# inferenceengine/shadernn

Measured on NVIDIA B200. Metric: frames/sec, higher is better.
Workload: dtype f32 (split-fp16 hi+lo storage for activations and weights, 3 fp16 MMAs per product, fp32 accumulate)

## Files before the change

### include/snnb.h

```cpp
#ifndef SNNB_H_
#define SNNB_H_

#include <stddef.h>
#include <stdint.h>

#ifdef __cplusplus
extern "C" {
#endif

#define SNNB_VERSION 100

typedef struct snnb_context snnb_context;
typedef struct snnb_tensor snnb_tensor;
typedef struct snnb_weights snnb_weights;
typedef struct snnb_model snnb_model;
typedef struct snnb_timer snnb_timer;

enum { SNNB_ACT_NONE = 0, SNNB_ACT_RELU = 1, SNNB_ACT_RELU6 = 2, SNNB_ACT_TANH = 3, SNNB_ACT_SIGMOID = 4, SNNB_ACT_LEAKY_RELU = 5, SNNB_ACT_SILU = 6, SNNB_ACT_SOFTMAX = 7 };
enum { SNNB_PAD_NONE = 0, SNNB_PAD_CONSTANT = 1, SNNB_PAD_REPLICATE = 2, SNNB_PAD_REFLECT = 3 };
enum { SNNB_ALGO_AUTO = 0, SNNB_ALGO_SIMT = 1, SNNB_ALGO_TCGEN05 = 2, SNNB_ALGO_TCGEN05_STREAMK = 3 };
enum { SNNB_PRECISION_FP32X3 = 0, SNNB_PRECISION_FP16W = 1, SNNB_PRECISION_FP16 = 2 };

int snnb_context_create(int device, snnb_context** out);
int snnb_context_destroy(snnb_context* ctx);
// ... 48 lines not shown
int snnb_instancenorm_launch(snnb_context* ctx, const snnb_weights* w, int activation, float leaky_alpha, const snnb_tensor* in, snnb_tensor* out);
int snnb_subpixel_launch(snnb_context* ctx, int r, const snnb_tensor* in, snnb_tensor* out);

int snnb_timer_create(snnb_context* ctx, snnb_timer** out);
int snnb_timer_start(snnb_timer* t);
int snnb_timer_stop(snnb_timer* t);
int snnb_timer_elapsed_ms(snnb_timer* t, float* ms);
int snnb_timer_destroy(snnb_timer* t);

typedef struct snnb_graph snnb_graph;
int snnb_graph_capture_begin(snnb_context* ctx);
int snnb_graph_capture_end(snnb_context* ctx, snnb_graph** out);
int snnb_graph_launch(snnb_graph* g);
int snnb_graph_destroy(snnb_graph* g);

typedef struct {
    int batch;
    int input_width;
    int input_height;
    int conv_algo;
    int use_cuda_graph;
    int fuse;
    int precision;
} snnb_model_options;

int snnb_model_load_json(snnb_context* ctx, const char* json_path, const snnb_model_options* opt, snnb_model** out);
int snnb_model_destroy(snnb_model* m);
int snnb_model_num_layers(const snnb_model* m);
int snnb_model_layer_info(const snnb_model* m, int i, char* name, int name_cap, char* type, int type_cap, int* n, int* h, int* w, int* c);
int snnb_model_num_inputs(const snnb_model* m);
int snnb_model_num_outputs(const snnb_model* m);
int snnb_model_input_dims(const snnb_model* m, int idx, int* n, int* h, int* w, int* c);
int snnb_model_output_dims(const snnb_model* m, int idx, int* n, int* h, int* w, int* c);
int snnb_model_run(snnb_model* m, const float* host_input_nhwc, float* host_output, size_t out_capacity, int* classes_1based);
int snnb_model_submit(snnb_model* m, const float* host_input_nhwc, float* host_output, size_t out_capacity, int* classes_1based, int* ticket);
int snnb_model_submit_u8(snnb_model* m, const uint8_t* host_input_nhwc_u8, const float* mean4, const float* norm4, float* host_output, size_t out_capacity,
                         int* classes_1based, int* ticket);
typedef struct {
    const uint8_t* input_u8;
    int src_height, src_width;
    int linear_filter;
    float mean4[4], norm4[4];
    float* output_f32;
    size_t output_capacity;
    uint8_t* output_u8;
    float out_scale, out_offset;
    int* classes_1based;
} snnb_image_io;
int snnb_model_submit_image(snnb_model* m, const snnb_image_io* io, int* ticket);
int snnb_model_wait(snnb_model* m, int ticket);
int snnb_model_set_input(snnb_model* m, int idx, const float* host_input_nhwc);
int snnb_model_forward(snnb_model* m);
int snnb_model_get_output(snnb_model* m, int idx, float* host_output, size_t out_capacity);
int snnb_model_layer_output(snnb_model* m, int layer, float* host_nhwc, size_t capacity);
int snnb_model_dump_outputs(snnb_model* m, const char* dir);
int snnb_model_time_layers(snnb_model* m, float* times_ms, int capacity);
int snnb_model_layer_kernel(const snnb_model* m, int layer, char* name, int name_cap);
int snnb_model_launches_per_forward(const snnb_model* m);
int snnb_model_get_boxes(snnb_model* m, int n, float* rows6, int max_rows, int* count);
int snnb_model_weight_arena(snnb_model* m, void** device_ptr, size_t* bytes);

typedef struct snnb_comm snnb_comm;
int snnb_nccl_unique_id(unsigned char id128[128]);
int snnb_nccl_comm_create(snnb_context* ctx, int rank, int world_size, const unsigned char id128[128], snnb_comm** out);
int snnb_nccl_comm_destroy(snnb_comm* comm);
int snnb_bcast_weights(snnb_model* m, snnb_comm* comm, int root);

typedef struct snnb_layer_json snnb_layer_json;
int snnb_layer_json_number(const snnb_layer_json* layer, const char* key, double* out);
int snnb_layer_json_string(const snnb_layer_json* layer, const char* key, char* buf, int cap);
int snnb_layer_json_numbers(const snnb_layer_json* layer, const char* path, const double** data, size_t* count);
typedef struct {
    void* user;
    int (*output_dims)(void* user, int num_inputs, const int* in_hwc, int* out_hwc);
    int (*run)(void* user, snnb_context* ctx, int num_inputs, const snnb_tensor* const* inputs, snnb_tensor* output);
    void (*destroy)(void* user);
} snnb_layer_impl;
typedef int (*snnb_layer_creator)(void* registry_user, const snnb_layer_json* layer, snnb_layer_impl* out);
int snnb_register_layer(const char* type_name, snnb_layer_creator creator, void* registry_user);
int snnb_unregister_layer(const char* type_name);
int snnb_tensor_planes(const snnb_tensor* t, void** hi, void** lo, int* cp);
int snnb_debug_streamk_schedule(int tiles, int num_kb, int sms, int* rows, int capacity);
int snnb_debug_feed_plan(int k, int stride, int pad_x, int ic, int out[5]);

#ifdef __cplusplus
}
#endif
#endif
```

### shadernn_b200/_lib.py

```python
import ctypes as C
import os

HERE = os.path.dirname(os.path.abspath(__file__))
LIB_PATH = os.path.join(HERE, "libsnn_b200.so")

c_float_p = C.POINTER(C.c_float)
c_int_p = C.POINTER(C.c_int)
vp = C.c_void_p


class ConvDesc(C.Structure):
    _fields_ = [
        ("in_channels", C.c_int),
        ("out_channels", C.c_int),
        ("kernel", C.c_int),
        ("stride", C.c_int),
        ("pad_x", C.c_int),
        ("pad_y", C.c_int),
        ("pad_mode", C.c_int),
        ("activation", C.c_int),
        ("leaky_alpha", C.c_float),
        ("algo", C.c_int),
    ]

# ... 29 lines not shown

SIGNATURES = {
    "snnb_version": (C.c_int, []),
    "snnb_last_error": (C.c_char_p, []),
    "snnb_context_create": (C.c_int, [C.c_int, C.POINTER(vp)]),
    "snnb_context_destroy": (C.c_int, [vp]),
    "snnb_sync": (C.c_int, [vp]),
    "snnb_context_stream": (vp, [vp]),
    "snnb_launch_count": (C.c_uint64, [vp]),
    "snnb_context_set_precision": (C.c_int, [vp, C.c_int]),
    "snnb_tensor_alloc": (C.c_int, [vp, C.c_int, C.c_int, C.c_int, C.c_int, C.POINTER(vp)]),
    "snnb_tensor_free": (C.c_int, [vp]),
    "snnb_tensor_dims": (C.c_int, [vp, c_int_p, c_int_p, c_int_p, c_int_p]),
    "snnb_tensor_upload_nhwc": (C.c_int, [vp, vp, vp]),
    "snnb_tensor_download_nhwc": (C.c_int, [vp, vp, vp]),
    "snnb_tensor_upload_c4hw4": (C.c_int, [vp, vp, vp]),
    "snnb_tensor_download_c4hw4": (C.c_int, [vp, vp, vp]),
    "snnb_tensor_dump": (C.c_int, [vp, vp, C.c_char_p]),
    "snnb_weights_pack_conv2d": (C.c_int, [vp, C.POINTER(ConvDesc), vp, vp, vp, vp, vp, vp, C.POINTER(vp)]),
    "snnb_weights_pack_depthwise": (C.c_int, [vp, C.POINTER(ConvDesc), vp, vp, vp, vp, vp, vp, C.POINTER(vp)]),
    "snnb_weights_pack_dense": (C.c_int, [vp, C.c_int, C.c_int, vp, vp, C.POINTER(vp)]),
    "snnb_weights_pack_channels": (C.c_int, [vp, C.c_int, vp, vp, vp, vp, C.POINTER(vp)]),
    "snnb_weights_free": (C.c_int, [vp]),
    "snnb_conv2d_launch": (C.c_int, [vp, C.POINTER(ConvDesc), vp, vp, vp, vp]),
    "snnb_depthwise_launch": (C.c_int, [vp, C.POINTER(ConvDesc), vp, vp, vp]),
    "snnb_maxpool_launch": (C.c_int, [vp, C.c_int, C.c_int, vp, vp]),
    "snnb_avgpool_launch": (C.c_int, [vp, C.c_int, C.c_int, vp, vp]),
    "snnb_add_launch": (C.c_int, [vp, C.c_int, C.c_float, vp, vp, vp]),
    "snnb_batchnorm_launch": (C.c_int, [vp, vp, C.c_int, C.c_float, vp, vp]),
    "snnb_activation_launch": (C.c_int, [vp, C.c_int, C.c_float, vp, vp]),
    "snnb_dense_launch": (C.c_int, [vp, vp, C.c_int, C.c_float, vp, vp]),
    "snnb_softmax_launch": (C.c_int, [vp, vp, vp]),
    "snnb_argmax1": (C.c_int, [vp, vp, c_int_p]),
    "snnb_flatten_launch": (C.c_int, [vp, vp, vp]),
    "snnb_concat_launch": (C.c_int, [vp, vp, vp, vp]),
    "snnb_upsample_launch": (C.c_int, [vp, C.c_float, C.c_int, vp, vp]),
    "snnb_pad_launch": (C.c_int, [vp, C.c_int, C.c_int, C.c_int, vp, vp]),
    "snnb_instancenorm_launch": (C.c_int, [vp, vp, C.c_int, C.c_float, vp, vp]),
    "snnb_subpixel_launch": (C.c_int, [vp, C.c_int, vp, vp]),
    "snnb_timer_create": (C.c_int, [vp, C.POINTER(vp)]),
    "snnb_timer_start": (C.c_int, [vp]),
    "snnb_timer_stop": (C.c_int, [vp]),
    "snnb_timer_elapsed_ms": (C.c_int, [vp, c_float_p]),
    "snnb_timer_destroy": (C.c_int, [vp]),
    "snnb_model_load_json": (C.c_int, [vp, C.c_char_p, C.POINTER(ModelOptions), C.POINTER(vp)]),
    "snnb_model_destroy": (C.c_int, [vp]),
    "snnb_model_num_layers": (C.c_int, [vp]),
    "snnb_model_layer_info": (C.c_int, [vp, C.c_int, C.c_char_p, C.c_int, C.c_char_p, C.c_int, c_int_p, c_int_p, c_int_p, c_int_p]),
    "snnb_model_num_inputs": (C.c_int, [vp]),
    "snnb_model_num_outputs": (C.c_int, [vp]),
    "snnb_model_input_dims": (C.c_int, [vp, C.c_int, c_int_p, c_int_p, c_int_p, c_int_p]),
    "snnb_model_output_dims": (C.c_int, [vp, C.c_int, c_int_p, c_int_p, c_int_p, c_int_p]),
    "snnb_model_run": (C.c_int, [vp, vp, vp, C.c_size_t, vp]),
    "snnb_graph_capture_begin": (C.c_int, [vp]),
    "snnb_graph_capture_end": (C.c_int, [vp, C.POINTER(C.c_void_p)]),
    "snnb_graph_launch": (C.c_int, [vp]),
    "snnb_graph_destroy": (C.c_int, [vp]),
    "snnb_model_submit": (C.c_int, [vp, vp, vp, C.c_size_t, vp, c_int_p]),
    "snnb_model_submit_u8": (C.c_int, [vp, vp, vp, vp, vp, C.c_size_t, vp, c_int_p]),
    "snnb_model_submit_image": (C.c_int, [vp, C.POINTER(ImageIO), c_int_p]),
    "snnb_model_wait": (C.c_int, [vp, C.c_int]),
    "snnb_model_set_input": (C.c_int, [vp, C.c_int, vp]),
    "snnb_model_forward": (C.c_int, [vp]),
    "snnb_model_get_output": (C.c_int, [vp, C.c_int, vp, C.c_size_t]),
    "snnb_model_layer_output": (C.c_int, [vp, C.c_int, vp, C.c_size_t]),
    "snnb_model_dump_outputs": (C.c_int, [vp, C.c_char_p]),
    "snnb_model_time_layers": (C.c_int, [vp, c_float_p, C.c_int]),
    "snnb_model_launches_per_forward": (C.c_int, [vp]),
    "snnb_model_layer_kernel": (C.c_int, [vp, C.c_int, C.c_char_p, C.c_int]),
    "snnb_model_get_boxes": (C.c_int, [vp, C.c_int, c_float_p, C.c_int, c_int_p]),
    "snnb_model_weight_arena": (C.c_int, [vp, C.POINTER(vp), C.POINTER(C.c_size_t)]),
    "snnb_nccl_unique_id": (C.c_int, [C.c_char_p]),
    "snnb_nccl_comm_create": (C.c_int, [vp, C.c_int, C.c_int, C.c_char_p, C.POINTER(vp)]),
    "snnb_nccl_comm_destroy": (C.c_int, [vp]),
    "snnb_bcast_weights": (C.c_int, [vp, vp, C.c_int]),
    "snnb_register_layer": (C.c_int, [C.c_char_p, vp, vp]),
    "snnb_unregister_layer": (C.c_int, [C.c_char_p]),
    "snnb_layer_json_number": (C.c_int, [vp, C.c_char_p, C.POINTER(C.c_double)]),
    "snnb_layer_json_string": (C.c_int, [vp, C.c_char_p, C.c_char_p, C.c_int]),
    "snnb_layer_json_numbers": (C.c_int, [vp, C.c_char_p, C.POINTER(C.POINTER(C.c_double)), C.POINTER(C.c_size_t)]),
    "snnb_tensor_planes": (C.c_int, [vp, C.POINTER(vp), C.POINTER(vp), c_int_p]),
    "snnb_debug_streamk_schedule": (C.c_int, [C.c_int, C.c_int, C.c_int, c_int_p, C.c_int]),
    "snnb_debug_feed_plan": (C.c_int, [C.c_int, C.c_int, C.c_int, C.c_int, c_int_p]),
}

_lib = None


class SnnbError(RuntimeError):
    pass


def lib():
    global _lib
    if _lib is None:
        if not os.path.exists(LIB_PATH):
            raise SnnbError(
                "%s is missing — build it with `python -m shadernn_b200._build` (or __graft_entry__.build()). "
                "shadernn_b200 has no CPU or PyTorch fallback." % LIB_PATH)
        l = C.CDLL(LIB_PATH)
        for name, (res, args) in SIGNATURES.items():
            fn = getattr(l, name)
            fn.restype = res
            fn.argtypes = args
        _lib = l
    return _lib


def check(rc, what=""):
    if rc != 0:
        msg = lib().snnb_last_error()
        raise SnnbError("%s failed (status %d): %s" % (what or "snnb call", rc, msg.decode("utf-8", "replace") if msg else "?"))
```

### shadernn_b200/csrc/capi.cpp

```cpp
#include <cstdarg>
#include <cstdlib>
#include <cstring>
#include <memory>

#include "snnb_internal.h"

namespace snnb {

static thread_local char g_err[1024] = "";
void set_error(const char* fmt, ...) {
    va_list ap;
    va_start(ap, fmt);
    vsnprintf(g_err, sizeof(g_err), fmt, ap);
    va_end(ap);
}
const char* get_error() { return g_err; }

bool pdl_enabled() {
    static const bool on = getenv("SNNB_NO_PDL") == nullptr;
    return on;
}

int ensure_stage(snnb_context* ctx, size_t bytes) {
    if (ctx->stage_dev_bytes < bytes) {
// ... 37 lines not shown
    const size_t plane  = ((size_t) t->n * feed_h * feed_w * 4 + 63) / 64 * 64;
    const size_t planes = t->lo ? 2 : 1;
    SNNB_CUDA_OK(cudaMalloc(&t->feed_hi, plane * planes * sizeof(__half)));
    SNNB_CUDA_OK(cudaMemsetAsync(t->feed_hi, 0, plane * planes * sizeof(__half), t->ctx->stream));
    t->feed_lo = t->lo ? t->feed_hi + plane : nullptr;
    t->feed_h = feed_h, t->feed_w = feed_w, t->feed_py = py, t->feed_px = px;
    return 0;
}

}

using namespace snnb;

#define CHECK_DIMS_EQ(a, b, what) SNNB_REQUIRE((a)->n == (b)->n && (a)->h == (b)->h && (a)->w == (b)->w && (a)->c == (b)->c, what ": tensor dims differ")

extern "C" {

int snnb_version(void) { return SNNB_VERSION; }
int snnb_context_set_precision(snnb_context* ctx, int precision) {
    SNNB_REQUIRE(ctx && (precision == SNNB_PRECISION_FP32X3 || precision == SNNB_PRECISION_FP16W), "snnb_context_set_precision: FP32X3 or FP16W (FP16 storage is a model option)");
    ctx->precision = precision;
    return 0;
}
const char* snnb_last_error(void) { return get_error(); }

int snnb_context_create(int device, snnb_context** out) {
    SNNB_REQUIRE(out, "snnb_context_create: null out");
    int count = 0;
    cudaError_t e = cudaGetDeviceCount(&count);
    if (e != cudaSuccess || count == 0) {
        set_error("snnb_context_create: no CUDA device available (%s). This library has no CPU fallback.", cudaGetErrorString(e));
        return 1;
    }
    SNNB_REQUIRE(device >= 0 && device < count, "snnb_context_create: device %d out of range (%d devices)", device, count);
    SNNB_CUDA_OK(cudaSetDevice(device));
    cudaDeviceProp prop;
    SNNB_CUDA_OK(cudaGetDeviceProperties(&prop, device));
    SNNB_REQUIRE(prop.major == 10, "snnb_context_create: device %d is sm_%d%d; this library is built for sm_100a (B200) only", device, prop.major, prop.minor);
    auto ctx      = std::make_unique<snnb_context>();
    ctx->device   = device;
    ctx->sm_count = prop.multiProcessorCount;
    SNNB_CUDA_OK(cudaStreamCreateWithFlags(&ctx->stream, cudaStreamNonBlocking));
    *out = ctx.release();
    return 0;
}

int snnb_context_destroy(snnb_context* ctx) {
    if (!ctx) return 0;
    cudaSetDevice(ctx->device);
    cudaStreamSynchronize(ctx->stream);
    if (ctx->stage_dev) cudaFree(ctx->stage_dev);
    if (ctx->stage_host) cudaFreeHost(ctx->stage_host);
    for (void* b : ctx->scratch_blocks) cudaFree(b);
    cudaStreamDestroy(ctx->stream);
    delete ctx;
    return 0;
}

int snnb_sync(snnb_context* ctx) {
    SNNB_REQUIRE(ctx, "snnb_sync: null context");
    SNNB_CUDA_OK(cudaStreamSynchronize(ctx->stream));
    return 0;
}
void* snnb_context_stream(snnb_context* ctx) { return ctx ? (void*) ctx->stream : nullptr; }
uint64_t snnb_launch_count(snnb_context* ctx) { return ctx ? ctx->launches : 0; }

int snnb_tensor_alloc(snnb_context* ctx, int n, int h, int w, int c, snnb_tensor** out) { return tensor_alloc(ctx, n, h, w, c, out); }
int snnb_tensor_free(snnb_tensor* t) {
    if (!t) return 0;
    if (t->owns && t->hi) cudaFree(t->hi);
    if (t->feed_hi) cudaFree(t->feed_hi);
    delete t;
    return 0;
}
int snnb_debug_feed_plan(int k, int stride, int pad_x, int ic, int out[5]) {
    FeedPlan fp;
    if (!out || !make_feed_plan(k, stride, pad_x, ic, fp)) return 0;
    out[0] = fp.px, out[1] = fp.d, out[2] = fp.nch, out[3] = fp.ksteps, out[4] = fp.rows_per_panel;
    return 1;
}
int snnb_debug_streamk_schedule(int tiles, int num_kb, int sms, int* rows, int capacity) {
    SNNB_REQUIRE(rows || capacity == 0, "snnb_debug_streamk_schedule: null buffer");
    return streamk_schedule(tiles, num_kb, sms, rows, capacity);
}
int snnb_tensor_planes(const snnb_tensor* t, void** hi, void** lo, int* cp) {
    SNNB_REQUIRE(t && hi && lo && cp, "snnb_tensor_planes: null argument");
    *hi = t->hi, *lo = t->lo, *cp = t->cp;
    return 0;
}
int snnb_tensor_dims(const snnb_tensor* t, int* n, int* h, int* w, int* c) {
    SNNB_REQUIRE(t, "snnb_tensor_dims: null tensor");
    if (n) *n = t->n;
    if (h) *h = t->h;
    if (w) *w = t->w;
    if (c) *c = t->c;
    return 0;
}
int snnb_tensor_upload_nhwc(snnb_context* ctx, snnb_tensor* t, const float* host) {
    SNNB_REQUIRE(ctx && t && host, "snnb_tensor_upload_nhwc: null argument");
    const size_t bytes = t->pixels() * t->c * sizeof(float);
    if (ensure_stage(ctx, bytes)) return 1;
    SNNB_CUDA_OK(cudaMemcpyAsync(ctx->stage_dev, host, bytes, cudaMemcpyHostToDevice, ctx->stream));
    if (launch_split_f32(ctx, ctx->stage_dev, t)) return 1;
    SNNB_CUDA_OK(cudaStreamSynchronize(ctx->stream));
    return 0;
}
int snnb_tensor_download_nhwc(snnb_context* ctx, const snnb_tensor* t, float* host) {
    SNNB_REQUIRE(ctx && t && host, "snnb_tensor_download_nhwc: null argument");
    const size_t bytes = t->pixels() * t->c * sizeof(float);
    if (ensure_stage(ctx, bytes)) return 1;
    if (launch_merge_f32(ctx, t, ctx->stage_dev)) return 1;
    SNNB_CUDA_OK(cudaMemcpyAsync(host, ctx->stage_dev, bytes, cudaMemcpyDeviceToHost, ctx->stream));
    SNNB_CUDA_OK(cudaStreamSynchronize(ctx->stream));
    return 0;
}

static void c4_to_nhwc(const float* c4, int N, int H, int W, int C, float* nhwc) {
    const int D = (C + 3) / 4;
    for (int n = 0; n < N; ++n)
        for (int y = 0; y < H; ++y)
            for (int x = 0; x < W; ++x)
                for (int c = 0; c < C; ++c)
                    nhwc[(((size_t) n * H + y) * W + x) * C + c] = c4[((((size_t) n * D + c / 4) * H + y) * W + x) * 4 + (c % 4)];
}
static void nhwc_to_c4(const float* nhwc, int N, int H, int W, int C, float* c4) {
    const int D = (C + 3) / 4;
    memset(c4, 0, sizeof(float) * (size_t) N * D * H * W * 4);
    for (int n = 0; n < N; ++n)
        for (int y = 0; y < H; ++y)
            for (int x = 0; x < W; ++x)
                for (int c = 0; c < C; ++c)
                    c4[((((size_t) n * D + c / 4) * H + y) * W + x) * 4 + (c % 4)] = nhwc[(((size_t) n * H + y) * W + x) * C + c];
}
int snnb_tensor_upload_c4hw4(snnb_context* ctx, snnb_tensor* t, const float* host_c4) {
    SNNB_REQUIRE(ctx && t && host_c4, "snnb_tensor_upload_c4hw4: null argument");
    std::vector<float> tmp(t->pixels() * t->c);
    c4_to_nhwc(host_c4, t->n, t->h, t->w, t->c, tmp.data());
    return snnb_tensor_upload_nhwc(ctx, t, tmp.data());
}
int snnb_tensor_download_c4hw4(snnb_context* ctx, const snnb_tensor* t, float* host_c4) {
    SNNB_REQUIRE(ctx && t && host_c4, "snnb_tensor_download_c4hw4: null argument");
    std::vector<float> tmp(t->pixels() * t->c);
    if (snnb_tensor_download_nhwc(ctx, t, tmp.data())) return 1;
    nhwc_to_c4(tmp.data(), t->n, t->h, t->w, t->c, host_c4);
    return 0;
}
int snnb_tensor_dump(snnb_context* ctx, const snnb_tensor* t, const char* path) {
    SNNB_REQUIRE(ctx && t && path, "snnb_tensor_dump: null argument");
    const int D = (t->c + 3) / 4;
    std::vector<float> c4((size_t) t->n * D * t->h * t->w * 4);
    if (snnb_tensor_download_c4hw4(ctx, t, c4.data())) return 1;
    for (int n = 0; n < t->n; ++n) {
        std::string p = path;
        if (t->n > 1) p += ".n" + std::to_string(n);
        FILE* f = fopen(p.c_str(), "wb");
        SNNB_REQUIRE(f, "snnb_tensor_dump: cannot open %s", p.c_str());
        char header[32];
        memset(header, 0, sizeof(header));
        snprintf(header, sizeof(header), "%d %d %d %d", t->w, t->h, D, t->c);
        fwrite(header, 1, sizeof(header), f);
        fwrite(c4.data() + (size_t) n * D * t->h * t->w * 4, sizeof(float), (size_t) D * t->h * t->w * 4, f);
        fclose(f);
    }
    return 0;
}

// ... 244 lines not shown
```

### shadernn_b200/csrc/engine/core.cpp

```cpp
#include <algorithm>
#include <cstring>
#include <unordered_map>
#include <unordered_set>

#include "engine.h"

using namespace snnb;

namespace snn {

using namespace dp;

MixedInferenceCore::~MixedInferenceCore() {
    if (ctx) {
        cudaSetDevice(ctx->device);
        cudaStreamSynchronize(ctx->stream);
    }
    if (cuGraphExec) cudaGraphExecDestroy(cuGraphExec);
    if (cuGraph) cudaGraphDestroy(cuGraph);
    for (auto* t : ownedTensors) snnb_tensor_free(t);
    if (arena) cudaFree(arena);
    if (scratchArena) cudaFree(scratchArena);
    if (ioStage) cudaFree(ioStage);
    if (argmaxDev) cudaFree(argmaxDev);
    if (yoloDev) cudaFree(yoloDev);
    if (yoloHost) cudaFreeHost(yoloHost);
    for (auto& sl : slots) {
        if (sl.yoloDev) cudaFree(sl.yoloDev);
        if (sl.yoloHost) cudaFreeHost(sl.yoloHost);
        if (sl.stageIn) cudaFree(sl.stageIn);
        if (sl.stageResize) cudaFree(sl.stageResize);
        if (sl.stageOut) cudaFree(sl.stageOut);
        if (sl.smallHost) cudaFreeHost(sl.smallHost);
        if (sl.argmax) cudaFree(sl.argmax);
        if (sl.h2dDone) cudaEventDestroy(sl.h2dDone);
        if (sl.stageFree) cudaEventDestroy(sl.stageFree);
        if (sl.resultReady) cudaEventDestroy(sl.resultReady);
    }
    if (copyStream) cudaStreamDestroy(copyStream);
}

std::unique_ptr<MixedInferenceCore> MixedInferenceCore::create(snnb_context* ctx, const std::string& modelFileName, const ShaderGenOptions& options,
                                                               std::string& err) {
    std::unique_ptr<MixedInferenceCore> core(new MixedInferenceCore());
    core->ctx     = ctx;
    core->options = options;
    try {
        core->layers = loadFromJsonModel(modelFileName);
        core->graph  = generateInferenceGraph(core->layers, options);
    } catch (std::exception& e) {
        err = e.what();
        return nullptr;
    }
    if (!core->init(err)) return nullptr;
    return core;
}

static bool allZeroPadding(const PaddingSpec& p) {
    uint32_t o[4];
    p.offsets(3, true, o);
    const bool keyword_same = !(p.t == "valid" || p.t == "none" || (!p.t.empty() && std::all_of(p.t.begin(), p.t.end(), ::isdigit)));
    return !keyword_same && o[0] == 0 && o[1] == 0 && o[2] == 0 && o[3] == 0;
}

bool MixedInferenceCore::init(std::string& err) {
    const int N = (int) options.batch;
    const bool twoPlanes = options.precision != SNNB_PRECISION_FP16;
    std::unordered_map<GenericModelLayer*, int> order;
    for (size_t i = 0; i < graph.sorted.size(); ++i) order[graph.sorted[i]] = (int) i;

    for (auto* L : graph.sorted) {
        if (L->isInputLayer) inputLayers.push_back(L);
        if (L->nextLayers.empty()) outputLayers.push_back(L);
        if (L->typeName == "YOLO") yolo = static_cast<YOLOLayer*>(L);
    }
    std::stable_sort(inputLayers.begin(), inputLayers.end(), [](GenericModelLayer* a, GenericModelLayer* b) {
        return static_cast<InputLayerLayer*>(a)->_desc.inputIndex < static_cast<InputLayerLayer*>(b)->_desc.inputIndex;
    });
    if (inputLayers.empty()) {
        err = "model has no InputLayer";
        return false;
    }

    std::unordered_map<GenericModelLayer*, GenericModelLayer*> alias;
    if (options.fuse) {
        for (auto* L : graph.sorted) {
            if (L->typeName == "Pad" && L->nextLayers.size() == 1 && L->prevLayers.size() == 1) {
                auto* pad  = static_cast<PadLayer*>(L);
                auto* next = L->nextLayers[0];
                PaddingSpec* np = nullptr;
                if (next->typeName == "Conv2D" && static_cast<Conv2DLayer*>(next)->_desc.kernelSize > 1) np = &static_cast<Conv2DLayer*>(next)->_desc.padding;
                if (next->typeName == "SeparableConv2D" && pad->mode == "constant") np = &static_cast<SeparableConv2DLayer*>(next)->_desc.padding;
                if (np && allZeroPadding(*np)) {
                    uint32_t o[4];
                    pad->padding.offsets(0, false, o);
                    np->t = std::to_string(o[0]), np->b = std::to_string(o[1]), np->l = std::to_string(o[2]), np->r = std::to_string(o[3]);
                    np->mode       = pad->mode;
                    L->fusedAway   = true;
                    alias[L]       = L->prevLayers[0];
                }
            }
            if (L->typeName == "Add" && L->prevLayers.size() == 2) {
                auto* add = static_cast<AddLayer*>(L);
                GenericModelLayer* a = L->prevLayers[0];
                GenericModelLayer* b = L->prevLayers[1];
                auto fusable = [&](GenericModelLayer* c, GenericModelLayer* other) {
                    if (c->typeName != "Conv2D" || c->nextLayers.size() != 1 || c->fusedAway) return false;
                    auto* conv = static_cast<Conv2DLayer*>(c);
                    if (conv->_desc.activation.id != SNNB_ACT_NONE || conv->residual || conv->fusedAct >= 0) return false;
                    return order[other] < order[c] && c != other;
                };
                GenericModelLayer* conv = nullptr;
                GenericModelLayer* other = nullptr;
                if (fusable(b, a))
                    conv = b, other = a;
                else if (fusable(a, b))
                    conv = a, other = b;
                if (conv) {
                    conv->fusedAct   = add->activation.id;
                    conv->fusedAlpha = add->activation.alpha;
                    conv->prevLayers.push_back(other);
                    L->fusedAway     = true;
                    alias[conv]      = L;
                }
            }
            if (L->typeName == "Dense" && L->prevLayers.size() == 1) {
                GenericModelLayer* f = L->prevLayers[0];
                GenericModelLayer* pool = (f->typeName == "Flatten" && f->prevLayers.size() == 1 && f->nextLayers.size() == 1 &&
                                           static_cast<FlattenLayer*>(f)->activation.id == SNNB_ACT_NONE)
                                              ? f->prevLayers[0]
                                              : f;
                auto dimsOf = [&](GenericModelLayer* x) { return graph.outputDims[order[x]]; };
                if (pool->typeName == "AveragePooling2D" && static_cast<PoolingLayer*>(pool)->isAvg && pool->nextLayers.size() == 1 && pool->prevLayers.size() == 1 &&
                    !pool->fusedAway && dimsOf(pool).width * dimsOf(pool).height == 1 && static_cast<DenseLayer*>(L)->units <= 256 &&
                    dimsOf(pool->prevLayers[0]).width * dimsOf(pool->prevLayers[0]).height >= 4 && dimsOf(pool->prevLayers[0]).depth <= 4096 &&
                    static_cast<PoolingLayer*>(pool)->_desc.kernelSize >= dimsOf(pool->prevLayers[0]).width &&
                    static_cast<PoolingLayer*>(pool)->_desc.kernelSize >= dimsOf(pool->prevLayers[0]).height) {
                    static_cast<DenseLayer*>(L)->gapSource = pool->prevLayers[0];
                    pool->fusedAway = true;
                }
            }
            if (L->typeName == "Flatten" && L->inputDims.size() == 1 && L->inputDims[0].width * L->inputDims[0].height == 1 &&
                static_cast<FlattenLayer*>(L)->activation.id == SNNB_ACT_NONE) {
                L->fusedAway = true;
                alias[L]     = L->prevLayers[0];
            }
        }
    }

    std::unordered_map<GenericModelLayer*, snnb_tensor*> outOf;
    auto resolve = [&](GenericModelLayer* L) -> GenericModelLayer* {
        std::unordered_set<GenericModelLayer*> seen;
        while (alias.count(L) && !seen.count(L)) {
            seen.insert(L);
            L = alias[L];
        }
        return L;
    };
    for (size_t i = 0; i < graph.sorted.size(); ++i) {
        GenericModelLayer* L = graph.sorted[i];
        if (L->typeName == "YOLO") continue;
        GenericModelLayer* owner = resolve(L);
        if (owner != L && !(L->typeName == "Conv2D")) continue;
        if (outOf.count(owner)) continue;
        const Dims& d = graph.outputDims[order[owner]];
        snnb_tensor* t = nullptr;
        if (tensor_alloc(ctx, N, (int) d.height, (int) d.width, (int) d.depth, &t, twoPlanes)) {
            err = get_error();
            return false;
        }
        ownedTensors.push_back(t);
        outOf[owner] = t;
    }
    for (auto* L : graph.sorted) {
        if (L->typeName == "YOLO") {
            for (auto* p : L->prevLayers) L->inputs.push_back(outOf.at(resolve(p)));
            continue;
        }
        GenericModelLayer* owner = resolve(L);
        L->output                = outOf.count(owner) ? outOf[owner] : nullptr;
        if (L->fusedAway) continue;
        size_t nin = L->prevLayers.size();
        if (L->typeName == "Conv2D" && static_cast<Conv2DLayer*>(L)->fusedAct >= 0) {
            nin -= 1;
            L->residual = outOf.at(resolve(L->prevLayers.back()));
        }
        for (size_t k = 0; k < nin; ++k) L->inputs.push_back(outOf.at(resolve(L->prevLayers[k])));
        if (L->typeName == "Conv2D") {
            auto* cl  = static_cast<Conv2DLayer*>(L);
            cl->algo = options.convAlgo;
            int ph = 0, pw = 0;
            snnb_weights probe_w;
            probe_w.w_hi = probe_w.w_lo = reinterpret_cast<__half*>(1);
            probe_w.w_row_hi = probe_w.w_row_lo = reinterpret_cast<__half*>(1);
            probe_w.row_stride = (int) cl->_desc.stride, probe_w.row_pad = 0;
            std::swap(cl->weights, probe_w);
            const bool prepad = cl->wantsPrepad(L->inputs[0], L->output, options.convAlgo, ph, pw);
            std::swap(cl->weights, probe_w);
            if (prepad) {
                if (tensor_alloc(ctx, N, ph, pw, L->inputs[0]->c, &cl->prepadded, twoPlanes)) {
                    err = get_error();
                    return false;
                }
                ownedTensors.push_back(cl->prepadded);
            }
            {
                static const bool noFeed = getenv("SNNB_NO_FEED") != nullptr;
                GenericModelLayer* src   = resolve(L->prevLayers[0]);
                snnb_tensor* in          = L->inputs[0];
                const int mode           = padModeId(cl->_desc.padding.mode);
                uint32_t offs[4];
                cl->_desc.padding.offsets((int) cl->_desc.kernelSize, true, offs);
                const int k = (int) cl->_desc.kernelSize, padX = (int) offs[0], padY = (int) offs[2];
                FeedPlan fp;
                if (!noFeed && !prepad && src->isInputLayer && !in->feed_hi && options.convAlgo != SNNB_ALGO_SIMT && !L->residual && L->output->c <= 64 &&
                    (mode == SNNB_PAD_NONE || mode == SNNB_PAD_CONSTANT) && make_feed_plan(k, (int) cl->_desc.stride, padX, in->c, fp)) {
                    const int tilesX = (L->output->w + 127) / 128;
                    const int needW  = 2 * (tilesX * 128 - 1) + 2 * fp.nch;
                    const int needH  = 2 * (L->output->h - 1) + k - padY + padY;
                    const int feedW  = (std::max(in->w + fp.px, needW) + 1) & ~1;
                    const int feedH  = std::max(in->h + padY, needH);
                    if (tensor_alloc_feed(in, feedH, feedW, padY, fp.px)) {
                        err = get_error();
                        return false;
                    }
                    cl->feedInput = true;
                }
            }
        }
        if (L->typeName == "Dense") {
            auto* dl = static_cast<DenseLayer*>(L);
            if (L->inputs[0]->h * L->inputs[0]->w != 1) {
                if (tensor_alloc(ctx, N, 1, 1, (int) dl->numInputPlanes, &dl->flat, twoPlanes)) {
                    err = get_error();
                    return false;
                }
                ownedTensors.push_back(dl->flat);
            }
            if ((uint32_t) (L->inputs[0]->h * L->inputs[0]->w * L->inputs[0]->c) != dl->numInputPlanes) {
                err = L->name + ": Dense expects " + std::to_string(dl->numInputPlanes) + " inputs, graph provides " +
                      std::to_string(L->inputs[0]->h * L->inputs[0]->w * L->inputs[0]->c);
                return false;
            }
        }
        if ((L->typeName == "Add" || L->typeName == "Concatenate") && L->inputs.size() != 2) {
            err = L->name + ": expects exactly two inputs";
            return false;
        }
        auto dimsStr = [](const snnb_tensor* t) { return std::to_string(t->h) + "x" + std::to_string(t->w) + "x" + std::to_string(t->c); };
        if (L->typeName == "Conv2D" || L->typeName == "SeparableConv2D" || L->typeName == "BatchNormalization" || L->typeName == "InstanceNorm") {
            if (L->inputs.empty() || !L->output) {
                err = L->name + ": layer has no input";
                return false;
            }
            if ((uint32_t) L->inputs[0]->c != L->numInputPlanes) {
                err = L->name + ": inputPlanes " + std::to_string(L->numInputPlanes) + " but the producing layer has " + std::to_string(L->inputs[0]->c) + " channels";
                return false;
            }
            const uint32_t wantOut = (L->typeName == "Conv2D") ? L->numOutputPlanes : L->numInputPlanes;
            if ((uint32_t) L->output->c != wantOut) {
                err = L->name + ": output tensor has " + std::to_string(L->output->c) + " channels, weights are packed for " + std::to_string(wantOut);
                return false;
            }
        }
        if (L->typeName == "Add") {
            for (auto* in : L->inputs)
                if (in->h != L->output->h || in->w != L->output->w || in->c != L->output->c) {
                    err = L->name + ": Add operand " + dimsStr(in) + " does not match the output " + dimsStr(L->output);
                    return false;
                }
        }
        if (L->typeName == "Conv2D" && L->residual &&
            (L->residual->h != L->output->h || L->residual->w != L->output->w || L->residual->c != L->output->c)) {
            err = L->name + ": fused Add operand " + dimsStr(L->residual) + " does not match the output " + dimsStr(L->output);
            return false;
        }
        if (L->typeName == "Concatenate") {
            if (L->inputs[0]->h != L->inputs[1]->h || L->inputs[0]->w != L->inputs[1]->w || L->inputs[0]->c + L->inputs[1]->c != L->output->c ||
                L->inputs[0]->h != L->output->h || L->inputs[0]->w != L->output->w) {
                err = L->name + ": Concatenate operands " + dimsStr(L->inputs[0]) + " and " + dimsStr(L->inputs[1]) + " do not stack into " + dimsStr(L->output);
                return false;
            }
        }
    }

    for (auto* in : inputLayers) {
        snnb_tensor* t = in->output;
        if (!t || !t->feed_hi || getenv("SNNB_NO_FEED_ONLY")) continue;
        bool only = true;
        int readers = 0;
        for (auto* L : graph.sorted) {
            if (L->fusedAway || L->isInputLayer) continue;
            const bool reads = std::find(L->inputs.begin(), L->inputs.end(), t) != L->inputs.end() || L->residual == t;
            if (!reads) continue;
            ++readers;
            only = only && L->typeName == "Conv2D" && static_cast<Conv2DLayer*>(L)->feedInput && L->inputs.size() >= 1 && L->inputs[0] == t && L->residual != t &&
                   std::count(L->inputs.begin(), L->inputs.end(), t) == 1;
        }
        for (auto* o : outputLayers) only = only && o->output != t;
        t->feed_only = only && readers > 0;
    }

    std::vector<std::pair<GenericModelLayer*, PackedHost>> packed;
    size_t total = 0, scratchTotal = 0;
    for (auto* L : graph.sorted) {
        PackedHost p;
        try {
            L->packWeights(p);
        } catch (std::exception& e) {
            err = L->name + ": " + e.what();
            return false;
        }
        if (p.kind) {
            total += p.device_bytes();
            packed.emplace_back(L, std::move(p));
        }
        if (L->typeName == "InstanceNorm") {
            static_cast<InstanceNormLayer*>(L)->computeScratch(N);
            scratchTotal += (L->scratchBytes() + 255) & ~(size_t) 255;
        }
    }
    arenaBytes = total ? total : 256;
    if (cudaMalloc(&arena, arenaBytes) != cudaSuccess) {
        err = "cudaMalloc(weight arena) failed";
        return false;
    }
    {
        char* cur = (char*) arena;
        for (auto& pr : packed) {
            if (place_weights(ctx, pr.second, cur, &pr.first->weights)) {
                err = get_error();
                return false;
            }
            cur += pr.first->weights.bytes;
        }
    }
    if (scratchTotal) {
        if (cudaMalloc(&scratchArena, scratchTotal) != cudaSuccess) {
            err = "cudaMalloc(scratch) failed";
            return false;
        }
        char* cur = (char*) scratchArena;
        for (auto* L : graph.sorted)
            if (L->scratchBytes()) {
                L->scratch = (float*) cur;
                cur += (L->scratchBytes() + 255) & ~(size_t) 255;
            }
    }

    size_t maxFloats = 1;
    for (auto* L : inputLayers) maxFloats = std::max(maxFloats, L->output->pixels() * (size_t) L->output->c);
    for (auto* L : outputLayers)
        if (L->output) maxFloats = std::max(maxFloats, L->output->pixels() * (size_t) L->output->c);
    ioStageBytes = maxFloats * sizeof(float);
    if (cudaMalloc(&ioStage, ioStageBytes) != cudaSuccess || cudaMalloc(&argmaxDev, sizeof(int) * N) != cudaSuccess) {
        err = "cudaMalloc(io staging) failed";
        return false;
    }
    if (yolo) {
        const size_t yb = yolo->candidateBytes();
        if (cudaMalloc(&yoloDev, yb) != cudaSuccess || cudaMallocHost(&yoloHost, yb) != cudaSuccess) {
            err = "cudaMalloc(YOLO candidate lists) failed";
            return false;
        }
    }
    {
        GenericModelLayer* last = nullptr;
        for (auto* L : outputLayers)
            if (L->output) {
                last = L;
                break;
            }
        isClassifier = last && last->output->h == 1 && last->output->w == 1 && last->output->c > 1;
    }

    const uint64_t before = ctx->launches;
// ... 160 lines not shown
    const bool resize = io && (io->src_height != in->h || io->src_width != in->w);
    const size_t inBytes = resize ? (size_t) in->n * io->src_height * io->src_width * in->c : in->pixels() * in->c * (u8 ? sizeof(uint8_t) : sizeof(float));
    const size_t outFloats = out ? out->pixels() * out->c : 0;
    SNNB_REQUIRE(!hostOutput || capacityFloats >= outFloats, "submit: output buffer too small (%zu < %zu floats)", capacityFloats, outFloats);
    SNNB_REQUIRE(!(io && io->output_u8) || (out && io->output_capacity >= outFloats), "submit_image: u8 output buffer too small or the model has no tensor output");
    void* stage = sl.stageIn;
    if (resize) {
        if (inBytes > sl.stageResizeBytes) {
            SNNB_CUDA_OK(cudaStreamSynchronize(ctx->stream));
            if (sl.stageResize) SNNB_CUDA_OK(cudaFree(sl.stageResize));
            SNNB_CUDA_OK(cudaMalloc(&sl.stageResize, inBytes));
            sl.stageResizeBytes = inBytes;
        }
        stage = sl.stageResize;
    }
    if (sl.everUsed) SNNB_CUDA_OK(cudaStreamWaitEvent(copyStream, sl.stageFree, 0));
    SNNB_CUDA_OK(cudaMemcpyAsync(stage, hostInput, inBytes, cudaMemcpyHostToDevice, copyStream));
    SNNB_CUDA_OK(cudaEventRecord(sl.h2dDone, copyStream));
    SNNB_CUDA_OK(cudaStreamWaitEvent(ctx->stream, sl.h2dDone, 0));
    if (resize) {
        if (launch_resize_u8(ctx, reinterpret_cast<const uint8_t*>(stage), io->src_height, io->src_width, in, mean, norm, io->linear_filter != 0)) return 1;
    } else if (u8 ? launch_split_u8(ctx, reinterpret_cast<const uint8_t*>(sl.stageIn), in, mean, norm) : launch_split_f32(ctx, sl.stageIn, in)) {
        return 1;
    }
    SNNB_CUDA_OK(cudaEventRecord(sl.stageFree, ctx->stream));
    if (forward()) return 1;
    sl.userOut = nullptr, sl.userClasses = nullptr, sl.userFloats = 0;
    static const bool noSmall = getenv("SNNB_NO_SMALL_RESULT") != nullptr;
    const bool small = !noSmall && isClassifier && !(io && io->output_u8) && (hostOutput || classes1) &&
                       outFloats * sizeof(float) + options.batch * sizeof(int) <= SMALL_RESULT_BYTES;
    if (small) {
        float* vals = static_cast<float*>(sl.smallDev);
        int* cls    = reinterpret_cast<int*>(static_cast<char*>(sl.smallDev) + outFloats * sizeof(float));
        if (launch_result_small(ctx, out, hostOutput ? vals : nullptr, classes1 ? cls : nullptr)) return 1;
        sl.userOut = hostOutput, sl.userClasses = classes1, sl.userFloats = outFloats;
        hostOutput = nullptr, classes1 = nullptr;
    }
    if (hostOutput) {
        if (launch_merge_f32(ctx, out, sl.stageOut)) return 1;
        SNNB_CUDA_OK(cudaMemcpyAsync(hostOutput, sl.stageOut, outFloats * sizeof(float), cudaMemcpyDeviceToHost, ctx->stream));
    }
    if (io && io->output_u8) {
        if (launch_merge_u8(ctx, out, reinterpret_cast<uint8_t*>(sl.stageOut), io->out_scale, io->out_offset)) return 1;
        SNNB_CUDA_OK(cudaMemcpyAsync(io->output_u8, sl.stageOut, outFloats, cudaMemcpyDeviceToHost, ctx->stream));
    }
    sl.classesHost = nullptr;
    if (classes1 && isClassifier) {
        if (launch_argmax(ctx, out, sl.argmax)) return 1;
        SNNB_CUDA_OK(cudaMemcpyAsync(classes1, sl.argmax, sizeof(int) * options.batch, cudaMemcpyDeviceToHost, ctx->stream));
        sl.classesHost = classes1;
    }
    if (yolo && decodeYolo(sl.yoloDev, sl.yoloHost, false)) return 1;
    SNNB_CUDA_OK(cudaEventRecord(sl.resultReady, ctx->stream));
    sl.busy = sl.everUsed = true;
    *ticket = nextTicket++;
    return 0;
}

int MixedInferenceCore::wait(int ticket) {
    SNNB_REQUIRE(ticket >= 0 && ticket < nextTicket && ticket >= nextTicket - 2, "wait: ticket %d is not in flight", ticket);
    Slot& sl = slots[ticket & 1];
    SNNB_REQUIRE(sl.busy, "wait: ticket %d was already waited for", ticket);
    SNNB_CUDA_OK(cudaEventSynchronize(sl.resultReady));
    if (sl.userOut) std::memcpy(sl.userOut, sl.smallHost, sl.userFloats * sizeof(float));
    if (sl.userClasses) {
        const int* cls = reinterpret_cast<const int*>(static_cast<const char*>(sl.smallHost) + sl.userFloats * sizeof(float));
        for (uint32_t i = 0; i < options.batch; ++i) sl.userClasses[i] = cls[i] + 1;
    }
    sl.userOut = nullptr, sl.userClasses = nullptr;
    if (sl.classesHost)
        for (uint32_t i = 0; i < options.batch; ++i) sl.classesHost[i] += 1;
    sl.busy = false;
    if (yolo) {
        const int rc = yolo->finishDecode(sl.yoloHost, sl.yoloDev, boxes);
        SNNB_REQUIRE(rc >= 0, "wait: corrupt detection candidate list");
        return rc;
    }
    return 0;
}

int MixedInferenceCore::layerOutput(int layerId, float* host, size_t capacityFloats) {
    SNNB_REQUIRE(layerId >= 0 && layerId < (int) layers.size() && host, "layerOutput: bad argument");
    GenericModelLayer* L = layers[layerId].get();
    SNNB_REQUIRE(L->output, "layerOutput: layer %d (%s) has no device tensor", layerId, L->name.c_str());
    SNNB_REQUIRE(!(L->typeName == "Conv2D" && static_cast<Conv2DLayer*>(L)->fusedAct >= 0),
                 "layerOutput: layer %d (%s) was fused into its Add; load the model with fuse=0 to observe it", layerId, L->name.c_str());
    SNNB_REQUIRE(!(L->fusedAway && L->typeName == "AveragePooling2D"),
                 "layerOutput: layer %d (%s) was fused into the classifier head (pool + Dense in one launch); load the model with fuse=0 to observe it", layerId,
                 L->name.c_str());
    const size_t floats = L->output->pixels() * L->output->c;
    SNNB_REQUIRE(capacityFloats >= floats, "layerOutput: buffer too small (%zu < %zu floats)", capacityFloats, floats);
    return snnb_tensor_download_nhwc(ctx, L->output, host);
}

int MixedInferenceCore::timeLayers(std::vector<float>& ms) {
    ms.assign(layers.size(), 0.0f);
    std::vector<cudaEvent_t> ev(graph.sorted.size() + 1);
    for (auto& e : ev) SNNB_CUDA_OK(cudaEventCreate(&e));
    ExecOptions eo;
    eo.convAlgo = options.convAlgo, eo.precision = options.precision;
    SNNB_CUDA_OK(cudaEventRecord(ev[0], ctx->stream));
    layerKernels.assign(layers.size(), std::string());
    for (size_t i = 0; i < graph.sorted.size(); ++i) {
        GenericModelLayer* L = graph.sorted[i];
        if (!(L->fusedAway || L->isInputLayer || L->typeName == "YOLO")) {
            ctx->last_kernel = nullptr;
            if (int rc = L->run(ctx, eo)) return rc;
            layerKernels[L->layerId] = ctx->last_kernel ? ctx->last_kernel : (L->typeName + " kernels");
        }
        SNNB_CUDA_OK(cudaEventRecord(ev[i + 1], ctx->stream));
    }
    SNNB_CUDA_OK(cudaStreamSynchronize(ctx->stream));
    for (size_t i = 0; i < graph.sorted.size(); ++i) {
        float t = 0;
        SNNB_CUDA_OK(cudaEventElapsedTime(&t, ev[i], ev[i + 1]));
        ms[graph.sorted[i]->layerId] = t;
    }
    for (auto& e : ev) cudaEventDestroy(e);
    return 0;
}

int MixedInferenceCore::dumpOutputs(const std::string& dir) {
    for (auto& l : layers) {
        if (!l->output || l->fusedAway) continue;
        SNNB_REQUIRE(!(l->typeName == "Conv2D" && l->fusedAct >= 0), "dumpOutputs: %s was fused into its Add; load the model with fuse=0 to dump every layer", l->name.c_str());
        std::string path = dir + "/" + l->name + " pass[0].dump";
        if (snnb_tensor_dump(ctx, l->output, path.c_str())) return 1;
    }
    return 0;
}

}
```

### shadernn_b200/csrc/engine/engine.h

```cpp
#pragma once

#include <algorithm>
#include <map>
#include <memory>
#include <string>
#include <vector>

#include "../snnb_internal.h"
#include "json.h"

namespace snn {

struct SNNModelOutputBoxes {
    std::vector<std::vector<float>> rows;
};

namespace dp {

class ModelParser {
public:
    explicit ModelParser(const std::string& fileName);
    ~ModelParser();
    int getLayerCount() const;
    std::string getLayerName(int layerId) const;
// ... 30 lines not shown
    int id      = SNNB_ACT_NONE;
    float alpha = 0.0f;
    static int fromString(const std::string& s);
};

struct ExecOptions;

class GenericModelLayer {
public:
    virtual ~GenericModelLayer() {}
    std::string name;
    std::string typeName;
    int layerId = -1;
    std::vector<GenericModelLayer*> prevLayers, nextLayers;
    std::vector<Dims> inputDims;
    uint32_t numInputPlanes = 0, numOutputPlanes = 0;
    bool isInputLayer = false;

    virtual void getOutputDims(uint32_t& width, uint32_t& height, uint32_t& depth) const;
    struct Transform { float scaleW = 1, scaleH = 1, transW = 0, transH = 0; };
    virtual Transform getOutputScaleDimAdjustment() const { return Transform(); }

    virtual void packWeights(snnb::PackedHost&) {}
    snnb_weights weights;
    std::vector<snnb_tensor*> inputs;
    snnb_tensor* output = nullptr;
    virtual int run(snnb_context* ctx, const ExecOptions& opt) = 0;
    bool fusedAway          = false;
    snnb_tensor* residual   = nullptr;
    int fusedAct            = -1;
    float fusedAlpha        = 0.0f;
    float* scratch          = nullptr;
    size_t scratchBytes() const { return _scratchBytes; }

protected:
    size_t _scratchBytes = 0;
};

class PluginLayer : public GenericModelLayer {
public:
    snnb_layer_impl impl {};
    ~PluginLayer() override {
        if (impl.destroy) impl.destroy(impl.user);
    }
    void getOutputDims(uint32_t& w, uint32_t& h, uint32_t& d) const override;
    int run(snnb_context* ctx, const ExecOptions& opt) override;
};

typedef GenericModelLayer* (*LayerCreator)(ModelParser&, int);
void initLayerRegisty();
void registerLayer(const std::string& layerName, LayerCreator creator);
GenericModelLayer* createLayerInstance(std::string layerName, ModelParser& parser, int i);

struct InputLayerDesc {
    uint32_t inputWidth = 0, inputHeight = 0, inputChannels = 0, inputIndex = 0;
    void parse(ModelParser& parser, int layerId);
};
class InputLayerLayer : public GenericModelLayer {
public:
    InputLayerDesc _desc;
    void getOutputDims(uint32_t& w, uint32_t& h, uint32_t& d) const override;
    int run(snnb_context*, const ExecOptions&) override { return 0; }
};

struct GenericConvDesc {
    uint32_t kernelSize = 1, stride = 1;
    PaddingSpec padding;
    ActivationSpec activation;
    std::string activationName;
    std::vector<float> weights;
    std::vector<float> biases;
    bool useBatchNormalization = false;
    std::map<std::string, std::vector<float>> batchNormalization;
};
struct Conv2DDesc : GenericConvDesc {
    void parse(ModelParser& parser, int layerId);
};
class Conv2DLayer : public GenericModelLayer {
public:
    Conv2DDesc _desc;
    int algo = SNNB_ALGO_AUTO;
    snnb_tensor* prepadded = nullptr;
    bool feedInput = false;
    bool wantsPrepad(const snnb_tensor* in, const snnb_tensor* out, int convAlgo, int& ph, int& pw) const;
    Transform getOutputScaleDimAdjustment() const override;
    void getOutputDims(uint32_t& w, uint32_t& h, uint32_t& d) const override;
    void packWeights(snnb::PackedHost& p) override;
    int run(snnb_context* ctx, const ExecOptions& opt) override;
};
struct SeparableConv2DDesc : GenericConvDesc {
    void parse(ModelParser& parser, int layerId);
};
class SeparableConv2DLayer : public GenericModelLayer {
public:
    SeparableConv2DDesc _desc;
    void getOutputDims(uint32_t& w, uint32_t& h, uint32_t& d) const override;
    void packWeights(snnb::PackedHost& p) override;
    int run(snnb_context* ctx, const ExecOptions& opt) override;
};
struct PoolDesc {
    uint32_t kernelSize = 1, stride = 1;
    PaddingSpec padding;
    void parseMax(ModelParser& parser, int layerId);
    void parseAvg(ModelParser& parser, int layerId);
};
class PoolingLayer : public GenericModelLayer {
public:
    PoolDesc _desc;
    bool isAvg = false;
    Transform getOutputScaleDimAdjustment() const override;
    int run(snnb_context* ctx, const ExecOptions& opt) override;
};
class AdaptiveAvgPool2dLayer : public GenericModelLayer {
public:
    uint32_t poolSize = 1;
    void getOutputDims(uint32_t& w, uint32_t& h, uint32_t& d) const override;
    int run(snnb_context* ctx, const ExecOptions& opt) override;
};
class AddLayer : public GenericModelLayer {
public:
    ActivationSpec activation;
    int run(snnb_context* ctx, const ExecOptions& opt) override;
};
class BatchNormalizationLayer : public GenericModelLayer {
public:
    std::map<std::string, std::vector<float>> batchNormalization;
    ActivationSpec activation;
    void packWeights(snnb::PackedHost& p) override;
    int run(snnb_context* ctx, const ExecOptions& opt) override;
};
class InstanceNormLayer : public GenericModelLayer {
public:
    std::vector<float> gamma, beta;
    ActivationSpec activation;
    void packWeights(snnb::PackedHost& p) override;
    int run(snnb_context* ctx, const ExecOptions& opt) override;
    void setScratch() { _scratchBytes = 0; }
    void computeScratch(int n) { _scratchBytes = snnb::instnorm_scratch_floats(n, snnb::round_up((int) numOutputPlanes, 8)) * sizeof(float); }
};
class ActivationLayer : public GenericModelLayer {
public:
    ActivationSpec activation;
    int run(snnb_context* ctx, const ExecOptions& opt) override;
};
class DenseLayer : public GenericModelLayer {
public:
    std::vector<float> kernel;
    std::vector<float> biases;
    ActivationSpec activation;
    uint32_t units = 0;
    void getOutputDims(uint32_t& w, uint32_t& h, uint32_t& d) const override;
    void packWeights(snnb::PackedHost& p) override;
    int run(snnb_context* ctx, const ExecOptions& opt) override;
    snnb_tensor* flat = nullptr;
    GenericModelLayer* gapSource = nullptr;
};
class FlattenLayer : public GenericModelLayer {
public:
    ActivationSpec activation;
    void getOutputDims(uint32_t& w, uint32_t& h, uint32_t& d) const override;
    int run(snnb_context* ctx, const ExecOptions& opt) override;
};
class ConcatenateLayer : public GenericModelLayer {
public:
    void getOutputDims(uint32_t& w, uint32_t& h, uint32_t& d) const override;
    int run(snnb_context* ctx, const ExecOptions& opt) override;
// ... 126 lines not shown
```

### shadernn_b200/csrc/engine/layers.cpp

```cpp
#include <algorithm>
#include <cmath>

#include <cstring>
#include <thread>

#include "engine.h"

using namespace snnb;

namespace snn {
namespace dp {

void GenericModelLayer::getOutputDims(uint32_t& width, uint32_t& height, uint32_t& depth) const {
    width = height = depth = 0U;
    float accSW = 0, accSH = 0, accTW = 0, accTH = 0;
    const Transform t = getOutputScaleDimAdjustment();
    for (auto& dim : inputDims) {
        accSW  = std::max(accSW, t.scaleW * dim.width);
        accTW  = std::max(accTW, t.transW);
        accSH  = std::max(accSH, t.scaleH * dim.height);
        accTH  = std::max(accTH, t.transH);
        width  = (uint32_t) (accSW + accTW);
        height = (uint32_t) (accSH + accTH);
        depth  = std::max(depth, dim.depth);
    }
}

void InputLayerLayer::getOutputDims(uint32_t& w, uint32_t& h, uint32_t& d) const {
    w = inputDims.empty() ? _desc.inputWidth : inputDims[0].width;
    h = inputDims.empty() ? _desc.inputHeight : inputDims[0].height;
    d = _desc.inputChannels;
}

GenericModelLayer::Transform Conv2DLayer::getOutputScaleDimAdjustment() const {
    uint32_t offset[4];
    _desc.padding.offsets((int) _desc.kernelSize, true, offset);
    float scale       = 1 / static_cast<float>(_desc.stride);
    float translation = 0.0f;
    if (_desc.kernelSize % 2 != 0) {
        translation = 1 + (static_cast<float>(offset[0] + offset[1]) - static_cast<float>(_desc.kernelSize)) / static_cast<float>(_desc.stride);
    } else {
        translation = 1 + (static_cast<float>(offset[0] + offset[1] - 1) - static_cast<float>(_desc.kernelSize)) / static_cast<float>(_desc.stride);
    }
    return Transform {scale, scale, translation, translation};
}
void Conv2DLayer::getOutputDims(uint32_t& w, uint32_t& h, uint32_t& d) const {
    GenericModelLayer::getOutputDims(w, h, d);
    d = numOutputPlanes;
}
int padModeId(const std::string& m) {
    if (m == "constant") return SNNB_PAD_CONSTANT;
    if (m == "replicate") return SNNB_PAD_REPLICATE;
    if (m == "reflect") return SNNB_PAD_REFLECT;
    return SNNB_PAD_NONE;
}
static const float* bnv(const std::map<std::string, std::vector<float>>& bn, const char* key) {
    auto it = bn.find(key);
    return (it == bn.end() || it->second.empty()) ? nullptr : it->second.data();
}
void Conv2DLayer::packWeights(PackedHost& p) {
    const auto& bn = _desc.batchNormalization;
    const bool use = _desc.useBatchNormalization;
    pack_conv2d_host((int) numInputPlanes, (int) numOutputPlanes, (int) _desc.kernelSize, _desc.weights.data(), _desc.biases.empty() ? nullptr : _desc.biases.data(),
                     use ? bnv(bn, "gamma") : nullptr, use ? bnv(bn, "beta") : nullptr, use ? bnv(bn, "movingMean") : nullptr,
                     use ? bnv(bn, "movingVariance") : nullptr, p);
    {
        uint32_t offs[4];
        _desc.padding.offsets((int) _desc.kernelSize, true, offs);
        const int mode = padModeId(_desc.padding.mode);
        if (mode == SNNB_PAD_NONE || mode == SNNB_PAD_CONSTANT) {
            pack_rowwin_host(p, (int) _desc.stride, _desc.kernelSize == 1 ? 0 : (int) offs[0]);
            if (feedInput) pack_feed_host(p, (int) _desc.stride, _desc.kernelSize == 1 ? 0 : (int) offs[0]);
        } else {
            pack_rowwin_host(p, (int) _desc.stride, 0);
        }
    }
    std::vector<float>().swap(_desc.weights);
}
bool Conv2DLayer::wantsPrepad(const snnb_tensor* in, const snnb_tensor* out, int convAlgo, int& ph, int& pw) const {
    const int mode = padModeId(_desc.padding.mode);
    if (!(mode == SNNB_PAD_REPLICATE || mode == SNNB_PAD_REFLECT) || _desc.kernelSize <= 1 || convAlgo == SNNB_ALGO_SIMT) return false;
    ConvArgs probe {in, nullptr, const_cast<snnb_tensor*>(out), &weights, (int) _desc.kernelSize, (int) _desc.stride, 0, 0, SNNB_PAD_CONSTANT, 0, 0.0f};
    if (!conv2d_umma_supported(probe)) return false;
    ph = (out->h - 1) * (int) _desc.stride + (int) _desc.kernelSize;
    pw = (out->w - 1) * (int) _desc.stride + (int) _desc.kernelSize;
    return true;
}

int Conv2DLayer::run(snnb_context* ctx, const ExecOptions& opt) {
    uint32_t offs[4];
    _desc.padding.offsets((int) _desc.kernelSize, true, offs);
    if (prepadded) {
        if (launch_pad(ctx, inputs[0], prepadded, (int) offs[0], (int) offs[2], padModeId(_desc.padding.mode))) return 1;
        ConvArgs a {prepadded, residual, output, &weights, (int) _desc.kernelSize, (int) _desc.stride, 0, 0, SNNB_PAD_CONSTANT,
                    fusedAct >= 0 ? fusedAct : _desc.activation.id, fusedAct >= 0 ? fusedAlpha : _desc.activation.alpha};
        a.precision = opt.precision;
        return launch_conv2d_umma(ctx, a);
    }
    ConvArgs a;
    a.in = inputs[0], a.residual = residual, a.out = output, a.w = &weights;
    a.k = (int) _desc.kernelSize, a.stride = (int) _desc.stride;
    a.pad_x = _desc.kernelSize == 1 ? 0 : (int) offs[0];
    a.pad_y = _desc.kernelSize == 1 ? 0 : (int) offs[2];
    a.pad_mode = padModeId(_desc.padding.mode);
    a.act      = fusedAct >= 0 ? fusedAct : _desc.activation.id;
    a.alpha    = fusedAct >= 0 ? fusedAlpha : _desc.activation.alpha;
    a.precision = opt.precision;
    const int want = algo != SNNB_ALGO_AUTO ? algo : opt.convAlgo;
    if (want != SNNB_ALGO_SIMT && conv2d_umma_supported(a)) return launch_conv2d_umma(ctx, a);
    if (want == SNNB_ALGO_TCGEN05) {
        set_error("%s: tcgen05 path requested but unsupported for this shape", name.c_str());
        return 2;
    }
    return launch_conv2d_simt(ctx, a);
}

void SeparableConv2DLayer::getOutputDims(uint32_t& width, uint32_t& height, uint32_t& depth) const {
    uint32_t po[4];
    _desc.padding.offsets((int) _desc.kernelSize, true, po);
    width = height = depth = 0;
    for (auto& dim : inputDims) {
        width  = (dim.width - _desc.kernelSize + po[0] + po[2]) / _desc.stride + 1;
        height = (dim.height - _desc.kernelSize + po[1] + po[3]) / _desc.stride + 1;
        depth  = dim.depth;
        break;
    }
}
void SeparableConv2DLayer::packWeights(PackedHost& p) {
    const auto& bn = _desc.batchNormalization;
    const bool use = _desc.useBatchNormalization;
    pack_depthwise_host((int) numInputPlanes, (int) _desc.kernelSize, _desc.weights.data(), _desc.biases.empty() ? nullptr : _desc.biases.data(),
                        use ? bnv(bn, "gamma") : nullptr, use ? bnv(bn, "beta") : nullptr, use ? bnv(bn, "movingMean") : nullptr,
                        use ? bnv(bn, "movingVariance") : nullptr, p);
}
int SeparableConv2DLayer::run(snnb_context* ctx, const ExecOptions&) {
    uint32_t offs[4];
    _desc.padding.offsets((int) _desc.kernelSize, true, offs);
    ConvArgs a;
    a.in = inputs[0], a.residual = nullptr, a.out = output, a.w = &weights;
    a.k = (int) _desc.kernelSize, a.stride = (int) _desc.stride;
    a.pad_x = (int) offs[0], a.pad_y = (int) offs[2];
    a.pad_mode = SNNB_PAD_CONSTANT, a.act = _desc.activation.id, a.alpha = _desc.activation.alpha;
    return launch_depthwise(ctx, a);
}

GenericModelLayer::Transform PoolingLayer::getOutputScaleDimAdjustment() const {
    float scale = 1.0f / _desc.stride, translation;
    if (_desc.padding.validLike())
        translation = 1.0f - (static_cast<float>(_desc.kernelSize) / static_cast<float>(_desc.stride));
    else
        translation = 1.0f - 1.0f / static_cast<float>(_desc.stride);
    return Transform {scale, scale, translation, translation};
}
int PoolingLayer::run(snnb_context* ctx, const ExecOptions&) { return launch_pool(ctx, inputs[0], output, (int) _desc.kernelSize, (int) _desc.stride, isAvg); }

void AdaptiveAvgPool2dLayer::getOutputDims(uint32_t& w, uint32_t& h, uint32_t& d) const {
    w = h = poolSize;
    d     = inputDims.empty() ? numOutputPlanes : inputDims[0].depth;
}
int AdaptiveAvgPool2dLayer::run(snnb_context* ctx, const ExecOptions&) {
    const snnb_tensor* in = inputs[0];
    if (in->h % (int) poolSize || in->w % (int) poolSize || in->h / (int) poolSize != in->w / (int) poolSize) {
        set_error("%s: AdaptiveAvgPool2d needs H and W divisible by pool (%d x %d -> %u)", name.c_str(), in->h, in->w, poolSize);
        return 2;
    }
    const int k = in->h / (int) poolSize;
    return launch_pool(ctx, in, output, k, k, true);
}

int AddLayer::run(snnb_context* ctx, const ExecOptions&) { return launch_add(ctx, inputs[0], inputs[1], output, activation.id, activation.alpha); }
void BatchNormalizationLayer::packWeights(PackedHost& p) {
    pack_channels_host((int) numOutputPlanes, bnv(batchNormalization, "gamma"), bnv(batchNormalization, "beta"), bnv(batchNormalization, "movingMean"),
                       bnv(batchNormalization, "movingVariance"), p);
}
int BatchNormalizationLayer::run(snnb_context* ctx, const ExecOptions&) { return launch_batchnorm(ctx, inputs[0], output, &weights, activation.id, activation.alpha); }
void InstanceNormLayer::packWeights(PackedHost& p) { pack_channels_host((int) numOutputPlanes, gamma.data(), beta.data(), nullptr, nullptr, p); }
int InstanceNormLayer::run(snnb_context* ctx, const ExecOptions&) {
    return launch_instancenorm(ctx, inputs[0], output, &weights, activation.id, activation.alpha, scratch);
}
int ActivationLayer::run(snnb_context* ctx, const ExecOptions&) { return launch_activation(ctx, inputs[0], output, activation.id, activation.alpha); }

void DenseLayer::getOutputDims(uint32_t& w, uint32_t& h, uint32_t& d) const {
    w = h = 1;
    d     = units;
}
void DenseLayer::packWeights(PackedHost& p) {
    pack_conv2d_host((int) numInputPlanes, (int) units, 1, kernel.data(), biases.empty() ? nullptr : biases.data(), nullptr, nullptr, nullptr, nullptr, p);
    p.kind = 3;
    std::vector<float>().swap(kernel);
}
int DenseLayer::run(snnb_context* ctx, const ExecOptions& opt) {
    if (gapSource && gapSource->output && gap_dense_supported(gapSource->output, output, &weights))
// ... 227 lines not shown
```

### shadernn_b200/csrc/kernels_umma.cu

```cuda
#include <cuda.h>

#include <algorithm>
#include <vector>
#include <cstdlib>

#include "snnb_internal.h"

namespace snnb {

constexpr int UM_BLOCK_M     = 128;
constexpr int UM_BLOCK_K     = 64;
constexpr int UM_MAX_N       = 128;
constexpr int UM_MAX_N2      = 256;
constexpr int UM_STAGES      = 3;
constexpr int UM_A_BYTES     = UM_BLOCK_M * 128;
constexpr int UM_B_BYTES     = UM_MAX_N * 128;
constexpr int UM_STAGE_BYTES = 2 * UM_A_BYTES + 2 * UM_B_BYTES;
constexpr int UM_EPI_WARPS   = 8;
constexpr int UM_THREADS     = 64 + 32 * UM_EPI_WARPS;
constexpr int UM_ACC_COLS    = 2 * UM_MAX_N;
constexpr int UM_TMEM_COLS   = 2 * UM_ACC_COLS;
constexpr int UM_STG_BYTES   = 2 * UM_BLOCK_M * 128;
constexpr int UM_SCHED_SLOTS = 8;
constexpr int UM_SMEM_BYTES  = UM_STAGES * UM_STAGE_BYTES + UM_STG_BYTES + 1024  + 320 ;
constexpr int UM_SMEM_BYTES_SPLIT = (UM_STAGES - 1) * UM_STAGE_BYTES + 2 * UM_STG_BYTES + 1024 + 320;

constexpr int HL_TW = 8, HL_TH = 16, HL_W = HL_TW + 2, HL_H = HL_TH + 2;
constexpr int HL_PLANE         = (HL_W * HL_H * 128 + 1023) / 1024 * 1024;
constexpr int HL_A_STAGES      = 2;
constexpr int HL_A_STAGE_BYTES = 2 * HL_PLANE;
constexpr int HL_B_STAGES      = 6;
constexpr int HL_B_RING_BYTES  = 6 * UM_B_BYTES;
constexpr int HL_SMEM_BYTES    = HL_A_STAGES * HL_A_STAGE_BYTES + HL_B_RING_BYTES + UM_STG_BYTES + 1024 + 384;

struct UmmaParams {
    __half* out_hi;
    __half* out_lo;
    const __half* res_hi;
    const __half* res_lo;
    const float* bias;
    int N, OH, OW, OC, OCp;
    int tw, th, tn, rows_used;
    int tiles_x, tiles_y, tiles_n, tiles_oc, n_blk;
    int ksize, stride, pad_x, pad_y;
    int cblocks, ICp;
    int act;
    float alpha;
    int has_res;
    int ksplit, kb_per_split;
    int* sched_counter;
    float* partials;
    int* counters;
    long long* trace;
    int ablate;
    int has_lo;
    int sk, sk_dp, sk_ctas;
    long long sk_units;
    int b_stages, b_stage_bytes;
};

__device__ __forceinline__ uint32_t smem_u32(const void* p) { return (uint32_t) __cvta_generic_to_shared(p); }

__device__ __forceinline__ void mbar_init(uint32_t bar, uint32_t count) { asm volatile("mbarrier.init.shared::cta.b64 [%0], %1;" ::"r"(bar), "r"(count)); }
__device__ __forceinline__ void mbar_expect_tx(uint32_t bar, uint32_t bytes) {
    asm volatile("mbarrier.arrive.expect_tx.shared::cta.b64 _, [%0], %1;" ::"r"(bar), "r"(bytes) : "memory");
}
__device__ __forceinline__ void mbar_arrive(uint32_t bar) { asm volatile("mbarrier.arrive.shared::cta.b64 _, [%0];" ::"r"(bar) : "memory"); }
__device__ __forceinline__ bool mbar_try_wait(uint32_t bar, uint32_t parity) {
    uint32_t ok;
    asm volatile(
        "{\n\t.reg .pred p;\n\t"
        "mbarrier.try_wait.parity.shared::cta.b64 p, [%1], %2;\n\t"
        "selp.u32 %0, 1, 0, p;\n\t}"
        : "=r"(ok)
        : "r"(bar), "r"(parity)
        : "memory");
    return ok != 0;
}
__device__ __forceinline__ bool mbar_test_wait(uint32_t bar, uint32_t parity) {
    uint32_t ok;
    asm volatile(
        "{\n\t.reg .pred p;\n\t"
        "mbarrier.test_wait.parity.shared::cta.b64 p, [%1], %2;\n\t"
        "selp.u32 %0, 1, 0, p;\n\t}"
        : "=r"(ok)
        : "r"(bar), "r"(parity)
        : "memory");
    return ok != 0;
}
__device__ unsigned int g_producer_progress[1024];
__device__ __forceinline__ void producer_progress(int lane, unsigned int code) {
    if (lane == 0) *reinterpret_cast<volatile unsigned int*>(&g_producer_progress[blockIdx.x & 1023]) = code;
}
__device__ __forceinline__ void mbar_wait(uint32_t bar, uint32_t parity) {
    if (mbar_try_wait(bar, parity)) return;
    const long long t0 = clock64();
    bool reported      = false;
    while (!mbar_try_wait(bar, parity)) {
        const long long dt = clock64() - t0;
        if (dt > 4000000000LL && !reported) {
            uint32_t dyn;
            asm volatile("mov.u32 %0, %%dynamic_smem_size;" : "=r"(dyn));
            printf("tcgen05 kernel (dynamic smem %u B): mbarrier wait timed out (block %d thread %d bar 0x%x parity %u, producer progress 0x%x)\n", dyn, blockIdx.x,
                   threadIdx.x, bar, parity, *reinterpret_cast<volatile unsigned int*>(&g_producer_progress[blockIdx.x & 1023]));
            reported = true;
        }
        if (dt > 4040000000LL) __trap();
    }
}
__device__ __forceinline__ bool elect_one() {
    uint32_t pred;
    asm volatile("{\n\t.reg .pred p;\n\telect.sync _|p, 0xffffffff;\n\tselp.u32 %0, 1, 0, p;\n\t}" : "=r"(pred));
    return pred != 0;
}
__device__ __forceinline__ void fence_barrier_init() { asm volatile("fence.mbarrier_init.release.cluster;" ::: "memory"); }
__device__ __forceinline__ void tc_fence_before() { asm volatile("tcgen05.fence::before_thread_sync;" ::: "memory"); }
__device__ __forceinline__ void tc_fence_after() { asm volatile("tcgen05.fence::after_thread_sync;" ::: "memory"); }

__device__ __forceinline__ void tma_prefetch_desc(const CUtensorMap* m) { asm volatile("prefetch.tensormap [%0];" ::"l"(m) : "memory"); }
__device__ __forceinline__ void tma_load_4d(uint32_t dst, const CUtensorMap* m, uint32_t bar, int c0, int c1, int c2, int c3) {
    asm volatile("cp.async.bulk.tensor.4d.shared::cluster.global.mbarrier::complete_tx::bytes [%0], [%1, {%3, %4, %5, %6}], [%2];" ::"r"(dst), "l"(m),
                 "r"(bar), "r"(c0), "r"(c1), "r"(c2), "r"(c3)
                 : "memory");
}
__device__ __forceinline__ void tma_load_2d(uint32_t dst, const CUtensorMap* m, uint32_t bar, int c0, int c1) {
    asm volatile("cp.async.bulk.tensor.2d.shared::cluster.global.mbarrier::complete_tx::bytes [%0], [%1, {%3, %4}], [%2];" ::"r"(dst), "l"(m), "r"(bar),
                 "r"(c0), "r"(c1)
                 : "memory");
}

__device__ __forceinline__ void tmem_alloc(uint32_t slot_smem, uint32_t cols) {
    asm volatile("tcgen05.alloc.cta_group::1.sync.aligned.shared::cta.b32 [%0], %1;" ::"r"(slot_smem), "r"(cols) : "memory");
    asm volatile("tcgen05.relinquish_alloc_permit.cta_group::1.sync.aligned;" ::: "memory");
}
__device__ __forceinline__ void tmem_dealloc(uint32_t taddr, uint32_t cols) {
    asm volatile("tcgen05.dealloc.cta_group::1.sync.aligned.b32 %0, %1;" ::"r"(taddr), "r"(cols) : "memory");
}
__device__ __forceinline__ void umma_f16(uint32_t d_tmem, uint64_t a_desc, uint64_t b_desc, uint32_t idesc, uint32_t accumulate) {
    asm volatile(
        "{\n\t.reg .pred p;\n\t"
        "setp.ne.b32 p, %4, 0;\n\t"
// ... 253 lines not shown
        }
        EPI_STAMP(4);
        fence_async_smem();
        EPI_STAMP(5);
        named_bar_sync(e.bar_id, NWARPS * 32);
        EPI_STAMP(6);
        if (leader) {
            if (!e.no_store && elect_one()) {
                tma_store_4d(sw ? e.o_hi64 : e.o_hiT, e.stg, slab_oc, c1, c2, c3);
                if (e.has_lo) tma_store_4d(sw ? e.o_lo64 : e.o_loT, e.stg + UM_BLOCK_M * 128, slab_oc, c1, c2, c3);
                bulk_commit();
            }
            __syncwarp();
        }
        EPI_STAMP(7);
    }
#undef EPI_STAMP
}
template <int NWARPS, int TERMS>
__device__ __forceinline__ void epilogue_dump_partial(const EpiArgs& e, uint32_t taddr, float* dst, int row, int half, int lane) {
    for (int c = (NWARPS == 8 ? half : 0) * 16; c < e.n_blk; c += (NWARPS == 8 ? 32 : 16)) {
        uint32_t r[16], r2[16];
        tmem_ld16(taddr + (uint32_t) c, r);
        if (TERMS == 3) {
            tmem_ld16(taddr + (uint32_t) (e.n_blk + c), r2);
        } else {
#pragma unroll
            for (int j = 0; j < 16; ++j) r2[j] = 0u;
        }
        tmem_ld_wait();
        float4* d = reinterpret_cast<float4*>(dst) + (size_t) (c >> 4) * 4 * UM_BLOCK_M + row;
#pragma unroll
        for (int j4 = 0; j4 < 4; ++j4)
            d[j4 * UM_BLOCK_M] = make_float4(__uint_as_float(r[4 * j4]) + __uint_as_float(r2[4 * j4]), __uint_as_float(r[4 * j4 + 1]) + __uint_as_float(r2[4 * j4 + 1]),
                                __uint_as_float(r[4 * j4 + 2]) + __uint_as_float(r2[4 * j4 + 2]), __uint_as_float(r[4 * j4 + 3]) + __uint_as_float(r2[4 * j4 + 3]));
    }
    tc_fence_before();
    __syncwarp();
    if (lane == 0) mbar_arrive(e.tmem_empty);
}

__device__ __forceinline__ void epilogue_drain(bool leader) {
    if (leader) {
        if (elect_one()) asm volatile("cp.async.bulk.wait_group 0;" ::: "memory");
        __syncwarp();
    }
}

struct WorkItem {
    int tile, kb0, kb1, piece, pieces, slot;
};
template <bool SK>
__host__ __device__ __forceinline__ WorkItem decode_work(const UmmaParams& p, int work, int total_tiles, int num_kb) {
    WorkItem w;
    if constexpr (!SK) {
        const int split = work / total_tiles;
        w.tile = work - split * total_tiles, w.kb0 = split * p.kb_per_split, w.kb1 = w.kb0 + p.kb_per_split < num_kb ? w.kb0 + p.kb_per_split : num_kb;
        w.piece = split, w.pieces = p.ksplit, w.slot = w.tile;
    } else if (work < p.sk_dp) {
        w.tile = work, w.kb0 = 0, w.kb1 = num_kb, w.piece = 0, w.pieces = 1, w.slot = 0;
    } else {
        const int c = (work - p.sk_dp) >> 2, j = (work - p.sk_dp) & 3;
        const long long b0 = (long long) c * p.sk_units / p.sk_ctas, b1 = (long long) (c + 1) * p.sk_units / p.sk_ctas;
        const int jt = (int) (b0 / num_kb) + j;
        const long long t0 = (long long) jt * num_kb, t1 = t0 + num_kb;
        w.tile = p.sk_dp + jt, w.slot = jt;
        w.kb0 = (int) ((b0 > t0 ? b0 : t0) - t0), w.kb1 = (int) ((b1 < t1 ? b1 : t1) - t0);
        const int c_first = (int) (((t0 + 1) * p.sk_ctas - 1) / p.sk_units), c_last = (int) ((t1 * p.sk_ctas - 1) / p.sk_units);
        w.piece = c - c_first, w.pieces = c_last - c_first + 1;
    }
    return w;
}
__host__ __device__ __forceinline__ int sk_next_work(const UmmaParams& p, int work, int cta, int grid, int num_kb, int end) {
    if (work < p.sk_dp) return work + grid < p.sk_dp ? work + grid : end;
    const int c = (work - p.sk_dp) >> 2, j = ((work - p.sk_dp) & 3) + 1;
    const long long b0 = (long long) c * p.sk_units / p.sk_ctas, b1 = (long long) (c + 1) * p.sk_units / p.sk_ctas;
    if (j < 4 && b0 / num_kb + j <= (b1 - 1) / num_kb) return work + 1;
    return cta < p.sk_dp ? cta : end;
}
__host__ __device__ __forceinline__ int sk_first_work(const UmmaParams& p, int cta, int end) {
    return cta < p.sk_ctas ? p.sk_dp + 4 * cta : (cta < p.sk_dp ? cta : end);
}

#define UM_TRACE(role, idx)                                                                          \
    do {                                                                                             \
        if (p.trace && blockIdx.x == 0 && lane == 0 && (idx) < 256) p.trace[(role) * 256 + (idx)] = clock64(); \
    } while (0)

template <int STAGES, bool SPLIT_EPI, int TERMS, bool HALO, bool SK = false>
__global__ void __launch_bounds__(UM_THREADS, 1)
conv_umma_kernel(const __grid_constant__ CUtensorMap tmA_hi, const __grid_constant__ CUtensorMap tmA_lo, const __grid_constant__ CUtensorMap tmB_hi,
                 const __grid_constant__ CUtensorMap tmB_lo, const __grid_constant__ CUtensorMap tmO_hi64, const __grid_constant__ CUtensorMap tmO_lo64,
                 const __grid_constant__ CUtensorMap tmO_hiT, const __grid_constant__ CUtensorMap tmO_loT, const __grid_constant__ CUtensorMap tmR_hi64,
                 const __grid_constant__ CUtensorMap tmR_lo64, const __grid_constant__ CUtensorMap tmR_hiT, const __grid_constant__ CUtensorMap tmR_loT,
                 const UmmaParams p) {
    extern __shared__ uint8_t smem_raw[];
    constexpr bool ONE_BLOCK = TERMS != 3 || SPLIT_EPI;
    constexpr int EPI_TERMS  = ONE_BLOCK ? 2 : 3;
    const uint32_t smem_base = (smem_u32(smem_raw) + 1023u) & ~1023u;
    const uint32_t b_ring    = smem_base + (HALO ? HL_A_STAGES * HL_A_STAGE_BYTES : 0);
    const uint32_t stg       = HALO ? b_ring + HL_B_RING_BYTES : smem_base + STAGES * UM_STAGE_BYTES;
    const uint32_t bar_base  = stg + (SPLIT_EPI ? 2 : 1) * UM_STG_BYTES;
    auto full_bar       = [&](int s) { return bar_base + 8u * s; };
    auto empty_bar      = [&](int s) { return bar_base + 8u * (STAGES + s); };
    auto tmem_full_bar  = [&](int a) { return bar_base + 8u * (2 * STAGES + a); };
    auto tmem_empty_bar = [&](int a) { return bar_base + 8u * (2 * STAGES + 2 + a); };
    const uint32_t tmem_slot = bar_base + 8u * (2 * STAGES + 4);
    const uint32_t res_bar   = bar_base + 8u * (2 * STAGES + 5);
    const uint32_t sched_base = bar_base + 8u * (2 * STAGES + 8);
    auto sched_full  = [&](int s) { return sched_base + 8u * s; };
    auto sched_empty = [&](int s) { return sched_base + 64u + 8u * s; };
    auto sched_id    = [&](int s) { return sched_base + 128u + 4u * s; };
    auto a_full_bar  = [&](int s) { return sched_base + 160u + 8u * s; };
    auto a_empty_bar = [&](int s) { return sched_base + 176u + 8u * s; };
    auto sched_take = [&](int seq, bool arrive) {
        const int slot = seq & (UM_SCHED_SLOTS - 1);
        mbar_wait(sched_full(slot), (uint32_t) (seq / UM_SCHED_SLOTS) & 1u);
        int w;
        asm volatile("ld.shared.b32 %0, [%1];" : "=r"(w) : "r"(sched_id(slot)) : "memory");
        if (arrive) mbar_arrive(sched_empty(slot));
        return w;
    };

    const int warp = threadIdx.x >> 5, lane = threadIdx.x & 31;
    pdl_trigger();
    if (warp == 0 && lane == 0) {
        mbar_init(res_bar, 1);
        mbar_init(res_bar + 16u, 1);
        tma_prefetch_desc(&tmO_hi64);
        tma_prefetch_desc(&tmO_lo64);
        tma_prefetch_desc(&tmA_hi);
        tma_prefetch_desc(&tmA_lo);
        tma_prefetch_desc(&tmB_hi);
        tma_prefetch_desc(&tmB_lo);
        for (int s = 0; s < STAGES; ++s) {
            mbar_init(full_bar(s), 1);
            mbar_init(empty_bar(s), 1);
        }
        if (HALO)
            for (int s = 0; s < HL_A_STAGES; ++s) {
                mbar_init(a_full_bar(s), 1);
                mbar_init(a_empty_bar(s), 1);
            }
        for (int s = 0; s < UM_SCHED_SLOTS; ++s) {
            mbar_init(sched_full(s), 1);
            mbar_init(sched_empty(s), 1 + UM_EPI_WARPS);
        }
        for (int a = 0; a < 2; ++a) {
            mbar_init(tmem_full_bar(a), 1);
            mbar_init(tmem_empty_bar(a), SPLIT_EPI ? UM_EPI_WARPS / 2 : UM_EPI_WARPS);
        }
        fence_barrier_init();
    }
    if (warp == 1) tmem_alloc(tmem_slot, UM_TMEM_COLS);
    tc_fence_before();
    __syncthreads();
    tc_fence_after();
    uint32_t tmem_base;
    asm volatile("ld.shared.b32 %0, [%1];" : "=r"(tmem_base) : "r"(tmem_slot));
    const int pre_total_tiles = p.tiles_x * p.tiles_y * p.tiles_n * p.tiles_oc;
    const int pre_num_kb      = p.ksize * p.ksize * p.cblocks;
    const int pre_end         = SK ? p.sk_dp + 4 * p.sk_ctas : pre_total_tiles * p.ksplit;
    const int first_work      = SK ? sk_first_work(p, (int) blockIdx.x, pre_end) : (int) blockIdx.x;
    const bool pre_b          = (p.ablate & (2 | 16)) == 0 && first_work < pre_end;
    if (warp == 0 && pre_b && elect_one()) {
        const WorkItem w0 = decode_work<SK>(p, first_work, pre_total_tiles, pre_num_kb);
        const int tile    = w0.tile;
        const int oc0  = (tile / (p.tiles_x * p.tiles_y * p.tiles_n)) * p.n_blk;
        const uint32_t b_lo_off = (uint32_t) p.n_blk * 128u;
        if (HALO) {
            for (int tap = 0; tap < 3; ++tap) {
                const uint32_t sB = b_ring + tap * p.b_stage_bytes, fb = full_bar(tap);
                mbar_expect_tx(fb, (TERMS == 3 ? 2u : 1u) * (uint32_t) p.n_blk * 128u);
                tma_load_2d(sB, &tmB_hi, fb, tap * p.ICp, oc0);
                if (TERMS == 3) tma_load_2d(sB + b_lo_off, &tmB_lo, fb, tap * p.ICp, oc0);
            }
        } else {
            const int kb0 = w0.kb0, cb = kb0 % p.cblocks, tap0 = kb0 / p.cblocks;
            const uint32_t fb = full_bar(0);
            mbar_expect_tx(fb, (TERMS == 1 ? 1u : 2u) * (uint32_t) p.rows_used * 128u + (TERMS == 3 ? 2u : 1u) * (uint32_t) p.n_blk * 128u);
            tma_load_2d(smem_base + 2 * UM_A_BYTES, &tmB_hi, fb, tap0 * p.ICp + cb * UM_BLOCK_K, oc0);
            if (TERMS == 3) tma_load_2d(smem_base + 2 * UM_A_BYTES + b_lo_off, &tmB_lo, fb, tap0 * p.ICp + cb * UM_BLOCK_K, oc0);
        }
    }
    pdl_wait();
    if (warp == 0) UM_TRACE(5, 0);
    if (p.trace && threadIdx.x == 0) {
        unsigned long long g;
        asm volatile("mov.u64 %0, %%globaltimer;" : "=l"(g));
        atomicMin(reinterpret_cast<unsigned long long*>(p.trace) + 5 * 256 + 8, g);
        if (blockIdx.x == 0) p.trace[5 * 256 + 10] = (long long) g;
    }

    if (warp == 0) UM_TRACE(5, 1);

    const int m_tiles     = p.tiles_x * p.tiles_y * p.tiles_n;
    const int total_tiles = m_tiles * p.tiles_oc;
    const int num_kb      = p.ksize * p.ksize * p.cblocks;
    const int total_work  = SK ? p.sk_dp + 4 * p.sk_ctas : total_tiles * p.ksplit;

    if (warp == 0) {
        {
            int stage = 0, hstage = 0;
            uint32_t phase = 0, hphase = 0;
            (void) hstage, (void) hphase;
            const uint32_t tx_bytes = (TERMS == 1 ? 1u : 2u) * (uint32_t) p.rows_used * 128u + (TERMS == 3 ? 2u : 1u) * (uint32_t) p.n_blk * 128u;
            const int ks = p.ksize, cbs = p.cblocks, icp = p.ICp;
            const bool skip_tma = (p.ablate & 2) != 0;
            const uint32_t b_lo_off = (uint32_t) p.n_blk * 128u;
            int tr = 0;
            const int draws_total = max(0, total_work - (int) gridDim.x) + (int) gridDim.x;
            int work = first_work;
            for (int seq = 0;; ++seq) {
                if (p.ablate & 32) producer_progress(lane, ((unsigned) seq << 16) | 0x01u);
                {
                    const int slot = seq & (UM_SCHED_SLOTS - 1);
                    mbar_wait(sched_empty(slot), ((uint32_t) (seq / UM_SCHED_SLOTS) & 1u) ^ 1u);
                    if (elect_one()) {
                        asm volatile("st.shared.b32 [%0], %1;" ::"r"(sched_id(slot)), "r"(work) : "memory");
                        mbar_arrive(sched_full(slot));
                    }
                }
                if (p.ablate & 32) producer_progress(lane, ((unsigned) seq << 16) | 0x02u);
                if (work >= total_work) break;
                int drawn = 0;
                if (!SK && elect_one()) drawn = atomicAdd(p.sched_counter, 1);
                auto take_next = [&]() {
                    if constexpr (SK) return sk_next_work(p, work, (int) blockIdx.x, (int) gridDim.x, num_kb, total_work);
                    const int c = __shfl_sync(0xffffffffu, drawn, 0);
                    if (lane == 0 && c == draws_total - 1) *p.sched_counter = 0;
                    return (int) gridDim.x + c;
                };
                const WorkItem wi = decode_work<SK>(p, work, total_tiles, num_kb);
                const int tile = wi.tile;
                const int m_idx = tile % m_tiles, oc_idx = tile / m_tiles;
                const int bx = m_idx % p.tiles_x, by = (m_idx / p.tiles_x) % p.tiles_y, bn = m_idx / (p.tiles_x * p.tiles_y);
                const int ix0 = bx * p.tw * p.stride - p.pad_x, iy0 = by * p.th * p.stride - p.pad_y, n0 = bn * p.tn;
                const int oc0 = oc_idx * p.n_blk;
                const int kb0 = wi.kb0, kb1 = wi.kb1;
                if constexpr (HALO) {
                    auto issue_halo = [&](int w, int cb) {
                        const int tile_ = w % total_tiles, m_ = tile_ % m_tiles;
                        const int bx_ = m_ % p.tiles_x, by_ = (m_ / p.tiles_x) % p.tiles_y, bn_ = m_ / (p.tiles_x * p.tiles_y);
                        mbar_wait(a_empty_bar(hstage), hphase ^ 1u);
                        if (elect_one()) {
                            const uint32_t sA = smem_base + hstage * HL_A_STAGE_BYTES, fb = a_full_bar(hstage);
                            if (skip_tma) {
                                mbar_arrive(fb);
                            } else {
                                mbar_expect_tx(fb, (TERMS == 1 ? 1u : 2u) * (uint32_t) (HL_W * HL_H * 128));
                                tma_load_4d(sA, &tmA_hi, fb, cb * UM_BLOCK_K, bx_ * HL_TW - p.pad_x, by_ * HL_TH - p.pad_y, bn_);
                                if (TERMS >= 2) tma_load_4d(sA + HL_PLANE, &tmA_lo, fb, cb * UM_BLOCK_K, bx_ * HL_TW - p.pad_x, by_ * HL_TH - p.pad_y, bn_);
                            }
                        }
                        __syncwarp();
                        if (++hstage == HL_A_STAGES) hstage = 0, hphase ^= 1u;
                    };
                    if (seq == 0) issue_halo(work, 0);
                    int nwork = total_work;
                    for (int cb = 0; cb < cbs; ++cb) {
                        int wk = cb * UM_BLOCK_K;
                        for (int tap = 0; tap < 9; ++tap, wk += icp) {
                            if (tap == 3) {
                                if (cb + 1 < cbs) {
                                    issue_halo(work, cb + 1);
                                } else {
                                    nwork = take_next();
                                    if (nwork < total_work) issue_halo(nwork, 0);
                                }
                            }
                            const bool pre_stage = seq == 0 && cb == 0 && tap < 3 && pre_b;
                            if (!pre_stage) mbar_wait(empty_bar(stage), phase ^ 1u);
                            UM_TRACE(0, tr);
                            ++tr;
                            if (pre_stage) {
                            } else if (elect_one()) {
                                const uint32_t sB = b_ring + stage * p.b_stage_bytes, fb = full_bar(stage);
                                if (skip_tma) {
                                    mbar_arrive(fb);
                                } else {
                                    mbar_expect_tx(fb, (TERMS == 3 ? 2u : 1u) * (uint32_t) p.n_blk * 128u);
                                    tma_load_2d(sB, &tmB_hi, fb, wk, oc0);
                                    if (TERMS == 3) tma_load_2d(sB + b_lo_off, &tmB_lo, fb, wk, oc0);
                                }
                            }
                            if (++stage == p.b_stages) stage = 0, phase ^= 1u;
                        }
                    }
                    work = nwork;
                    continue;
                }
                int cb = kb0 % cbs, tap0 = kb0 / cbs;
                int kx = tap0 % ks, ky = tap0 / ks;
                int wk = tap0 * icp;
                for (int kb = kb0; kb < kb1; ++kb) {
                    mbar_wait(empty_bar(stage), phase ^ 1u);
                    UM_TRACE(0, tr);
                    ++tr;
                    if (elect_one()) {
                        const uint32_t sA = smem_base + stage * UM_STAGE_BYTES, fb = full_bar(stage);
                        if (skip_tma) {
                            mbar_arrive(fb);
                        } else {
                            const bool pre = seq == 0 && kb == kb0 && pre_b;
                            if (!pre) mbar_expect_tx(fb, tx_bytes);
                            tma_load_4d(sA, &tmA_hi, fb, cb * UM_BLOCK_K, ix0 + kx, iy0 + ky, n0);
                            if (TERMS >= 2) tma_load_4d(sA + UM_A_BYTES, &tmA_lo, fb, cb * UM_BLOCK_K, ix0 + kx, iy0 + ky, n0);
                            if (!pre) {
                                tma_load_2d(sA + 2 * UM_A_BYTES, &tmB_hi, fb, wk + cb * UM_BLOCK_K, oc0);
                                if (TERMS == 3) tma_load_2d(sA + 2 * UM_A_BYTES + b_lo_off, &tmB_lo, fb, wk + cb * UM_BLOCK_K, oc0);
                            }
                        }
                    }
                    if (++stage == STAGES) stage = 0, phase ^= 1u;
                    if (++cb == cbs) {
                        cb = 0, wk += icp;
                        if (++kx == ks) kx = 0, ++ky;
                    }
                }
                work = take_next();
            }
        }
    } else if (warp == 1) {
        int stage = 0;
        uint32_t phase = 0;
        const uint32_t idesc_cat = TERMS == 3 ? make_idesc(UM_BLOCK_M, 2 * p.n_blk) : 0u;
        const uint32_t idesc     = make_idesc(UM_BLOCK_M, p.n_blk);
        const uint64_t desc0 = make_smem_desc(smem_base);
        if (elect_one()) {
            int it = 0, tr = 0, hstage = 0;
            uint32_t hphase = 0;
            (void) hstage, (void) hphase;
            bool ready = false;
            const bool no_mma = (p.ablate & 4) != 0;
            for (;; ++it) {
                const int work = sched_take(it, true);
                if (work >= total_work) break;
                const int acc = it & 1;
                const uint32_t acc_phase = (uint32_t) (it >> 1) & 1u;
                mbar_wait(tmem_empty_bar(acc), acc_phase ^ 1u);
                tc_fence_after();
                const uint32_t d_tmem = tmem_base + (uint32_t) (acc * UM_ACC_COLS);
                if constexpr (HALO) {
                    const uint64_t bdesc0 = make_smem_desc(b_ring);
                    for (int cb = 0; cb < p.cblocks; ++cb) {
                        mbar_wait(a_full_bar(hstage), hphase);
                        const uint64_t halo = make_smem_desc_sbo(smem_base + hstage * HL_A_STAGE_BYTES, HL_W * 128);
                        int tap_off = 0;
                        for (int tap = 0; tap < 9; ++tap) {
                            if (!ready) mbar_wait(full_bar(stage), phase);
                            tc_fence_after();
                            UM_TRACE(1, tr);
                            const uint64_t a_hi = halo + (uint64_t) (uint32_t) tap_off, a_lo = a_hi + (HL_PLANE >> 4);
                            const uint64_t b_cat = bdesc0 + (uint64_t) (uint32_t) (stage * (p.b_stage_bytes >> 4));
                            const uint32_t first = (cb > 0 || tap > 0) ? 1u : 0u;
                            if (!no_mma) {
                                umma_f16(d_tmem, a_hi, b_cat, TERMS == 3 ? idesc_cat : idesc, first);
                                if (TERMS == 2) umma_f16(d_tmem, a_lo, b_cat, idesc, 1u);
                            }
                            const int cur         = stage;
                            const uint32_t nphase = phase ^ (stage == p.b_stages - 1 ? 1u : 0u);
                            stage                 = stage == p.b_stages - 1 ? 0 : stage + 1;
                            phase                 = nphase;
                            ready                 = mbar_test_wait(full_bar(stage), phase);
                            if (!no_mma) {
                                if (TERMS == 3) {
#pragma unroll
                                    for (int j = 1; j < UM_BLOCK_K / 16; ++j) umma_f16(d_tmem, a_hi + 2u * j, b_cat + 2u * j, idesc_cat, 1u);
#pragma unroll
                                    for (int j = 0; j < UM_BLOCK_K / 16; ++j) umma_f16(d_tmem, a_lo + 2u * j, b_cat + 2u * j, idesc, 1u);
                                } else if (TERMS == 2) {
#pragma unroll
                                    for (int j = 1; j < UM_BLOCK_K / 16; ++j) {
                                        umma_f16(d_tmem, a_hi + 2u * j, b_cat + 2u * j, idesc, 1u);
                                        umma_f16(d_tmem, a_lo + 2u * j, b_cat + 2u * j, idesc, 1u);
                                    }
                                } else {
#pragma unroll
                                    for (int j = 1; j < UM_BLOCK_K / 16; ++j) umma_f16(d_tmem, a_hi + 2u * j, b_cat + 2u * j, idesc, 1u);
                                }
                            }
                            umma_commit(empty_bar(cur));
                            UM_TRACE(2, tr);
                            ++tr;
                            tap_off += (tap % 3 == 2) ? ((HL_W - 2) * 128 >> 4) : (128 >> 4);
                        }
                        umma_commit(a_empty_bar(hstage));
                        if (++hstage == HL_A_STAGES) hstage = 0, hphase ^= 1u;
                    }
                    umma_commit(tmem_full_bar(acc));
                    continue;
                }
                const WorkItem wi = decode_work<SK>(p, work, total_tiles, num_kb);
                const int kb0 = wi.kb0, kb1 = wi.kb1;
                for (int kb = kb0; kb < kb1; ++kb) {
                    if (!ready) mbar_wait(full_bar(stage), phase);
                    tc_fence_after();
                    UM_TRACE(1, tr);
                    const uint64_t a_hi = desc0 + (uint64_t) (uint32_t) (stage * (UM_STAGE_BYTES >> 4)), a_lo = a_hi + (UM_A_BYTES >> 4);
                    const uint64_t b_cat = a_hi + (2 * UM_A_BYTES >> 4);
                    const uint32_t first = kb > kb0 ? 1u : 0u;
                    const uint64_t b_lo = b_cat + (uint64_t) ((uint32_t) p.n_blk * 8u);
// ... 565 lines not shown
    static const int no_split = getenv("SNNB_NO_SPLITK") != nullptr;
    const int max_n = terms == 3 ? UM_MAX_N : UM_MAX_N2;
    const int t_min = (OC + max_n - 1) / max_n, t_max = (OC + 15) / 16;
    for (int t = t_min; t <= t_max; ++t) {
        const int blk = std::min(max_n, round_up((OC + t - 1) / t, 16));
        if (blk * t < OC) continue;
        const double ingest  = tile_w < 8 ? 58.0 : 72.0;
        const double a_bytes = (terms == 1 ? 1.0 : 2.0) * rows_used * 128.0, b_bytes = (terms == 3 ? 2.0 : 1.0) * blk * 128;
        const double mma     = terms == 3 ? 4.0 * (mma_clk(2 * blk) + mma_clk(blk)) : 4.0 * terms * mma_clk(blk);
        const double kb_cost = halo ? mma + 125.0 : std::max((a_bytes + b_bytes) / (ingest * 1.05), mma + 45.0);
        for (int sp = 1; sp <= ((no_split || halo) ? 1 : 4); ++sp) {
            if (sp > 1 && (num_kb < 8 * sp)) break;
            const int kbps          = (num_kb + sp - 1) / sp;
            if ((sp - 1) * kbps >= num_kb) continue;
            const long long items = (long long) m_tiles * t * sp;
            const long long rounds = (items + sm_count - 1) / sm_count;
            const double cost      = (double) rounds * (kbps * kb_cost + 7000.0 + (sp > 1 ? 9000.0 : 0.0));
            if (cost < best_cost * (sp > 1 ? 0.93 : 1.0) - 1e-9)
                best_cost = cost, best.cost = cost, best.n_blk = blk, best.tiles_oc = t, best.ksplit = sp, best.kb_per_split = kbps, best.sk = 0;
        }
        static const int env_sk = getenv("SNNB_SK") != nullptr;
        const long long tiles = (long long) m_tiles * t;
        if ((stream_k || env_sk) && !no_split && !halo && num_kb >= 6 && tiles % sm_count != 0) {
            int dp = 0, ctas = 0;
            long long units = 0;
            if (streamk_split(tiles, num_kb, sm_count, dp, units, ctas)) {
                const double u    = std::ceil((double) units / ctas);
                const double cost = (double) (dp / sm_count) * (num_kb * kb_cost + 7000.0) + u * kb_cost + 7000.0 + 4000.0;
                if (cost < best_cost * 0.95 - 1e-9)
                    best_cost = cost, best.cost = cost, best.n_blk = blk, best.tiles_oc = t, best.ksplit = 1, best.kb_per_split = num_kb, best.sk = 1, best.sk_dp = dp,
                    best.sk_ctas = ctas, best.sk_units = units;
            }
        }
        if (blk <= 16) break;
    }
    return best;
}

static int ensure_splitk_scratch(snnb_context* ctx, size_t partial_bytes, size_t n_counters) {
    if (partial_bytes > ctx->splitk_bytes) {
        void* pnew = nullptr;
        SNNB_CUDA_OK(cudaMalloc(&pnew, partial_bytes));
        ctx->scratch_blocks.push_back(pnew);
        ctx->splitk_partials = static_cast<float*>(pnew), ctx->splitk_bytes = partial_bytes;
    }
    if (n_counters > ctx->splitk_counter_n) {
        void* pnew = nullptr;
        SNNB_CUDA_OK(cudaMalloc(&pnew, n_counters * sizeof(int)));
        SNNB_CUDA_OK(cudaMemset(pnew, 0, n_counters * sizeof(int)));
        ctx->scratch_blocks.push_back(pnew);
        ctx->splitk_counters = static_cast<int*>(pnew), ctx->splitk_counter_n = n_counters;
    }
    return 0;
}

static int conv_terms(const snnb_context* ctx, const ConvArgs& a) {
    if (!a.in->lo || !a.out->lo) return 1;
    const int prec = a.precision >= 0 ? a.precision : ctx->precision;
    return prec == SNNB_PRECISION_FP16W ? 2 : (prec == SNNB_PRECISION_FP16 ? 1 : 3);
}

static bool feed_usable(const ConvArgs& a, FeedPlan& fp);
static bool rowwin_supported(const ConvArgs& a) {
    RowPlan rp;
    if (!(a.in->cp == 8 && a.w && a.w->w_row_hi && a.w->w_row_lo && a.w->row_stride == a.stride && a.w->row_pad == a.pad_x && a.out->c <= RW_MAX_N &&
          a.residual == nullptr && make_row_plan(a.k, a.stride, a.pad_x, rp) && 128 + rp.span <= RW_BOXW))
        return false;
    FeedPlan fp;
    const int wrows = feed_usable(a, fp) ? (a.k + fp.rows_per_panel - 1) / fp.rows_per_panel : a.k * ((rp.ksteps + 3) / 4);
    return wrows * 2 * round_up(a.out->c, 16) * 128 <= RW_B_MAX_BYTES;
}

bool conv2d_umma_supported(const ConvArgs& a) {
    if (!a.w || !a.w->w_hi || !a.w->w_lo) return false;
    if (!(a.pad_mode == SNNB_PAD_NONE || a.pad_mode == SNNB_PAD_CONSTANT)) return false;
    if (rowwin_supported(a)) return true;
    if (!(a.stride == 1 || a.stride == 2)) return false;
    if (a.in->c < 16) return false;
    if (a.k < 1 || a.k > 11) return false;
    if (a.pad_x > 127 || a.pad_y > 127) return false;
    return true;
}

enum { ATTR_UMMA = 1u, ATTR_ROWWIN = 2u, ATTR_DW1 = 4u, ATTR_DW2 = 8u };

typedef void (*RowWinKernel)(const CUtensorMap, const CUtensorMap, const CUtensorMap, const CUtensorMap, const CUtensorMap, const CUtensorMap, const CUtensorMap,
                             const CUtensorMap, const RowWinParams);
template <int TERMS> static RowWinKernel rowwin_kernel_fks(int fks) {
    switch (fks) {
    case 1: return conv_rowwin_kernel<TERMS, 1>;
    case 2: return conv_rowwin_kernel<TERMS, 2>;
    case 3: return conv_rowwin_kernel<TERMS, 3>;
    case 4: return conv_rowwin_kernel<TERMS, 4>;
    default: return conv_rowwin_kernel<TERMS, 0>;
    }
}
static RowWinKernel rowwin_kernel_of(int terms, int fks) { return terms == 3 ? rowwin_kernel_fks<3>(fks) : (terms == 2 ? rowwin_kernel_fks<2>(fks) : rowwin_kernel_fks<1>(fks)); }

static bool feed_usable(const ConvArgs& a, FeedPlan& fp) {
    const snnb_tensor* in = a.in;
    if (!in->feed_hi || !a.w->w_feed_hi || !a.w->w_feed_lo || a.w->feed_pad != a.pad_x) return false;
    if (!make_feed_plan(a.k, a.stride, a.pad_x, in->c, fp) || fp.px != in->feed_px || in->feed_py != a.pad_y) return false;
    const int tiles_x = (a.out->w + UM_BLOCK_M - 1) / UM_BLOCK_M;
    return in->feed_w >= 2 * (tiles_x * UM_BLOCK_M - 1) + 2 * fp.nch && in->feed_h >= 2 * (a.out->h - 1) + a.k &&
           (254 + 2 * fp.nch) * 8 <= RW_ARR_BYTES;
}

static int launch_conv2d_rowwin(snnb_context* ctx, const ConvArgs& a, EncodeTiledFn encode) {
    const snnb_tensor* in = a.in;
    snnb_tensor* out      = a.out;
    RowPlan rp;
    SNNB_REQUIRE(make_row_plan(a.k, a.stride, a.pad_x, rp), "launch_conv2d_rowwin: no row plan");
    FeedPlan fp;
    const bool feed = feed_usable(a, fp);
    SNNB_REQUIRE(feed || !in->feed_only, "launch_conv2d_rowwin: the input tensor only exists as a stem feed, which this launch cannot read");
    if (feed) {
        rp.parities = 1, rp.ksteps = fp.ksteps;
        for (int q = 0; q < fp.ksteps; ++q) rp.ks_parity[q] = 0, rp.ks_erel[q] = 2 * q;
    }
    ctx->last_kernel = feed ? "conv_rowwin_kernel<feed>" : "conv_rowwin_kernel";
    RowWinParams p;
    p.out_hi = out->hi, p.out_lo = out->lo, p.bias = a.w->bias;
    p.N = out->n, p.OH = out->h, p.OW = out->w, p.OC = out->c, p.OCp = out->cp;
    p.n_blk = round_up(out->c, 16), p.ocr = a.w->ocr;
    p.kh = a.k, p.stride = a.stride, p.pad_y = a.pad_y;
    p.tiles_x  = (out->w + UM_BLOCK_M - 1) / UM_BLOCK_M;
    p.parities = rp.parities, p.dmin[0] = rp.dmin[0], p.dmin[1] = rp.dmin[1];
    p.ksteps   = rp.ksteps, p.panels = (rp.ksteps + 3) / 4;
    for (int q = 0; q < 8; ++q) p.ks_parity[q] = q < rp.ksteps ? rp.ks_parity[q] : 0, p.ks_erel[q] = q < rp.ksteps ? rp.ks_erel[q] : 0;
    p.act = a.act, p.alpha = a.alpha;
    static const int rw_ablate = getenv("SNNB_UMMA_ABLATE") ? atoi(getenv("SNNB_UMMA_ABLATE")) : 0;
    p.ablate                   = rw_ablate;
    p.feed_hi = in->feed_hi, p.feed_lo = in->feed_lo, p.feed_h = in->feed_h, p.feed_w = in->feed_w, p.feed_py = in->feed_py;
    p.feed_seg_bytes = feed ? (uint32_t) (254 + 2 * fp.nch) * 8u : 0u;
    const int terms = conv_terms(ctx, a);
    p.lo_off      = (uint32_t) p.parities * RW_ARR_BYTES;
    p.row_bytes   = (terms == 1 ? 1u : 2u) * p.lo_off;
    static const int one_row = getenv("SNNB_FEED_ONE_ROW") != nullptr;
    p.rows_per_stage = (feed && !one_row) ? (a.k + (a.k + 3) / 4 - 1) / ((a.k + 3) / 4) : 1;
    p.stage_bytes    = (uint32_t) p.rows_per_stage * p.row_bytes;
    p.feed_prows  = feed ? (a.k + fp.rows_per_panel - 1) / fp.rows_per_panel : 0;
    p.b_bytes     = (uint32_t) round_up((terms == 3 ? 2 : 1) * (feed ? p.feed_prows : a.k * p.panels) * p.n_blk * 128, 1024);
    static const int one_stg = getenv("SNNB_ROWWIN_ONE_STAGING") != nullptr;
    const int ring_room      = RW_SMEM_BYTES - 1024 - RW_BAR_BYTES - (int) p.b_bytes;
    p.stg_bufs    = (!one_stg && (ring_room - 2 * UM_STG_BYTES) / (int) p.stage_bytes >= 2) ? 2 : 1;
    p.stages      = std::min(RW_MAX_STAGES, (ring_room - p.stg_bufs * UM_STG_BYTES) / (int) p.stage_bytes);
    SNNB_REQUIRE(p.stages >= 2, "launch_conv2d_rowwin: weight panels of %u bytes leave no room for the activation ring", p.b_bytes);

    CUtensorMap tmA[4], tmB[2];
    for (int plane = 0; plane < 2; ++plane)
        for (int par = 0; par < 2; ++par) {
            const int pp = par < rp.parities ? par : 0;
            __half* base = ((plane && in->lo) ? in->lo : in->hi) + (size_t) pp * 8;
            const int wp        = (in->w - pp + a.stride - 1) / a.stride;
            const cuuint64_t dims[4]    = {8, (cuuint64_t) (wp > 0 ? wp : 1), (cuuint64_t) in->h, (cuuint64_t) in->n};
            const cuuint64_t strides[3] = {(cuuint64_t) a.stride * 16, (cuuint64_t) in->w * 16, (cuuint64_t) in->h * in->w * 16};
            const cuuint32_t box[4]     = {8, (cuuint32_t) RW_BOXW, 1, 1};
            const cuuint32_t estr[4]    = {1, 1, 1, 1};
            CUresult r = encode(&tmA[plane * 2 + par], CU_TENSOR_MAP_DATA_TYPE_FLOAT16, 4, base, dims, strides, box, estr, CU_TENSOR_MAP_INTERLEAVE_NONE,
                                CU_TENSOR_MAP_SWIZZLE_NONE, CU_TENSOR_MAP_L2_PROMOTION_L2_128B, CU_TENSOR_MAP_FLOAT_OOB_FILL_NONE);
            SNNB_REQUIRE(r == CUDA_SUCCESS, "cuTensorMapEncodeTiled(A, rowwin) failed: %d", (int) r);
        }
    {
        const cuuint64_t dims[2]    = {64, (cuuint64_t) (feed ? (a.k + fp.rows_per_panel - 1) / fp.rows_per_panel : a.k * p.panels) * a.w->ocr};
        const cuuint64_t strides[1] = {128};
        const cuuint32_t box[2]     = {64, (cuuint32_t) p.n_blk};
        const cuuint32_t estr[2]    = {1, 1};
        void* planes[2] = {(void*) (feed ? a.w->w_feed_hi : a.w->w_row_hi), (void*) (feed ? a.w->w_feed_lo : a.w->w_row_lo)};
        for (int i = 0; i < 2; ++i) {
            CUresult r = encode(&tmB[i], CU_TENSOR_MAP_DATA_TYPE_FLOAT16, 2, planes[i], dims, strides, box, estr,
                                CU_TENSOR_MAP_INTERLEAVE_NONE, CU_TENSOR_MAP_SWIZZLE_128B, CU_TENSOR_MAP_L2_PROMOTION_L2_256B, CU_TENSOR_MAP_FLOAT_OOB_FILL_NONE);
            SNNB_REQUIRE(r == CUDA_SUCCESS, "cuTensorMapEncodeTiled(B, rowwin) failed: %d", (int) r);
        }
    }
    CUtensorMap tmO[2];
    if (encode_nhwc_box_maps(encode, out, p.n_blk, UM_BLOCK_M, 1, 1, p.n_blk == 64, tmO)) return 2;
    if (!(ctx->func_attr_mask & ATTR_ROWWIN)) {
        for (int t = 1; t <= 3; ++t)
            for (int f = 0; f <= 4; ++f) SNNB_CUDA_OK(cudaFuncSetAttribute(rowwin_kernel_of(t, f), cudaFuncAttributeMaxDynamicSharedMemorySize, RW_SMEM_BYTES));
        ctx->func_attr_mask |= ATTR_ROWWIN;
    }
    const int total_tiles = p.N * p.OH * p.tiles_x;
    const int grid        = std::min(total_tiles, ctx->sm_count);
    p.trace = nullptr;
    if (trace_enabled() && trace_begin(ctx, &p.trace)) return 1;
    auto* kern = rowwin_kernel_of(terms, feed ? fp.ksteps : 0);
    const cudaError_t le = launch_k_pdl(kern, dim3(grid), dim3(RW_THREADS), RW_SMEM_BYTES, ctx->stream, tmA[0], tmA[1], tmA[2], tmA[3], tmB[0], tmB[1], tmO[0], tmO[1], p);
    if (p.trace) {
        char hdr[256];
        snprintf(hdr, sizeof hdr, "rowwin%s k%d s%d IC%d OC%d out %dx%dx%d n_blk %d tiles %d grid %d kh %d ksteps %d terms %d", feed ? "<feed>" : "", a.k, a.stride, a.in->c,
                 a.out->c, a.out->n, a.out->h, a.out->w, p.n_blk, total_tiles, grid, p.kh, p.ksteps, terms);
        if (trace_end(ctx, p.trace, hdr)) return 1;
    }
    cudaError_t e = le != cudaSuccess ? le : cudaGetLastError();
    if (e != cudaSuccess) {
        set_error("conv_rowwin_kernel launch failed: %s", cudaGetErrorString(e));
        return 1;
    }
    ctx->launches++;
    return 0;
}

int launch_conv2d_umma(snnb_context* ctx, const ConvArgs& a) {
    EncodeTiledFn encode = get_encode(ctx);
    SNNB_REQUIRE(encode, "launch_conv2d_umma: cuTensorMapEncodeTiled is unavailable in this driver");
    if (rowwin_supported(a)) return launch_conv2d_rowwin(ctx, a, encode);
    SNNB_REQUIRE(!a.in->feed_only, "launch_conv2d_umma: the input tensor only exists as a stem feed, which this launch cannot read");
    const snnb_tensor* in = a.in;
    snnb_tensor* out      = a.out;
    UmmaParams p;
    p.out_hi = out->hi, p.out_lo = out->lo;
    p.res_hi = a.residual ? a.residual->hi : nullptr, p.res_lo = a.residual ? a.residual->lo : nullptr;
    p.has_res = a.residual != nullptr;
    p.bias    = a.w->bias;
    p.N = out->n, p.OH = out->h, p.OW = out->w, p.OC = out->c, p.OCp = out->cp;
    const TilePlan tp = plan_tiles(out->n, out->h, out->w, a.stride);
    SNNB_REQUIRE(tp.tw > 0, "launch_conv2d_umma: no tile plan");
    p.tw = tp.tw, p.th = tp.th, p.tn = tp.tn, p.rows_used = tp.tw * tp.th * tp.tn;
    p.tiles_x = tp.tiles_x, p.tiles_y = tp.tiles_y, p.tiles_n = tp.tiles_n;
    p.ksize = a.k, p.stride = a.stride, p.pad_x = a.pad_x, p.pad_y = a.pad_y;
    p.cblocks = (in->c + UM_BLOCK_K - 1) / UM_BLOCK_K;
    const int terms = conv_terms(ctx, a);
    p.has_lo        = out->lo != nullptr;
    p.b_stages = 0, p.b_stage_bytes = 0;
    OcPlan op       = plan_oc_ksplit(out->c, tp.tiles_x * tp.tiles_y * tp.tiles_n, p.rows_used, tp.tw, a.k * a.k * p.cblocks, ctx->sm_count, terms, false, a.stream_k);
    static const bool no_halo = getenv("SNNB_NO_HALO") != nullptr;
    bool halo                 = false;
    if (!no_halo && a.k == 3 && a.stride == 1 && a.pad_x <= 1 && a.pad_y <= 1) {
        const int hx = (out->w + HL_TW - 1) / HL_TW, hy = (out->h + HL_TH - 1) / HL_TH;
        const OcPlan hp = plan_oc_ksplit(out->c, hx * hy * out->n, UM_BLOCK_M, HL_TW, 9 * p.cblocks, ctx->sm_count, terms, true);
        if (hp.n_blk > 0 && hp.cost < op.cost) {
            halo = true, op = hp;
            p.b_stage_bytes = (terms == 3 ? 2 : 1) * op.n_blk * 128 <= UM_B_BYTES ? UM_B_BYTES : 2 * UM_B_BYTES;
            p.b_stages      = HL_B_RING_BYTES / p.b_stage_bytes;
            p.tw = HL_TW, p.th = HL_TH, p.tn = 1, p.rows_used = UM_BLOCK_M;
            p.tiles_x = hx, p.tiles_y = hy, p.tiles_n = out->n;
        }
    }
    SNNB_REQUIRE(op.n_blk > 0, "launch_conv2d_umma: no output-channel plan");
    p.n_blk = op.n_blk, p.tiles_oc = op.tiles_oc, p.ksplit = op.ksplit, p.kb_per_split = op.kb_per_split;
    p.sk = halo ? 0 : op.sk, p.sk_dp = op.sk_dp, p.sk_ctas = op.sk_ctas, p.sk_units = op.sk_units;
    p.partials = nullptr, p.counters = nullptr;
    if (!ctx->sched_counter) {
        cudaStreamCaptureStatus cap = cudaStreamCaptureStatusNone;
        SNNB_CUDA_OK(cudaStreamIsCapturing(ctx->stream, &cap));
        SNNB_REQUIRE(cap == cudaStreamCaptureStatusNone, "launch_conv2d_umma: the scheduler counter must be allocated by an eager pass before graph capture");
        void* pnew = nullptr;
        SNNB_CUDA_OK(cudaMalloc(&pnew, 256));
        SNNB_CUDA_OK(cudaMemset(pnew, 0, 256));
        ctx->scratch_blocks.push_back(pnew);
        ctx->sched_counter = static_cast<int*>(pnew);
    }
    p.sched_counter = ctx->sched_counter;
    if (p.ksplit > 1 || p.sk) {
        const size_t tiles = p.sk ? (size_t) p.tiles_x * p.tiles_y * p.tiles_n * p.tiles_oc - p.sk_dp : (size_t) p.tiles_x * p.tiles_y * p.tiles_n * p.tiles_oc;
        cudaStreamCaptureStatus cap = cudaStreamCaptureStatusNone;
        SNNB_CUDA_OK(cudaStreamIsCapturing(ctx->stream, &cap));
        const size_t need = tiles * (p.sk ? 4 : p.ksplit) * UM_BLOCK_M * p.n_blk * sizeof(float);
        SNNB_REQUIRE(cap == cudaStreamCaptureStatusNone || (need <= ctx->splitk_bytes && tiles <= ctx->splitk_counter_n),
                     "launch_conv2d_umma: split-K scratch must be allocated by an eager pass before graph capture");
        if (ensure_splitk_scratch(ctx, need, tiles)) return 1;
        p.partials = ctx->splitk_partials, p.counters = ctx->splitk_counters;
    }
    p.ICp     = round_up(in->c, 8);
    p.act = a.act, p.alpha = a.alpha;
    static const int ablate = getenv("SNNB_UMMA_ABLATE") ? atoi(getenv("SNNB_UMMA_ABLATE")) : 0;
    p.ablate                = ablate;
    SNNB_REQUIRE(a.w->kp == a.k * a.k * p.ICp, "launch_conv2d_umma: packed weights do not match (kp %d vs %d)", a.w->kp, a.k * a.k * p.ICp);

    CUtensorMap tmA[2], tmB[2];
    {
        const cuuint64_t dims[4]    = {(cuuint64_t) in->c, (cuuint64_t) in->w, (cuuint64_t) in->h, (cuuint64_t) in->n};
        const cuuint64_t strides[3] = {(cuuint64_t) in->cp * 2, (cuuint64_t) in->w * in->cp * 2, (cuuint64_t) in->h * in->w * in->cp * 2};
        const cuuint32_t box[4]     = {(cuuint32_t) UM_BLOCK_K, (cuuint32_t) (halo ? HL_W : p.tw * a.stride), (cuuint32_t) (halo ? HL_H : p.th * a.stride), (cuuint32_t) p.tn};
        const cuuint32_t estr[4]    = {1, (cuuint32_t) a.stride, (cuuint32_t) a.stride, 1};
        __half* planes[2]    = {in->hi, in->lo ? in->lo : in->hi};
        for (int i = 0; i < 2; ++i) {
            CUresult r = encode(&tmA[i], CU_TENSOR_MAP_DATA_TYPE_FLOAT16, 4, planes[i], dims, strides, box, estr, CU_TENSOR_MAP_INTERLEAVE_NONE,
                                CU_TENSOR_MAP_SWIZZLE_128B, CU_TENSOR_MAP_L2_PROMOTION_L2_128B, CU_TENSOR_MAP_FLOAT_OOB_FILL_NONE);
            SNNB_REQUIRE(r == CUDA_SUCCESS, "cuTensorMapEncodeTiled(A) failed: %d (dims %d %d %d %d box %u %u %u %u)", (int) r, in->c, in->w, in->h, in->n, box[0],
                         box[1], box[2], box[3]);
        }
    }
    {
        const cuuint64_t dims[2]    = {(cuuint64_t) a.w->kp, (cuuint64_t) a.w->ocr};
        const cuuint64_t strides[1] = {(cuuint64_t) a.w->kp * 2};
        const cuuint32_t box[2]     = {(cuuint32_t) UM_BLOCK_K, (cuuint32_t) p.n_blk};
        const cuuint32_t estr[2]    = {1, 1};
        void* planes[2]             = {(void*) a.w->w_hi, (void*) a.w->w_lo};
        for (int i = 0; i < 2; ++i) {
            CUresult r = encode(&tmB[i], CU_TENSOR_MAP_DATA_TYPE_FLOAT16, 2, planes[i], dims, strides, box, estr,
                                CU_TENSOR_MAP_INTERLEAVE_NONE, CU_TENSOR_MAP_SWIZZLE_128B, CU_TENSOR_MAP_L2_PROMOTION_L2_256B, CU_TENSOR_MAP_FLOAT_OOB_FILL_NONE);
            SNNB_REQUIRE(r == CUDA_SUCCESS, "cuTensorMapEncodeTiled(B) failed: %d (kp %d ocr %d n_blk %d)", (int) r, a.w->kp, a.w->ocr, p.n_blk);
        }
    }
    CUtensorMap tmO64[2], tmOT[2], tmR64[2], tmRT[2];
    {
        const int wT = p.n_blk % 64;
        const snnb_tensor* res = a.residual ? a.residual : out;
        if (encode_nhwc_box_maps(encode, out, p.n_blk >= 64 ? 64 : wT, p.tw, p.th, p.tn, p.n_blk >= 64, tmO64)) return 2;
        if (encode_nhwc_box_maps(encode, out, wT ? wT : 64, p.tw, p.th, p.tn, wT == 0, tmOT)) return 2;
        if (encode_nhwc_box_maps(encode, res, p.n_blk >= 64 ? 64 : wT, p.tw, p.th, p.tn, p.n_blk >= 64, tmR64)) return 2;
        if (encode_nhwc_box_maps(encode, res, wT ? wT : 64, p.tw, p.th, p.tn, wT == 0, tmRT)) return 2;
    }
    if (!(ctx->func_attr_mask & ATTR_UMMA)) {
        SNNB_CUDA_OK(cudaFuncSetAttribute(conv_umma_kernel<UM_STAGES, false, 1, false>, cudaFuncAttributeMaxDynamicSharedMemorySize, UM_SMEM_BYTES));
        SNNB_CUDA_OK(cudaFuncSetAttribute(conv_umma_kernel<UM_STAGES, false, 2, false>, cudaFuncAttributeMaxDynamicSharedMemorySize, UM_SMEM_BYTES));
        SNNB_CUDA_OK(cudaFuncSetAttribute(conv_umma_kernel<UM_STAGES, false, 3, false>, cudaFuncAttributeMaxDynamicSharedMemorySize, UM_SMEM_BYTES));
        SNNB_CUDA_OK(cudaFuncSetAttribute(conv_umma_kernel<UM_STAGES - 1, true, 1, false>, cudaFuncAttributeMaxDynamicSharedMemorySize, UM_SMEM_BYTES_SPLIT));
        SNNB_CUDA_OK(cudaFuncSetAttribute(conv_umma_kernel<UM_STAGES - 1, true, 2, false>, cudaFuncAttributeMaxDynamicSharedMemorySize, UM_SMEM_BYTES_SPLIT));
        SNNB_CUDA_OK(cudaFuncSetAttribute(conv_umma_kernel<UM_STAGES - 1, true, 3, false>, cudaFuncAttributeMaxDynamicSharedMemorySize, UM_SMEM_BYTES_SPLIT));
        SNNB_CUDA_OK(cudaFuncSetAttribute(conv_umma_kernel<HL_B_STAGES, false, 1, true>, cudaFuncAttributeMaxDynamicSharedMemorySize, HL_SMEM_BYTES));
        SNNB_CUDA_OK(cudaFuncSetAttribute(conv_umma_kernel<HL_B_STAGES, false, 2, true>, cudaFuncAttributeMaxDynamicSharedMemorySize, HL_SMEM_BYTES));
        SNNB_CUDA_OK(cudaFuncSetAttribute(conv_umma_kernel<HL_B_STAGES, false, 3, true>, cudaFuncAttributeMaxDynamicSharedMemorySize, HL_SMEM_BYTES));
        SNNB_CUDA_OK(cudaFuncSetAttribute(conv_umma_kernel<UM_STAGES, false, 1, false, true>, cudaFuncAttributeMaxDynamicSharedMemorySize, UM_SMEM_BYTES));
        SNNB_CUDA_OK(cudaFuncSetAttribute(conv_umma_kernel<UM_STAGES, false, 2, false, true>, cudaFuncAttributeMaxDynamicSharedMemorySize, UM_SMEM_BYTES));
        SNNB_CUDA_OK(cudaFuncSetAttribute(conv_umma_kernel<UM_STAGES, false, 3, false, true>, cudaFuncAttributeMaxDynamicSharedMemorySize, UM_SMEM_BYTES));
        ctx->func_attr_mask |= ATTR_UMMA;
    }
    const int total_tiles = p.tiles_x * p.tiles_y * p.tiles_n * p.tiles_oc;
    const int grid        = p.sk ? (p.sk_dp > 0 ? ctx->sm_count : p.sk_ctas) : std::min(total_tiles * p.ksplit, ctx->sm_count);
    static const bool no_split_epi = getenv("SNNB_NO_SPLIT_EPI") != nullptr;
    const bool split_epi           = !halo && !no_split_epi && !p.sk && p.ksplit == 1 && p.ksize * p.ksize * p.cblocks <= 3 && total_tiles >= 2 * grid;
    ctx->last_kernel = halo ? "conv_umma_kernel<halo>"
                            : (split_epi ? "conv_umma_kernel<short-K>" : (p.sk ? "conv_umma_kernel<stream-K>" : (p.ksplit > 1 ? "conv_umma_kernel<split-K>" : "conv_umma_kernel")));
    p.trace = nullptr;
    if (trace_enabled() && trace_begin(ctx, &p.trace)) return 1;
    auto* k_split = terms == 3 ? conv_umma_kernel<UM_STAGES - 1, true, 3, false> : (terms == 2 ? conv_umma_kernel<UM_STAGES - 1, true, 2, false> : conv_umma_kernel<UM_STAGES - 1, true, 1, false>);
    auto* k_plain = p.sk ? (terms == 3 ? conv_umma_kernel<UM_STAGES, false, 3, false, true>
                                       : (terms == 2 ? conv_umma_kernel<UM_STAGES, false, 2, false, true> : conv_umma_kernel<UM_STAGES, false, 1, false, true>) )
                         : (terms == 3 ? conv_umma_kernel<UM_STAGES, false, 3, false> : (terms == 2 ? conv_umma_kernel<UM_STAGES, false, 2, false> : conv_umma_kernel<UM_STAGES, false, 1, false>) );
    auto* k_halo  = terms == 3 ? conv_umma_kernel<HL_B_STAGES, false, 3, true> : (terms == 2 ? conv_umma_kernel<HL_B_STAGES, false, 2, true> : conv_umma_kernel<HL_B_STAGES, false, 1, true>);
    const cudaError_t le =
        halo      ? launch_k_pdl(k_halo, dim3(grid), dim3(UM_THREADS), HL_SMEM_BYTES, ctx->stream, tmA[0], tmA[1], tmB[0], tmB[1], tmO64[0], tmO64[1], tmOT[0], tmOT[1], tmR64[0],
                                 tmR64[1], tmRT[0], tmRT[1], p)
        : split_epi ? launch_k_pdl(k_split, dim3(grid), dim3(UM_THREADS), UM_SMEM_BYTES_SPLIT, ctx->stream, tmA[0], tmA[1], tmB[0], tmB[1], tmO64[0], tmO64[1], tmOT[0], tmOT[1],
                                 tmR64[0], tmR64[1], tmRT[0], tmRT[1], p)
                  : launch_k_pdl(k_plain, dim3(grid), dim3(UM_THREADS), UM_SMEM_BYTES, ctx->stream, tmA[0], tmA[1], tmB[0], tmB[1], tmO64[0], tmO64[1], tmOT[0], tmOT[1], tmR64[0],
                                 tmR64[1], tmRT[0], tmRT[1], p);
    if (p.trace) {
        char hdr[256];
        snprintf(hdr, sizeof hdr, "conv k%d s%d IC%d OC%d out %dx%dx%d n_blk %d tiles %d grid %d num_kb %d ksplit %d terms %d halo %d", a.k, a.stride, in->c, out->c, out->n,
                 out->h, out->w, p.n_blk, total_tiles, grid, p.ksize * p.ksize * p.cblocks, split_epi ? -1 : (p.sk ? -2 : p.ksplit), terms, (int) halo);
        if (trace_end(ctx, p.trace, hdr)) return 1;
    }
    cudaError_t e = le != cudaSuccess ? le : cudaGetLastError();
    if (e != cudaSuccess) {
        set_error("conv_umma_kernel launch failed: %s", cudaGetErrorString(e));
        return 1;
    }
    ctx->launches++;
    return 0;
}


constexpr int DW_THREADS = 256;
constexpr int DW_STAGES  = 2;
template <int S> struct DwTile {
    static constexpr int TW = S == 1 ? 16 : 8, TH = S == 1 ? 8 : 4;
    static constexpr int TXT = S == 1 ? 4 : 1;
    static constexpr int IW = (TW - 1) * S + 3, IH = (TH - 1) * S + 3;
    static constexpr int PLANE_BYTES = IW * IH * 128;
    static constexpr int STAGE_BYTES = 2 * PLANE_BYTES;
    static constexpr int SMEM_BYTES  = DW_STAGES * STAGE_BYTES + 128  + 64 ;
};
struct DwTmaParams {
    __half* out_hi;
    __half* out_lo;
    const float* w;
    const float* bias;
    int N, OH, OW, C, Cp;
    int pad_x, pad_y;
    int tiles_x, tiles_y, chunks;
    int act;
    float alpha;
};

template <int S>
__global__ void __launch_bounds__(DW_THREADS, 2) depthwise_tma_kernel(const __grid_constant__ CUtensorMap tmI_hi, const __grid_constant__ CUtensorMap tmI_lo, const DwTmaParams p) {
    using T = DwTile<S>;
    extern __shared__ uint8_t smem_raw[];
    const uint32_t smem_base = (smem_u32(smem_raw) + 127u) & ~127u;
    const uint32_t bar_base  = smem_base + DW_STAGES * T::STAGE_BYTES;
    const int tid = threadIdx.x, warp = tid >> 5;
    pdl_trigger();
    if (tid == 0) {
        tma_prefetch_desc(&tmI_hi);
        tma_prefetch_desc(&tmI_lo);
        for (int s = 0; s < DW_STAGES; ++s) mbar_init(bar_base + 8u * s, 1);
        fence_barrier_init();
    }
    __syncthreads();
    pdl_wait();

    const int sp_tiles = p.N * p.tiles_y * p.tiles_x;
    const int total    = sp_tiles * p.chunks;
    auto issue = [&](int tile, int stage) {
        const int chunk = tile / sp_tiles, sp = tile - chunk * sp_tiles;
        const int tx = sp % p.tiles_x, ty = (sp / p.tiles_x) % p.tiles_y, n = sp / (p.tiles_x * p.tiles_y);
        const uint32_t dst = smem_base + stage * T::STAGE_BYTES, bar = bar_base + 8u * stage;
        mbar_expect_tx(bar, T::STAGE_BYTES);
        tma_load_4d(dst, &tmI_hi, bar, chunk * 64, tx * T::TW * S - p.pad_x, ty * T::TH * S - p.pad_y, n);
        tma_load_4d(dst + T::PLANE_BYTES, &tmI_lo, bar, chunk * 64, tx * T::TW * S - p.pad_x, ty * T::TH * S - p.pad_y, n);
    };
    if (tid == 0)
        for (int j = 0; j < DW_STAGES; ++j) {
            const int tile = blockIdx.x + j * gridDim.x;
            if (tile < total) issue(tile, j);
        }

    const int cg  = tid & 7, pt = tid >> 3;
    const int tyl = S == 1 ? (pt >> 2) : (pt >> 3), txl = S == 1 ? (pt & 3) * 4 : (pt & 7);
    const float slope   = (p.act == SNNB_ACT_RELU || p.act == SNNB_ACT_RELU6) ? 0.0f : (p.act == SNNB_ACT_LEAKY_RELU ? p.alpha : 1.0f);
    const float hi_clip = p.act == SNNB_ACT_RELU6 ? 6.0f : __int_as_float(0x7f800000);
    const bool fast_act = p.act == SNNB_ACT_NONE || p.act == SNNB_ACT_RELU || p.act == SNNB_ACT_RELU6 || p.act == SNNB_ACT_LEAKY_RELU;

    float wreg[9][8], breg[8];
    int cur_chunk = -1;
    int it = 0;
    for (int tile = blockIdx.x; tile < total; tile += gridDim.x, ++it) {
        const int stage = it % DW_STAGES;
        const int chunk = tile / sp_tiles, sp = tile - chunk * sp_tiles;
        const int tx = sp % p.tiles_x, ty = (sp / p.tiles_x) % p.tiles_y, n = sp / (p.tiles_x * p.tiles_y);
        const int c = chunk * 64 + cg * 8;
        if (chunk != cur_chunk) {
            cur_chunk = chunk;
// ... 84 lines not shown
            }
        }
    }
    (void) warp;
}

bool depthwise_tma_supported(const ConvArgs& a) {
    if (!a.in->lo || !a.out->lo) return false;
    const int tw = a.stride == 1 ? 16 : 8, th = a.stride == 1 ? 8 : 4;
    const int tx = (a.out->w + tw - 1) / tw, ty = (a.out->h + th - 1) / th;
    if ((double) a.out->w * a.out->h < 0.5 * (double) tx * tw * ty * th) return false;
    return a.k == 3 && (a.stride == 1 || a.stride == 2) && a.residual == nullptr && a.in->c == a.out->c && a.w->w_f32 != nullptr &&
           a.pad_mode <= SNNB_PAD_CONSTANT;
}

template <int S> static int launch_depthwise_tma_s(snnb_context* ctx, const ConvArgs& a, EncodeTiledFn encode) {
    ctx->last_kernel = "depthwise_tma_kernel";
    using T = DwTile<S>;
    const snnb_tensor* in = a.in;
    snnb_tensor* out      = a.out;
    DwTmaParams p;
    p.out_hi = out->hi, p.out_lo = out->lo;
    p.w = a.w->w_f32, p.bias = a.w->bias;
    p.N = out->n, p.OH = out->h, p.OW = out->w, p.C = out->c, p.Cp = out->cp;
    p.pad_x = a.pad_x, p.pad_y = a.pad_y;
    p.tiles_x = (out->w + T::TW - 1) / T::TW, p.tiles_y = (out->h + T::TH - 1) / T::TH, p.chunks = (out->cp + 63) / 64;
    p.act = a.act, p.alpha = a.alpha;
    CUtensorMap tmI[2];
    {
        const cuuint64_t dims[4]    = {(cuuint64_t) in->c, (cuuint64_t) in->w, (cuuint64_t) in->h, (cuuint64_t) in->n};
        const cuuint64_t strides[3] = {(cuuint64_t) in->cp * 2, (cuuint64_t) in->w * in->cp * 2, (cuuint64_t) in->h * in->w * in->cp * 2};
        const cuuint32_t box[4]     = {64, (cuuint32_t) T::IW, (cuuint32_t) T::IH, 1};
        const cuuint32_t estr[4]    = {1, 1, 1, 1};
        __half* planes[2]    = {in->hi, in->lo};
        for (int i = 0; i < 2; ++i) {
            CUresult r = encode(&tmI[i], CU_TENSOR_MAP_DATA_TYPE_FLOAT16, 4, planes[i], dims, strides, box, estr, CU_TENSOR_MAP_INTERLEAVE_NONE, CU_TENSOR_MAP_SWIZZLE_NONE,
                                CU_TENSOR_MAP_L2_PROMOTION_L2_128B, CU_TENSOR_MAP_FLOAT_OOB_FILL_NONE);
            SNNB_REQUIRE(r == CUDA_SUCCESS, "cuTensorMapEncodeTiled(depthwise input) failed: %d", (int) r);
        }
    }
    const uint32_t attr_bit = S == 1 ? ATTR_DW1 : ATTR_DW2;
    if (!(ctx->func_attr_mask & attr_bit)) {
        SNNB_CUDA_OK(cudaFuncSetAttribute(depthwise_tma_kernel<S>, cudaFuncAttributeMaxDynamicSharedMemorySize, T::SMEM_BYTES));
        ctx->func_attr_mask |= attr_bit;
    }
    const long long total = (long long) p.N * p.tiles_y * p.tiles_x * p.chunks;
    const int grid        = (int) std::min<long long>(total, 2 * ctx->sm_count);
    const cudaError_t le  = launch_k_pdl(depthwise_tma_kernel<S>, dim3(grid), dim3(DW_THREADS), T::SMEM_BYTES, ctx->stream, tmI[0], tmI[1], p);
    cudaError_t e = le != cudaSuccess ? le : cudaGetLastError();
    if (e != cudaSuccess) {
        set_error("depthwise_tma_kernel launch failed: %s", cudaGetErrorString(e));
        return 1;
    }
    ctx->launches++;
    return 0;
}

int launch_depthwise_tma(snnb_context* ctx, const ConvArgs& a) {
    EncodeTiledFn encode = get_encode(ctx);
    SNNB_REQUIRE(encode, "launch_depthwise_tma: cuTensorMapEncodeTiled is unavailable in this driver");
    return a.stride == 1 ? launch_depthwise_tma_s<1>(ctx, a, encode) : launch_depthwise_tma_s<2>(ctx, a, encode);
}

int streamk_schedule(int tiles, int num_kb, int sms, int* rows, int capacity) {
    UmmaParams p {};
    int dp = 0, ctas = 0;
    long long units = 0;
    if (tiles <= 0 || num_kb <= 0 || sms <= 0 || tiles % sms == 0 || !streamk_split(tiles, num_kb, sms, dp, units, ctas)) return -1;
    p.sk = 1, p.sk_dp = dp, p.sk_ctas = ctas, p.sk_units = units, p.ksplit = 1, p.kb_per_split = num_kb;
    const int grid = dp > 0 ? sms : ctas, end = dp + 4 * ctas;
    int n = 0;
    for (int cta = 0; cta < grid; ++cta)
        for (int work = sk_first_work(p, cta, end); work < end; work = sk_next_work(p, work, cta, grid, num_kb, end)) {
            const WorkItem w = decode_work<true>(p, work, tiles, num_kb);
            if (n < capacity) {
                int* r = rows + 6 * (size_t) n;
                r[0] = cta, r[1] = w.tile, r[2] = w.kb0, r[3] = w.kb1, r[4] = w.piece, r[5] = w.pieces;
            }
            ++n;
        }
    return n;
}

}
```

### shadernn_b200/csrc/pack.cpp

```cpp
#include <cmath>
#include <cstring>

#include "snnb_internal.h"

namespace snnb {

static inline size_t align256(size_t v) { return (v + 255) & ~(size_t) 255; }

size_t PackedHost::device_bytes() const {
    size_t b = 0;
    b += align256(w_f32.size() * sizeof(float));
    b += align256(w_hi.size() * sizeof(__half));
    b += align256(w_lo.size() * sizeof(__half));
    b += align256(w_row_hi.size() * sizeof(__half));
    b += align256(w_row_lo.size() * sizeof(__half));
    b += align256(w_feed_hi.size() * sizeof(__half));
    b += align256(w_feed_lo.size() * sizeof(__half));
    b += align256(bias.size() * sizeof(float));
    b += align256(gamma.size() * sizeof(float));
    b += align256(beta.size() * sizeof(float));
    b += align256(mean.size() * sizeof(float));
    b += align256(var.size() * sizeof(float));
    return b;
}

static void bn_fold(int OC, const float* bias, const float* g, const float* b, const float* m, const float* v, std::vector<float>& scale,
                    std::vector<float>& shift) {
    scale.assign(OC, 1.0f);
    shift.assign(OC, 0.0f);
    const bool has_bn = (m != nullptr) || (v != nullptr) || (g != nullptr) || (b != nullptr);
    for (int o = 0; o < OC; ++o) {
        const float bi = bias ? bias[o] : 0.0f;
        if (has_bn) {
            const float gamma = g ? g[o] : 1.0f, beta = b ? b[o] : 0.0f, mean = m ? m[o] : 0.0f, var = v ? v[o] : 1.0f;
            float s  = std::sqrt(var + 0.001f);
            s        = std::max(s, 0.0001f);
            scale[o] = gamma / s;
            shift[o] = (bi - mean) * scale[o] + beta;
        } else {
            shift[o] = bi;
        }
    }
}

void pack_conv2d_host(int IC, int OC, int k, const float* w_oihw, const float* bias, const float* g, const float* b, const float* m, const float* v,
                      PackedHost& out) {
    out.kind = 1, out.in_ch = IC, out.out_ch = OC, out.kernel = k;
    std::vector<float> scale, shift;
    bn_fold(OC, bias, g, b, m, v, scale, shift);
    const int K = k * k * IC;
    const int ICp = round_up(IC, 8);
    out.ocw     = round_up(OC, 64);
    out.kp      = k * k * ICp;
    out.ocr     = round_up(OC, 16);
    out.w_f32.assign((size_t) K * out.ocw, 0.0f);
    out.w_hi.assign((size_t) out.ocr * out.kp, __float2half_rn(0.0f));
    out.w_lo.assign((size_t) out.ocr * out.kp, __float2half_rn(0.0f));
    out.bias.assign(out.ocw + 320, 0.0f);
    for (int o = 0; o < OC; ++o) {
        out.bias[o] = shift[o];
        for (int i = 0; i < IC; ++i)
            for (int ky = 0; ky < k; ++ky)
                for (int kx = 0; kx < k; ++kx) {
                    const float wv  = w_oihw[(((size_t) o * IC + i) * k + ky) * k + kx] * scale[o];
                    const int kidx  = (ky * k + kx) * IC + i;
                    out.w_f32[(size_t) kidx * out.ocw + o] = wv;
                    const int kcol                         = (ky * k + kx) * ICp + i;
                    const __half h                  = __float2half_rn(wv);
                    out.w_hi[(size_t) o * out.kp + kcol]   = h;
                    out.w_lo[(size_t) o * out.kp + kcol]   = __float2half_rn(wv - __half2float(h));
                }
    }
}

void pack_rowwin_host(PackedHost& p, int stride, int pad_x) {
    RowPlan rp;
    if (p.kind != 1 || p.in_ch > 8 || p.out_ch > 64 || !make_row_plan(p.kernel, stride, pad_x, rp)) return;
    const int k = p.kernel, IC = p.in_ch, OC = p.out_ch;
    p.row_stride = stride, p.row_pad = pad_x;
    const int panels = (rp.ksteps + 3) / 4;
    p.w_row_hi.assign((size_t) k * panels * p.ocr * 64, __float2half_rn(0.0f));
    p.w_row_lo.assign((size_t) k * panels * p.ocr * 64, __float2half_rn(0.0f));
    for (int ky = 0; ky < k; ++ky)
        for (int o = 0; o < OC; ++o)
            for (int q = 0; q < rp.ksteps; ++q)
                for (int h = 0; h < 2; ++h) {
                    const int j = rp.ks_tap[q][h];
                    if (j < 0) continue;
                    for (int c = 0; c < IC; ++c) {
                        const float wv        = p.w_f32[(size_t) ((ky * k + j) * IC + c) * p.ocw + o];
                        const size_t idx      = (((size_t) ky * panels + q / 4) * p.ocr + o) * 64 + (q % 4) * 16 + h * 8 + c;
                        const __half hh = __float2half_rn(wv);
                        p.w_row_hi[idx]       = hh;
                        p.w_row_lo[idx]       = __float2half_rn(wv - __half2float(hh));
                    }
                }
}

void pack_feed_host(PackedHost& p, int stride, int pad_x) {
    FeedPlan fp;
    if (p.kind != 1 || p.out_ch > 64 || p.w_row_hi.empty() || !make_feed_plan(p.kernel, stride, pad_x, p.in_ch, fp)) return;
    const int k = p.kernel, IC = p.in_ch, OC = p.out_ch;
    p.feed_pad = pad_x;
    const int rpp = fp.rows_per_panel, prows = (k + rpp - 1) / rpp, sub = 64 / rpp;
    p.w_feed_hi.assign((size_t) prows * p.ocr * 64, __float2half_rn(0.0f));
    p.w_feed_lo.assign((size_t) prows * p.ocr * 64, __float2half_rn(0.0f));
    for (int ky = 0; ky < k; ++ky)
        for (int o = 0; o < OC; ++o)
            for (int off = 0; off < 2 * fp.nch; ++off) {
                const int t = off - fp.d;
                if (t < 0 || t >= k) continue;
                for (int c = 0; c < IC; ++c) {
                    const float wv   = p.w_f32[(size_t) ((ky * k + t) * IC + c) * p.ocw + o];
                    const size_t idx = ((size_t) (ky / rpp) * p.ocr + o) * 64 + (ky % rpp) * sub + off * 4 + c;
                    const __half hh  = __float2half_rn(wv);
                    p.w_feed_hi[idx] = hh;
                    p.w_feed_lo[idx] = __float2half_rn(wv - __half2float(hh));
                }
            }
}

void pack_depthwise_host(int C, int k, const float* w_chw, const float* bias, const float* g, const float* b, const float* m, const float* v,
                         PackedHost& out) {
    out.kind = 2, out.in_ch = C, out.out_ch = C, out.kernel = k;
    std::vector<float> scale, shift;
    bn_fold(C, bias, g, b, m, v, scale, shift);
    const int Cp = round_up(C, 8);
    out.ocw      = Cp;
    out.w_f32.assign((size_t) k * k * Cp, 0.0f);
    out.bias.assign(round_up(C, 64), 0.0f);
    for (int c = 0; c < C; ++c) {
        out.bias[c] = shift[c];
        for (int t = 0; t < k * k; ++t) out.w_f32[(size_t) t * Cp + c] = w_chw[(size_t) c * k * k + t] * scale[c];
    }
}

void pack_channels_host(int C, const float* g, const float* b, const float* m, const float* v, PackedHost& out) {
    out.kind = 4, out.in_ch = C, out.out_ch = C;
    const int Cp = round_up(C, 8);
    out.gamma.assign(Cp, 0.0f), out.beta.assign(Cp, 0.0f), out.mean.assign(Cp, 0.0f), out.var.assign(Cp, 0.0f);
    for (int c = 0; c < C; ++c) {
        out.gamma[c] = g ? g[c] : 1.0f;
        out.beta[c]  = b ? b[c] : 0.0f;
        out.mean[c]  = m ? m[c] : 0.0f;
        float s      = std::sqrt((v ? v[c] : 1.0f) + 0.001f);
        s            = std::max(s, 0.0001f);
        out.var[c]   = out.gamma[c] / s;
    }
}

template <class T> static int put(snnb_context* ctx, const std::vector<T>& src, char*& cur, T** dst) {
    *dst = nullptr;
    if (src.empty()) return 0;
    *dst = reinterpret_cast<T*>(cur);
    SNNB_CUDA_OK(cudaMemcpyAsync(cur, src.data(), src.size() * sizeof(T), cudaMemcpyHostToDevice, ctx->stream));
    cur += align256(src.size() * sizeof(T));
    return 0;
// ... 27 lines not shown
```

### shadernn_b200/csrc/snnb_internal.h

```cpp
#pragma once

#include <cuda_runtime.h>
#include <cuda_fp16.h>
#include <cstdint>
#include <cstdio>
#include <string>
#include <utility>
#include <vector>

#include "snnb.h"

namespace snnb {

void set_error(const char* fmt, ...);
const char* get_error();

#define SNNB_CUDA_OK(expr)                                                                              \
    do {                                                                                                \
        cudaError_t _e = (expr);                                                                        \
        if (_e != cudaSuccess) {                                                                        \
            ::snnb::set_error("%s:%d: %s -> %s", __FILE__, __LINE__, #expr, cudaGetErrorString(_e));    \
            return 1;                                                                                   \
        }                                                                                               \
    } while (0)
// ... 39 lines not shown

}

struct snnb_tensor {
    snnb_context* ctx = nullptr;
    __half* hi = nullptr;
    __half* lo = nullptr;
    int n = 0, h = 0, w = 0, c = 0, cp = 0;
    size_t plane_elems = 0;
    bool owns = true;
    __half* feed_hi = nullptr;
    __half* feed_lo = nullptr;
    int feed_h = 0, feed_w = 0, feed_py = 0, feed_px = 0;
    bool feed_only = false;
    size_t pixels() const { return (size_t) n * h * w; }
};

struct snnb_weights {
    snnb_context* ctx = nullptr;
    int kind = 0;
    int in_ch = 0, out_ch = 0, kernel = 1;
    float* w_f32 = nullptr;
    int ocw = 0;
    __half* w_hi = nullptr;
    __half* w_lo = nullptr;
    int kp = 0, ocr = 0;
    __half* w_row_hi = nullptr;
    __half* w_row_lo = nullptr;
    int row_stride = 0, row_pad = 0;
    __half* w_feed_hi = nullptr;
    __half* w_feed_lo = nullptr;
    int feed_pad = -1;
    float* bias = nullptr;
    float *gamma = nullptr, *beta = nullptr, *mean = nullptr, *var = nullptr;
    void* owned = nullptr;
    size_t bytes = 0;
};

struct snnb_context {
    int device          = 0;
    cudaStream_t stream = nullptr;
    int sm_count        = 148;
    uint64_t launches   = 0;
    float* stage_dev    = nullptr;
    size_t stage_dev_bytes = 0;
    float* stage_host   = nullptr;
    size_t stage_host_bytes = 0;
    void* tmap_encode_fn = nullptr;
    float* splitk_partials = nullptr;
    size_t splitk_bytes    = 0;
    int* splitk_counters   = nullptr;
    size_t splitk_counter_n = 0;
    int* sched_counter      = nullptr;
    uint32_t func_attr_mask = 0;
    const char* last_kernel = nullptr;
    int precision = SNNB_PRECISION_FP32X3;
    std::vector<void*> scratch_blocks;
};

struct snnb_graph {
    snnb_context* ctx     = nullptr;
    cudaGraph_t graph     = nullptr;
    cudaGraphExec_t exec  = nullptr;
};

struct snnb_timer {
    snnb_context* ctx = nullptr;
    cudaEvent_t e0 = nullptr, e1 = nullptr;
};

namespace snnb {

int ensure_stage(snnb_context* ctx, size_t bytes);

struct ConvArgs {
    const snnb_tensor* in;
    const snnb_tensor* residual;
    snnb_tensor* out;
    const snnb_weights* w;
    int k, stride, pad_x, pad_y, pad_mode, act;
    float alpha;
    int precision = -1;
    bool stream_k = false;
};
int launch_conv2d_simt(snnb_context* ctx, const ConvArgs& a);
int launch_conv2d_umma(snnb_context* ctx, const ConvArgs& a);
bool conv2d_umma_supported(const ConvArgs& a);
int streamk_schedule(int tiles, int num_kb, int sms, int* rows, int capacity);
int launch_depthwise(snnb_context* ctx, const ConvArgs& a);
bool depthwise_tma_supported(const ConvArgs& a);
int launch_depthwise_tma(snnb_context* ctx, const ConvArgs& a);
int launch_pool(snnb_context* ctx, const snnb_tensor* in, snnb_tensor* out, int k, int stride, bool avg);
bool gap_dense_supported(const snnb_tensor* in, const snnb_tensor* out, const snnb_weights* w);
int launch_gap_dense(snnb_context* ctx, const snnb_tensor* in, snnb_tensor* out, const snnb_weights* w, int act, float alpha, bool softmax);
int launch_add(snnb_context* ctx, const snnb_tensor* a, const snnb_tensor* b, snnb_tensor* out, int act, float alpha);
int launch_batchnorm(snnb_context* ctx, const snnb_tensor* in, snnb_tensor* out, const snnb_weights* w, int act, float alpha);
int launch_activation(snnb_context* ctx, const snnb_tensor* in, snnb_tensor* out, int act, float alpha);
int launch_softmax(snnb_context* ctx, const snnb_tensor* in, snnb_tensor* out);
int launch_argmax(snnb_context* ctx, const snnb_tensor* in, int* dev_idx);
int launch_yolo_candidates(snnb_context* ctx, const snnb_tensor* h0, const snnb_tensor* h1, float thresh, int maxc, int* counts, float* cand);
int launch_flatten(snnb_context* ctx, const snnb_tensor* in, snnb_tensor* out);
int launch_concat(snnb_context* ctx, const snnb_tensor* a, const snnb_tensor* b, snnb_tensor* out);
int launch_upsample(snnb_context* ctx, const snnb_tensor* in, snnb_tensor* out, float scale, bool bilinear);
int launch_pad(snnb_context* ctx, const snnb_tensor* in, snnb_tensor* out, int pad_x, int pad_y, int mode);
constexpr int INSTNORM_MAX_CHUNKS = 64;
static inline size_t instnorm_scratch_floats(int n, int cp) { return (size_t) n * cp * 2 + (size_t) n * (cp >> 3) * INSTNORM_MAX_CHUNKS * 16; }
int launch_instancenorm(snnb_context* ctx, const snnb_tensor* in, snnb_tensor* out, const snnb_weights* w, int act, float alpha, float* scratch = nullptr);
int launch_subpixel(snnb_context* ctx, const snnb_tensor* in, snnb_tensor* out, int r);
int launch_split_f32(snnb_context* ctx, const float* dev_nhwc, snnb_tensor* t);
int launch_split_u8(snnb_context* ctx, const uint8_t* dev_nhwc_u8, snnb_tensor* t, const float mean[4], const float norm[4]);
int launch_merge_f32(snnb_context* ctx, const snnb_tensor* t, float* dev_nhwc);
int launch_result_small(snnb_context* ctx, const snnb_tensor* t, float* values, int* idx);
int launch_resize_u8(snnb_context* ctx, const uint8_t* dev_nhwc_u8, int src_h, int src_w, snnb_tensor* t, const float mean[4], const float norm[4], bool linear);
int launch_merge_u8(snnb_context* ctx, const snnb_tensor* t, uint8_t* dev_nhwc_u8, float scale, float offset);

struct RowPlan {
    int parities = 0;
    int dmin[2]  = {0, 0};
    int ntaps[2] = {0, 0};
    int ksteps   = 0;
    int ks_parity[8], ks_erel[8], ks_tap[8][2];
    int span = 0;
};
static inline bool make_row_plan(int k, int stride, int pad_x, RowPlan& rp) {
    if (k < 1 || k > 9 || !(stride == 1 || stride == 2)) return false;
    rp = RowPlan();
    rp.parities = stride;
    for (int par = 0; par < stride; ++par) {
        int js[9], t = 0;
        for (int j = 0; j < k; ++j)
            if ((((j - pad_x) % stride) + stride) % stride == par) js[t++] = j;
        rp.ntaps[par] = t;
        if (!t) continue;
        const int a  = js[0] - pad_x;
        rp.dmin[par] = a >= 0 ? a / stride : -((-a + stride - 1) / stride);
        for (int q = 0; q < (t + 1) / 2; ++q) {
            if (rp.ksteps >= 8) return false;
            rp.ks_parity[rp.ksteps] = par;
            rp.ks_erel[rp.ksteps]   = 2 * q;
            rp.ks_tap[rp.ksteps][0] = js[2 * q];
            rp.ks_tap[rp.ksteps][1] = (2 * q + 1 < t) ? js[2 * q + 1] : -1;
            rp.ksteps++;
        }
        rp.span = rp.span > 2 * ((t + 1) / 2) ? rp.span : 2 * ((t + 1) / 2);
    }
    return rp.ksteps > 0;
}

struct FeedPlan {
    int px = 0, d = 0, nch = 0, ksteps = 0;
    int rows_per_panel = 1;
};
static inline bool make_feed_plan(int k, int stride, int pad_x, int ic, FeedPlan& fp) {
    if (stride != 2 || ic > 4 || k < 2 || k > 9 || pad_x < 0 || pad_x > 8) return false;
    fp.px     = (pad_x + 1) & ~1;
    fp.d      = fp.px - pad_x;
    fp.nch    = ((fp.d + k + 1) / 2 + 1) & ~1;
    fp.ksteps = fp.nch / 2;
    fp.rows_per_panel = fp.ksteps == 1 ? 4 : (fp.ksteps == 2 ? 2 : 1);
    return fp.ksteps <= 4;
}

struct PackedHost {
    std::vector<float> w_f32;
    std::vector<__half> w_hi, w_lo;
    std::vector<__half> w_row_hi, w_row_lo;
    int row_stride = 0, row_pad = 0;
    std::vector<__half> w_feed_hi, w_feed_lo;
    int feed_pad = -1;
    std::vector<float> bias;
    std::vector<float> gamma, beta, mean, var;
    int kind = 0, in_ch = 0, out_ch = 0, kernel = 1, ocw = 0, kp = 0, ocr = 0;
    size_t device_bytes() const;
};
void pack_conv2d_host(int IC, int OC, int k, const float* w_oihw, const float* bias, const float* g, const float* b, const float* m, const float* v,
                      PackedHost& out);
void pack_rowwin_host(PackedHost& p, int stride, int pad_x);
void pack_feed_host(PackedHost& p, int stride, int pad_x);
void pack_depthwise_host(int C, int k, const float* w_chw, const float* bias, const float* g, const float* b, const float* m, const float* v,
                         PackedHost& out);
void pack_channels_host(int C, const float* g, const float* b, const float* m, const float* v, PackedHost& out);
int place_weights(snnb_context* ctx, const PackedHost& p, char* base, snnb_weights* w);

int tensor_alloc(snnb_context* ctx, int n, int h, int w, int c, snnb_tensor** out, bool lo_plane = true);
int tensor_alloc_feed(snnb_tensor* t, int feed_h, int feed_w, int py, int px);

}
```

Measured before the change: 58470.

## Fold projection-shortcut 1x1 conv into the main conv's K loop

Detects ResNet-style Add(conv, 1x1 downsample conv) patterns and appends the shortcut's 1x1 weights as extra K blocks of the main convolution, so the tensor-core kernel accumulates both GEMMs into the same accumulator and applies the Add's activation in the epilogue. This removes a separate shortcut conv launch, its output tensor write and readback, and the separate Add. In exchange the main conv carries a longer K loop with a second TMA descriptor for the shortcut input, and folded layers can no longer be inspected or run on the SIMT path.

```diff
diff --git a/include/snnb.h b/include/snnb.h
--- a/include/snnb.h
+++ b/include/snnb.h
@@ -154,6 +154,7 @@
 int snnb_tensor_planes(const snnb_tensor* t, void** hi, void** lo, int* cp);
 int snnb_debug_streamk_schedule(int tiles, int num_kb, int sms, int* rows, int capacity);
 int snnb_debug_feed_plan(int k, int stride, int pad_x, int ic, int out[5]);
+int snnb_debug_kblock_schedule(int ksize, int cblocks, int icp, int sc_cblocks, int tiles, int ksplit, int sms, int* rows, int capacity);
 
 #ifdef __cplusplus
 }
diff --git a/shadernn_b200/_lib.py b/shadernn_b200/_lib.py
--- a/shadernn_b200/_lib.py
+++ b/shadernn_b200/_lib.py
@@ -135,6 +135,7 @@
     "snnb_tensor_planes": (C.c_int, [vp, C.POINTER(vp), C.POINTER(vp), c_int_p]),
     "snnb_debug_streamk_schedule": (C.c_int, [C.c_int, C.c_int, C.c_int, c_int_p, C.c_int]),
     "snnb_debug_feed_plan": (C.c_int, [C.c_int, C.c_int, C.c_int, C.c_int, c_int_p]),
+    "snnb_debug_kblock_schedule": (C.c_int, [C.c_int] * 7 + [c_int_p, C.c_int]),
 }
 
 _lib = None
diff --git a/shadernn_b200/csrc/capi.cpp b/shadernn_b200/csrc/capi.cpp
--- a/shadernn_b200/csrc/capi.cpp
+++ b/shadernn_b200/csrc/capi.cpp
@@ -143,6 +143,10 @@
 int snnb_debug_streamk_schedule(int tiles, int num_kb, int sms, int* rows, int capacity) {
     SNNB_REQUIRE(rows || capacity == 0, "snnb_debug_streamk_schedule: null buffer");
     return streamk_schedule(tiles, num_kb, sms, rows, capacity);
+}
+int snnb_debug_kblock_schedule(int ksize, int cblocks, int icp, int sc_cblocks, int tiles, int ksplit, int sms, int* rows, int capacity) {
+    SNNB_REQUIRE(rows || capacity == 0, "snnb_debug_kblock_schedule: null buffer");
+    return kblock_schedule(ksize, cblocks, icp, sc_cblocks, tiles, ksplit, sms, rows, capacity);
 }
 int snnb_tensor_planes(const snnb_tensor* t, void** hi, void** lo, int* cp) {
     SNNB_REQUIRE(t && hi && lo && cp, "snnb_tensor_planes: null argument");
diff --git a/shadernn_b200/csrc/engine/core.cpp b/shadernn_b200/csrc/engine/core.cpp
--- a/shadernn_b200/csrc/engine/core.cpp
+++ b/shadernn_b200/csrc/engine/core.cpp
@@ -83,6 +83,42 @@
     }
 
     std::unordered_map<GenericModelLayer*, GenericModelLayer*> alias;
+    const bool shortcutFold = options.fuse && options.convAlgo != SNNB_ALGO_SIMT && getenv("SNNB_NO_SHORTCUT_FOLD") == nullptr;
+    auto foldable = [&](GenericModelLayer* c2, GenericModelLayer* ds) {
+        if (c2 == ds || c2->typeName != "Conv2D" || ds->typeName != "Conv2D" || c2->fusedAway || ds->fusedAway) return false;
+        auto* cc = static_cast<Conv2DLayer*>(c2);
+        auto* dc = static_cast<Conv2DLayer*>(ds);
+        if (c2->nextLayers.size() != 1 || ds->nextLayers.size() != 1 || c2->prevLayers.size() != 1 || ds->prevLayers.size() != 1) return false;
+        if (cc->_desc.activation.id != SNNB_ACT_NONE || dc->_desc.activation.id != SNNB_ACT_NONE || cc->residual || cc->fusedAct >= 0 || cc->shortcut ||
+            dc->shortcut || dc->foldedInto)
+            return false;
+        const int dsMode = padModeId(dc->_desc.padding.mode);
+        if (cc->_desc.stride != 1 || dc->_desc.kernelSize != 1 || !(dsMode == SNNB_PAD_NONE || dsMode == SNNB_PAD_CONSTANT)) return false;
+        GenericModelLayer* x = ds->prevLayers[0];
+        if (order[x] >= order[c2]) return false;
+        const Dims &dc2 = graph.outputDims[order[c2]], &dds = graph.outputDims[order[ds]];
+        if (dc2.width != dds.width || dc2.height != dds.height || dc2.depth != dds.depth || graph.outputDims[order[x]].depth != ds->numInputPlanes) return false;
+        auto stand_in = [&](GenericModelLayer* X) {
+            snnb_tensor t;
+            const Dims& d = graph.outputDims[order[X]];
+            t.n = N, t.h = (int) d.height, t.w = (int) d.width, t.c = (int) d.depth, t.cp = round_up(t.c, 8);
+            t.hi = reinterpret_cast<__half*>(1), t.lo = twoPlanes ? t.hi : nullptr;
+            return t;
+        };
+        const snnb_tensor in = stand_in(c2->prevLayers[0]), sc = stand_in(x), out = stand_in(c2);
+        snnb_weights probe;
+        probe.w_hi = probe.w_lo = probe.w_row_hi = probe.w_row_lo = reinterpret_cast<__half*>(1);
+        uint32_t offs[4];
+        cc->_desc.padding.offsets((int) cc->_desc.kernelSize, true, offs);
+        ConvArgs a;
+        a.in = &in, a.residual = nullptr, a.out = const_cast<snnb_tensor*>(&out), a.w = &probe;
+        a.k = (int) cc->_desc.kernelSize, a.stride = 1;
+        a.pad_x = a.k == 1 ? 0 : (int) offs[0], a.pad_y = a.k == 1 ? 0 : (int) offs[2], a.pad_mode = padModeId(cc->_desc.padding.mode);
+        probe.row_stride = 1, probe.row_pad = a.pad_x;
+        a.act = SNNB_ACT_NONE, a.alpha = 0.0f, a.precision = options.precision;
+        a.shortcut = &sc, a.sc_stride = (int) dc->_desc.stride;
+        return conv2d_umma_fold_supported(ctx, a);
+    };
     if (options.fuse) {
         for (auto* L : graph.sorted) {
             if (L->typeName == "Pad" && L->nextLayers.size() == 1 && L->prevLayers.size() == 1) {
@@ -100,7 +136,24 @@
                     alias[L]       = L->prevLayers[0];
                 }
             }
-            if (L->typeName == "Add" && L->prevLayers.size() == 2) {
+            if (shortcutFold && L->typeName == "Add" && L->prevLayers.size() == 2) {
+                auto* add = static_cast<AddLayer*>(L);
+                for (int o = 0; o < 2; ++o) {
+                    GenericModelLayer* c2 = L->prevLayers[o];
+                    GenericModelLayer* ds = L->prevLayers[1 - o];
+                    if (!foldable(c2, ds)) continue;
+                    auto* cc       = static_cast<Conv2DLayer*>(c2);
+                    cc->fusedAct   = add->activation.id;
+                    cc->fusedAlpha = add->activation.alpha;
+                    cc->shortcut   = static_cast<Conv2DLayer*>(ds);
+                    cc->shortcut->foldedInto = cc;
+                    ds->fusedAway  = true;
+                    L->fusedAway   = true;
+                    alias[c2]      = L;
+                    break;
+                }
+            }
+            if (L->typeName == "Add" && L->prevLayers.size() == 2 && !L->fusedAway) {
                 auto* add = static_cast<AddLayer*>(L);
                 GenericModelLayer* a = L->prevLayers[0];
                 GenericModelLayer* b = L->prevLayers[1];
@@ -162,6 +215,7 @@
         if (L->typeName == "YOLO") continue;
         GenericModelLayer* owner = resolve(L);
         if (owner != L && !(L->typeName == "Conv2D")) continue;
+        if (L->typeName == "Conv2D" && static_cast<Conv2DLayer*>(L)->foldedInto) continue;
         if (outOf.count(owner)) continue;
         const Dims& d = graph.outputDims[order[owner]];
         snnb_tensor* t = nullptr;
@@ -181,7 +235,7 @@
         L->output                = outOf.count(owner) ? outOf[owner] : nullptr;
         if (L->fusedAway) continue;
         size_t nin = L->prevLayers.size();
-        if (L->typeName == "Conv2D" && static_cast<Conv2DLayer*>(L)->fusedAct >= 0) {
+        if (L->typeName == "Conv2D" && static_cast<Conv2DLayer*>(L)->fusedAct >= 0 && !static_cast<Conv2DLayer*>(L)->shortcut) {
             nin -= 1;
             L->residual = outOf.at(resolve(L->prevLayers.back()));
         }
@@ -189,6 +243,7 @@
         if (L->typeName == "Conv2D") {
             auto* cl  = static_cast<Conv2DLayer*>(L);
             cl->algo = options.convAlgo;
+            if (cl->shortcut) cl->shortcutIn = outOf.at(resolve(cl->shortcut->prevLayers[0]));
             int ph = 0, pw = 0;
             snnb_weights probe_w;
             probe_w.w_hi = probe_w.w_lo = reinterpret_cast<__half*>(1);
@@ -213,7 +268,7 @@
                 cl->_desc.padding.offsets((int) cl->_desc.kernelSize, true, offs);
                 const int k = (int) cl->_desc.kernelSize, padX = (int) offs[0], padY = (int) offs[2];
                 FeedPlan fp;
-                if (!noFeed && !prepad && src->isInputLayer && !in->feed_hi && options.convAlgo != SNNB_ALGO_SIMT && !L->residual && L->output->c <= 64 &&
+                if (!noFeed && !prepad && src->isInputLayer && !in->feed_hi && options.convAlgo != SNNB_ALGO_SIMT && !L->residual && !cl->shortcut && L->output->c <= 64 &&
                     (mode == SNNB_PAD_NONE || mode == SNNB_PAD_CONSTANT) && make_feed_plan(k, (int) cl->_desc.stride, padX, in->c, fp)) {
                     const int tilesX = (L->output->w + 127) / 128;
                     const int needW  = 2 * (tilesX * 128 - 1) + 2 * fp.nch;
@@ -291,7 +346,8 @@
         int readers = 0;
         for (auto* L : graph.sorted) {
             if (L->fusedAway || L->isInputLayer) continue;
-            const bool reads = std::find(L->inputs.begin(), L->inputs.end(), t) != L->inputs.end() || L->residual == t;
+            const bool reads = std::find(L->inputs.begin(), L->inputs.end(), t) != L->inputs.end() || L->residual == t ||
+                               (L->typeName == "Conv2D" && static_cast<Conv2DLayer*>(L)->shortcutIn == t);
             if (!reads) continue;
             ++readers;
             only = only && L->typeName == "Conv2D" && static_cast<Conv2DLayer*>(L)->feedInput && L->inputs.size() >= 1 && L->inputs[0] == t && L->residual != t &&
@@ -618,6 +674,9 @@
 int MixedInferenceCore::layerOutput(int layerId, float* host, size_t capacityFloats) {
     SNNB_REQUIRE(layerId >= 0 && layerId < (int) layers.size() && host, "layerOutput: bad argument");
     GenericModelLayer* L = layers[layerId].get();
+    SNNB_REQUIRE(!(L->typeName == "Conv2D" && static_cast<Conv2DLayer*>(L)->foldedInto),
+                 "layerOutput: layer %d (%s) was fused into the K loop of the convolution it is added to; load the model with fuse=0 to observe it", layerId,
+                 L->name.c_str());
     SNNB_REQUIRE(L->output, "layerOutput: layer %d (%s) has no device tensor", layerId, L->name.c_str());
     SNNB_REQUIRE(!(L->typeName == "Conv2D" && static_cast<Conv2DLayer*>(L)->fusedAct >= 0),
                  "layerOutput: layer %d (%s) was fused into its Add; load the model with fuse=0 to observe it", layerId, L->name.c_str());
diff --git a/shadernn_b200/csrc/engine/engine.h b/shadernn_b200/csrc/engine/engine.h
--- a/shadernn_b200/csrc/engine/engine.h
+++ b/shadernn_b200/csrc/engine/engine.h
@@ -136,6 +136,9 @@
     int algo = SNNB_ALGO_AUTO;
     snnb_tensor* prepadded = nullptr;
     bool feedInput = false;
+    Conv2DLayer* shortcut    = nullptr;
+    Conv2DLayer* foldedInto  = nullptr;
+    snnb_tensor* shortcutIn  = nullptr;
     bool wantsPrepad(const snnb_tensor* in, const snnb_tensor* out, int convAlgo, int& ph, int& pw) const;
     Transform getOutputScaleDimAdjustment() const override;
     void getOutputDims(uint32_t& w, uint32_t& h, uint32_t& d) const override;
diff --git a/shadernn_b200/csrc/engine/layers.cpp b/shadernn_b200/csrc/engine/layers.cpp
--- a/shadernn_b200/csrc/engine/layers.cpp
+++ b/shadernn_b200/csrc/engine/layers.cpp
@@ -59,6 +59,7 @@
     return (it == bn.end() || it->second.empty()) ? nullptr : it->second.data();
 }
 void Conv2DLayer::packWeights(PackedHost& p) {
+    if (foldedInto) return;
     const auto& bn = _desc.batchNormalization;
     const bool use = _desc.useBatchNormalization;
     pack_conv2d_host((int) numInputPlanes, (int) numOutputPlanes, (int) _desc.kernelSize, _desc.weights.data(), _desc.biases.empty() ? nullptr : _desc.biases.data(),
@@ -75,6 +76,14 @@
             pack_rowwin_host(p, (int) _desc.stride, 0);
         }
     }
+    if (shortcut) {
+        const auto& sd = shortcut->_desc;
+        const bool sbn = sd.useBatchNormalization;
+        pack_shortcut_host((int) shortcut->numInputPlanes, sd.weights.data(), sd.biases.empty() ? nullptr : sd.biases.data(),
+                           sbn ? bnv(sd.batchNormalization, "gamma") : nullptr, sbn ? bnv(sd.batchNormalization, "beta") : nullptr,
+                           sbn ? bnv(sd.batchNormalization, "movingMean") : nullptr, sbn ? bnv(sd.batchNormalization, "movingVariance") : nullptr, p);
+        std::vector<float>().swap(shortcut->_desc.weights);
+    }
     std::vector<float>().swap(_desc.weights);
 }
 bool Conv2DLayer::wantsPrepad(const snnb_tensor* in, const snnb_tensor* out, int convAlgo, int& ph, int& pw) const {
@@ -106,8 +115,13 @@
     a.act      = fusedAct >= 0 ? fusedAct : _desc.activation.id;
     a.alpha    = fusedAct >= 0 ? fusedAlpha : _desc.activation.alpha;
     a.precision = opt.precision;
+    a.shortcut = shortcutIn, a.sc_stride = shortcut ? (int) shortcut->_desc.stride : 1;
     const int want = algo != SNNB_ALGO_AUTO ? algo : opt.convAlgo;
     if (want != SNNB_ALGO_SIMT && conv2d_umma_supported(a)) return launch_conv2d_umma(ctx, a);
+    if (shortcut) {
+        set_error("%s: a folded projection shortcut runs on the tensor-core kernel only; load the model with fuse=0 for another algorithm", name.c_str());
+        return 2;
+    }
     if (want == SNNB_ALGO_TCGEN05) {
         set_error("%s: tcgen05 path requested but unsupported for this shape", name.c_str());
         return 2;
diff --git a/shadernn_b200/csrc/kernels_umma.cu b/shadernn_b200/csrc/kernels_umma.cu
--- a/shadernn_b200/csrc/kernels_umma.cu
+++ b/shadernn_b200/csrc/kernels_umma.cu
@@ -57,6 +57,7 @@
     int sk, sk_dp, sk_ctas;
     long long sk_units;
     int b_stages, b_stage_bytes;
+    int sc_cblocks, sc_stride;
 };
 
 __device__ __forceinline__ uint32_t smem_u32(const void* p) { return (uint32_t) __cvta_generic_to_shared(p); }
@@ -476,6 +477,34 @@
     return cta < p.sk_ctas ? p.sk_dp + 4 * cta : (cta < p.sk_dp ? cta : end);
 }
 
+struct KBlock {
+    int sc, tap, cb, wcol;
+};
+__host__ __device__ __forceinline__ KBlock decode_kblock(const UmmaParams& p, int kb) {
+    const int kb_main = p.ksize * p.ksize * p.cblocks;
+    KBlock k;
+    k.sc  = kb >= kb_main;
+    k.tap = k.sc ? 0 : kb / p.cblocks;
+    k.cb  = k.sc ? kb - kb_main : kb - k.tap * p.cblocks;
+    k.wcol = (k.sc ? p.ksize * p.ksize : k.tap) * p.ICp + k.cb * UM_BLOCK_K;
+    return k;
+}
+template <class F> __host__ __device__ __forceinline__ void for_each_kblock(const UmmaParams& p, int kb0, int kb1, F&& f) {
+    const int ks = p.ksize, cbs = p.cblocks, icp = p.ICp, kb_main = ks * ks * cbs;
+    const KBlock k0 = decode_kblock(p, kb0);
+    int cb = k0.cb, kx = k0.tap % ks, ky = k0.tap / ks;
+    int wk = k0.wcol - k0.cb * UM_BLOCK_K;
+    int kb = kb0;
+    for (const int e = kb1 < kb_main ? kb1 : kb_main; kb < e; ++kb) {
+        f(kb, false, cb, kx, ky, wk + cb * UM_BLOCK_K);
+        if (++cb == cbs) {
+            cb = 0, wk += icp;
+            if (++kx == ks) kx = 0, ++ky;
+        }
+    }
+    for (; kb < kb1; ++kb, ++cb) f(kb, true, cb, 0, 0, wk + cb * UM_BLOCK_K);
+}
+
 #define UM_TRACE(role, idx)                                                                          \
     do {                                                                                             \
         if (p.trace && blockIdx.x == 0 && lane == 0 && (idx) < 256) p.trace[(role) * 256 + (idx)] = clock64(); \
@@ -487,7 +516,7 @@
                  const __grid_constant__ CUtensorMap tmB_lo, const __grid_constant__ CUtensorMap tmO_hi64, const __grid_constant__ CUtensorMap tmO_lo64,
                  const __grid_constant__ CUtensorMap tmO_hiT, const __grid_constant__ CUtensorMap tmO_loT, const __grid_constant__ CUtensorMap tmR_hi64,
                  const __grid_constant__ CUtensorMap tmR_lo64, const __grid_constant__ CUtensorMap tmR_hiT, const __grid_constant__ CUtensorMap tmR_loT,
-                 const UmmaParams p) {
+                 const __grid_constant__ CUtensorMap tmS_hi, const __grid_constant__ CUtensorMap tmS_lo, const UmmaParams p) {
     extern __shared__ uint8_t smem_raw[];
     constexpr bool ONE_BLOCK = TERMS != 3 || SPLIT_EPI;
     constexpr int EPI_TERMS  = ONE_BLOCK ? 2 : 3;
@@ -553,7 +582,7 @@
     uint32_t tmem_base;
     asm volatile("ld.shared.b32 %0, [%1];" : "=r"(tmem_base) : "r"(tmem_slot));
     const int pre_total_tiles = p.tiles_x * p.tiles_y * p.tiles_n * p.tiles_oc;
-    const int pre_num_kb      = p.ksize * p.ksize * p.cblocks;
+    const int pre_num_kb      = p.ksize * p.ksize * p.cblocks + p.sc_cblocks;
     const int pre_end         = SK ? p.sk_dp + 4 * p.sk_ctas : pre_total_tiles * p.ksplit;
     const int first_work      = SK ? sk_first_work(p, (int) blockIdx.x, pre_end) : (int) blockIdx.x;
     const bool pre_b          = (p.ablate & (2 | 16)) == 0 && first_work < pre_end;
@@ -570,11 +599,11 @@
                 if (TERMS == 3) tma_load_2d(sB + b_lo_off, &tmB_lo, fb, tap * p.ICp, oc0);
             }
         } else {
-            const int kb0 = w0.kb0, cb = kb0 % p.cblocks, tap0 = kb0 / p.cblocks;
+            const int wcol    = decode_kblock(p, w0.kb0).wcol;
             const uint32_t fb = full_bar(0);
             mbar_expect_tx(fb, (TERMS == 1 ? 1u : 2u) * (uint32_t) p.rows_used * 128u + (TERMS == 3 ? 2u : 1u) * (uint32_t) p.n_blk * 128u);
-            tma_load_2d(smem_base + 2 * UM_A_BYTES, &tmB_hi, fb, tap0 * p.ICp + cb * UM_BLOCK_K, oc0);
-            if (TERMS == 3) tma_load_2d(smem_base + 2 * UM_A_BYTES + b_lo_off, &tmB_lo, fb, tap0 * p.ICp + cb * UM_BLOCK_K, oc0);
+            tma_load_2d(smem_base + 2 * UM_A_BYTES, &tmB_hi, fb, wcol, oc0);
+            if (TERMS == 3) tma_load_2d(smem_base + 2 * UM_A_BYTES + b_lo_off, &tmB_lo, fb, wcol, oc0);
         }
     }
     pdl_wait();
@@ -590,7 +619,7 @@
 
     const int m_tiles     = p.tiles_x * p.tiles_y * p.tiles_n;
     const int total_tiles = m_tiles * p.tiles_oc;
-    const int num_kb      = p.ksize * p.ksize * p.cblocks;
+    const int num_kb      = p.ksize * p.ksize * p.cblocks + p.sc_cblocks;
     const int total_work  = SK ? p.sk_dp + 4 * p.sk_ctas : total_tiles * p.ksplit;
 
     if (warp == 0) {
@@ -599,7 +628,7 @@
             uint32_t phase = 0, hphase = 0;
             (void) hstage, (void) hphase;
             const uint32_t tx_bytes = (TERMS == 1 ? 1u : 2u) * (uint32_t) p.rows_used * 128u + (TERMS == 3 ? 2u : 1u) * (uint32_t) p.n_blk * 128u;
-            const int ks = p.ksize, cbs = p.cblocks, icp = p.ICp;
+            const int cbs = p.cblocks, icp = p.ICp;
             const bool skip_tma = (p.ablate & 2) != 0;
             const uint32_t b_lo_off = (uint32_t) p.n_blk * 128u;
             int tr = 0;
@@ -684,10 +713,8 @@
                     work = nwork;
                     continue;
                 }
-                int cb = kb0 % cbs, tap0 = kb0 / cbs;
-                int kx = tap0 % ks, ky = tap0 / ks;
-                int wk = tap0 * icp;
-                for (int kb = kb0; kb < kb1; ++kb) {
+                const int sx0 = bx * p.tw * p.sc_stride, sy0 = by * p.th * p.sc_stride;
+                for_each_kblock(p, kb0, kb1, [&](int kb, bool sc, int cb, int kx, int ky, int wcol) {
                     mbar_wait(empty_bar(stage), phase ^ 1u);
                     UM_TRACE(0, tr);
                     ++tr;
@@ -698,20 +725,19 @@
                         } else {
                             const bool pre = seq == 0 && kb == kb0 && pre_b;
                             if (!pre) mbar_expect_tx(fb, tx_bytes);
-                            tma_load_4d(sA, &tmA_hi, fb, cb * UM_BLOCK_K, ix0 + kx, iy0 + ky, n0);
-                            if (TERMS >= 2) tma_load_4d(sA + UM_A_BYTES, &tmA_lo, fb, cb * UM_BLOCK_K, ix0 + kx, iy0 + ky, n0);
+                            const CUtensorMap* a_hi = sc ? &tmS_hi : &tmA_hi;
+                            const CUtensorMap* a_lo = sc ? &tmS_lo : &tmA_lo;
+                            const int ax = sc ? sx0 : ix0 + kx, ay = sc ? sy0 : iy0 + ky;
+                            tma_load_4d(sA, a_hi, fb, cb * UM_BLOCK_K, ax, ay, n0);
+                            if (TERMS >= 2) tma_load_4d(sA + UM_A_BYTES, a_lo, fb, cb * UM_BLOCK_K, ax, ay, n0);
                             if (!pre) {
-                                tma_load_2d(sA + 2 * UM_A_BYTES, &tmB_hi, fb, wk + cb * UM_BLOCK_K, oc0);
-                                if (TERMS == 3) tma_load_2d(sA + 2 * UM_A_BYTES + b_lo_off, &tmB_lo, fb, wk + cb * UM_BLOCK_K, oc0);
+                                tma_load_2d(sA + 2 * UM_A_BYTES, &tmB_hi, fb, wcol, oc0);
+                                if (TERMS == 3) tma_load_2d(sA + 2 * UM_A_BYTES + b_lo_off, &tmB_lo, fb, wcol, oc0);
                             }
                         }
                     }
                     if (++stage == STAGES) stage = 0, phase ^= 1u;
-                    if (++cb == cbs) {
-                        cb = 0, wk += icp;
-                        if (++kx == ks) kx = 0, ++ky;
-                    }
-                }
+                });
                 work = take_next();
             }
         }
@@ -1443,6 +1469,26 @@
     return true;
 }
 
+static bool halo_plan(const snnb_context* ctx, const ConvArgs& a, int cblocks, int terms, double plain_cost, OcPlan& hp) {
+    static const bool no_halo = getenv("SNNB_NO_HALO") != nullptr;
+    if (no_halo || a.k != 3 || a.stride != 1 || a.pad_x > 1 || a.pad_y > 1) return false;
+    const int hx = (a.out->w + HL_TW - 1) / HL_TW, hy = (a.out->h + HL_TH - 1) / HL_TH;
+    hp = plan_oc_ksplit(a.out->c, hx * hy * a.out->n, UM_BLOCK_M, HL_TW, 9 * cblocks, ctx->sm_count, terms, true);
+    return hp.n_blk > 0 && hp.cost < plain_cost;
+}
+
+bool conv2d_umma_fold_supported(const snnb_context* ctx, const ConvArgs& a) {
+    if (!a.shortcut || a.residual || !conv2d_umma_supported(a) || rowwin_supported(a)) return false;
+    if (!(a.sc_stride == 1 || a.sc_stride == 2) || a.shortcut->n != a.out->n || !a.shortcut->lo != !a.in->lo) return false;
+    const TilePlan tp = plan_tiles(a.out->n, a.out->h, a.out->w, a.stride);
+    if (tp.tw <= 0) return false;
+    const int cblocks = (a.in->c + UM_BLOCK_K - 1) / UM_BLOCK_K, terms = conv_terms(ctx, a);
+    const OcPlan op   = plan_oc_ksplit(a.out->c, tp.tiles_x * tp.tiles_y * tp.tiles_n, tp.tw * tp.th * tp.tn, tp.tw, a.k * a.k * cblocks, ctx->sm_count, terms, false,
+                                       a.stream_k);
+    OcPlan hp;
+    return op.n_blk > 0 && !halo_plan(ctx, a, cblocks, terms, op.cost, hp);
+}
+
 enum { ATTR_UMMA = 1u, ATTR_ROWWIN = 2u, ATTR_DW1 = 4u, ATTR_DW2 = 8u };
 
 typedef void (*RowWinKernel)(const CUtensorMap, const CUtensorMap, const CUtensorMap, const CUtensorMap, const CUtensorMap, const CUtensorMap, const CUtensorMap,
@@ -1565,8 +1611,14 @@
 int launch_conv2d_umma(snnb_context* ctx, const ConvArgs& a) {
     EncodeTiledFn encode = get_encode(ctx);
     SNNB_REQUIRE(encode, "launch_conv2d_umma: cuTensorMapEncodeTiled is unavailable in this driver");
-    if (rowwin_supported(a)) return launch_conv2d_rowwin(ctx, a, encode);
-    SNNB_REQUIRE(!a.in->feed_only, "launch_conv2d_umma: the input tensor only exists as a stem feed, which this launch cannot read");
+    if (rowwin_supported(a)) {
+        SNNB_REQUIRE(!a.shortcut, "launch_conv2d_umma: a folded shortcut needs the plain tensor-core kernel, not the row-window kernel");
+        return launch_conv2d_rowwin(ctx, a, encode);
+    }
+    SNNB_REQUIRE(!a.in->feed_only && !(a.shortcut && a.shortcut->feed_only), "launch_conv2d_umma: the input tensor only exists as a stem feed, which this launch cannot read");
+    SNNB_REQUIRE(!(a.shortcut && a.residual), "launch_conv2d_umma: a folded shortcut and a residual operand are exclusive");
+    SNNB_REQUIRE(!a.shortcut || ((a.sc_stride == 1 || a.sc_stride == 2) && a.shortcut->n == a.out->n), "launch_conv2d_umma: unsupported shortcut (stride %d)",
+                 a.sc_stride);
     const snnb_tensor* in = a.in;
     snnb_tensor* out      = a.out;
     UmmaParams p;
@@ -1581,22 +1633,20 @@
     p.tiles_x = tp.tiles_x, p.tiles_y = tp.tiles_y, p.tiles_n = tp.tiles_n;
     p.ksize = a.k, p.stride = a.stride, p.pad_x = a.pad_x, p.pad_y = a.pad_y;
     p.cblocks = (in->c + UM_BLOCK_K - 1) / UM_BLOCK_K;
+    p.sc_cblocks = a.shortcut ? (a.shortcut->c + UM_BLOCK_K - 1) / UM_BLOCK_K : 0, p.sc_stride = a.shortcut ? a.sc_stride : 1;
+    const int num_kb = a.k * a.k * p.cblocks + p.sc_cblocks;
     const int terms = conv_terms(ctx, a);
     p.has_lo        = out->lo != nullptr;
     p.b_stages = 0, p.b_stage_bytes = 0;
-    OcPlan op       = plan_oc_ksplit(out->c, tp.tiles_x * tp.tiles_y * tp.tiles_n, p.rows_used, tp.tw, a.k * a.k * p.cblocks, ctx->sm_count, terms, false, a.stream_k);
-    static const bool no_halo = getenv("SNNB_NO_HALO") != nullptr;
-    bool halo                 = false;
-    if (!no_halo && a.k == 3 && a.stride == 1 && a.pad_x <= 1 && a.pad_y <= 1) {
-        const int hx = (out->w + HL_TW - 1) / HL_TW, hy = (out->h + HL_TH - 1) / HL_TH;
-        const OcPlan hp = plan_oc_ksplit(out->c, hx * hy * out->n, UM_BLOCK_M, HL_TW, 9 * p.cblocks, ctx->sm_count, terms, true);
-        if (hp.n_blk > 0 && hp.cost < op.cost) {
-            halo = true, op = hp;
-            p.b_stage_bytes = (terms == 3 ? 2 : 1) * op.n_blk * 128 <= UM_B_BYTES ? UM_B_BYTES : 2 * UM_B_BYTES;
-            p.b_stages      = HL_B_RING_BYTES / p.b_stage_bytes;
-            p.tw = HL_TW, p.th = HL_TH, p.tn = 1, p.rows_used = UM_BLOCK_M;
-            p.tiles_x = hx, p.tiles_y = hy, p.tiles_n = out->n;
-        }
+    OcPlan op       = plan_oc_ksplit(out->c, tp.tiles_x * tp.tiles_y * tp.tiles_n, p.rows_used, tp.tw, num_kb, ctx->sm_count, terms, false, a.stream_k);
+    OcPlan hp;
+    const bool halo = !a.shortcut && halo_plan(ctx, a, p.cblocks, terms, op.cost, hp);
+    if (halo) {
+        op              = hp;
+        p.b_stage_bytes = (terms == 3 ? 2 : 1) * op.n_blk * 128 <= UM_B_BYTES ? UM_B_BYTES : 2 * UM_B_BYTES;
+        p.b_stages      = HL_B_RING_BYTES / p.b_stage_bytes;
+        p.tw = HL_TW, p.th = HL_TH, p.tn = 1, p.rows_used = UM_BLOCK_M;
+        p.tiles_x = (out->w + HL_TW - 1) / HL_TW, p.tiles_y = (out->h + HL_TH - 1) / HL_TH, p.tiles_n = out->n;
     }
     SNNB_REQUIRE(op.n_blk > 0, "launch_conv2d_umma: no output-channel plan");
     p.n_blk = op.n_blk, p.tiles_oc = op.tiles_oc, p.ksplit = op.ksplit, p.kb_per_split = op.kb_per_split;
@@ -1627,21 +1677,29 @@
     p.act = a.act, p.alpha = a.alpha;
     static const int ablate = getenv("SNNB_UMMA_ABLATE") ? atoi(getenv("SNNB_UMMA_ABLATE")) : 0;
     p.ablate                = ablate;
-    SNNB_REQUIRE(a.w->kp == a.k * a.k * p.ICp, "launch_conv2d_umma: packed weights do not match (kp %d vs %d)", a.w->kp, a.k * a.k * p.ICp);
-
-    CUtensorMap tmA[2], tmB[2];
-    {
-        const cuuint64_t dims[4]    = {(cuuint64_t) in->c, (cuuint64_t) in->w, (cuuint64_t) in->h, (cuuint64_t) in->n};
-        const cuuint64_t strides[3] = {(cuuint64_t) in->cp * 2, (cuuint64_t) in->w * in->cp * 2, (cuuint64_t) in->h * in->w * in->cp * 2};
-        const cuuint32_t box[4]     = {(cuuint32_t) UM_BLOCK_K, (cuuint32_t) (halo ? HL_W : p.tw * a.stride), (cuuint32_t) (halo ? HL_H : p.th * a.stride), (cuuint32_t) p.tn};
-        const cuuint32_t estr[4]    = {1, (cuuint32_t) a.stride, (cuuint32_t) a.stride, 1};
-        __half* planes[2]    = {in->hi, in->lo ? in->lo : in->hi};
+    const int kp_want = a.k * a.k * p.ICp + (a.shortcut ? round_up(a.shortcut->c, 8) : 0);
+    SNNB_REQUIRE(a.w->kp == kp_want, "launch_conv2d_umma: packed weights do not match (kp %d vs %d)", a.w->kp, kp_want);
+
+    auto encode_a = [&](const snnb_tensor* t, int s, int bw, int bh, CUtensorMap (&maps)[2]) {
+        const cuuint64_t dims[4]    = {(cuuint64_t) t->c, (cuuint64_t) t->w, (cuuint64_t) t->h, (cuuint64_t) t->n};
+        const cuuint64_t strides[3] = {(cuuint64_t) t->cp * 2, (cuuint64_t) t->w * t->cp * 2, (cuuint64_t) t->h * t->w * t->cp * 2};
+        const cuuint32_t box[4]     = {(cuuint32_t) UM_BLOCK_K, (cuuint32_t) bw, (cuuint32_t) bh, (cuuint32_t) p.tn};
+        const cuuint32_t estr[4]    = {1, (cuuint32_t) s, (cuuint32_t) s, 1};
+        __half* planes[2]    = {t->hi, t->lo ? t->lo : t->hi};
         for (int i = 0; i < 2; ++i) {
-            CUresult r = encode(&tmA[i], CU_TENSOR_MAP_DATA_TYPE_FLOAT16, 4, planes[i], dims, strides, box, estr, CU_TENSOR_MAP_INTERLEAVE_NONE,
+            CUresult r = encode(&maps[i], CU_TENSOR_MAP_DATA_TYPE_FLOAT16, 4, planes[i], dims, strides, box, estr, CU_TENSOR_MAP_INTERLEAVE_NONE,
                                 CU_TENSOR_MAP_SWIZZLE_128B, CU_TENSOR_MAP_L2_PROMOTION_L2_128B, CU_TENSOR_MAP_FLOAT_OOB_FILL_NONE);
-            SNNB_REQUIRE(r == CUDA_SUCCESS, "cuTensorMapEncodeTiled(A) failed: %d (dims %d %d %d %d box %u %u %u %u)", (int) r, in->c, in->w, in->h, in->n, box[0],
+            SNNB_REQUIRE(r == CUDA_SUCCESS, "cuTensorMapEncodeTiled(A) failed: %d (dims %d %d %d %d box %u %u %u %u)", (int) r, t->c, t->w, t->h, t->n, box[0],
                          box[1], box[2], box[3]);
         }
+        return 0;
+    };
+    CUtensorMap tmA[2], tmB[2], tmS[2];
+    if (encode_a(in, a.stride, halo ? HL_W : p.tw * a.stride, halo ? HL_H : p.th * a.stride, tmA)) return 2;
+    if (!a.shortcut) {
+        tmS[0] = tmA[0], tmS[1] = tmA[1];
+    } else if (encode_a(a.shortcut, a.sc_stride, p.tw * a.sc_stride, p.th * a.sc_stride, tmS)) {
+        return 2;
     }
     {
         const cuuint64_t dims[2]    = {(cuuint64_t) a.w->kp, (cuuint64_t) a.w->ocr};
@@ -1682,7 +1740,7 @@
     const int total_tiles = p.tiles_x * p.tiles_y * p.tiles_n * p.tiles_oc;
     const int grid        = p.sk ? (p.sk_dp > 0 ? ctx->sm_count : p.sk_ctas) : std::min(total_tiles * p.ksplit, ctx->sm_count);
     static const bool no_split_epi = getenv("SNNB_NO_SPLIT_EPI") != nullptr;
-    const bool split_epi           = !halo && !no_split_epi && !p.sk && p.ksplit == 1 && p.ksize * p.ksize * p.cblocks <= 3 && total_tiles >= 2 * grid;
+    const bool split_epi           = !halo && !no_split_epi && !p.sk && p.ksplit == 1 && num_kb <= 3 && total_tiles >= 2 * grid;
     ctx->last_kernel = halo ? "conv_umma_kernel<halo>"
                             : (split_epi ? "conv_umma_kernel<short-K>" : (p.sk ? "conv_umma_kernel<stream-K>" : (p.ksplit > 1 ? "conv_umma_kernel<split-K>" : "conv_umma_kernel")));
     p.trace = nullptr;
@@ -1694,15 +1752,15 @@
     auto* k_halo  = terms == 3 ? conv_umma_kernel<HL_B_STAGES, false, 3, true> : (terms == 2 ? conv_umma_kernel<HL_B_STAGES, false, 2, true> : conv_umma_kernel<HL_B_STAGES, false, 1, true>);
     const cudaError_t le =
         halo      ? launch_k_pdl(k_halo, dim3(grid), dim3(UM_THREADS), HL_SMEM_BYTES, ctx->stream, tmA[0], tmA[1], tmB[0], tmB[1], tmO64[0], tmO64[1], tmOT[0], tmOT[1], tmR64[0],
-                                 tmR64[1], tmRT[0], tmRT[1], p)
+                                 tmR64[1], tmRT[0], tmRT[1], tmS[0], tmS[1], p)
         : split_epi ? launch_k_pdl(k_split, dim3(grid), dim3(UM_THREADS), UM_SMEM_BYTES_SPLIT, ctx->stream, tmA[0], tmA[1], tmB[0], tmB[1], tmO64[0], tmO64[1], tmOT[0], tmOT[1],
-                                 tmR64[0], tmR64[1], tmRT[0], tmRT[1], p)
+                                 tmR64[0], tmR64[1], tmRT[0], tmRT[1], tmS[0], tmS[1], p)
                   : launch_k_pdl(k_plain, dim3(grid), dim3(UM_THREADS), UM_SMEM_BYTES, ctx->stream, tmA[0], tmA[1], tmB[0], tmB[1], tmO64[0], tmO64[1], tmOT[0], tmOT[1], tmR64[0],
-                                 tmR64[1], tmRT[0], tmRT[1], p);
+                                 tmR64[1], tmRT[0], tmRT[1], tmS[0], tmS[1], p);
     if (p.trace) {
         char hdr[256];
         snprintf(hdr, sizeof hdr, "conv k%d s%d IC%d OC%d out %dx%dx%d n_blk %d tiles %d grid %d num_kb %d ksplit %d terms %d halo %d", a.k, a.stride, in->c, out->c, out->n,
-                 out->h, out->w, p.n_blk, total_tiles, grid, p.ksize * p.ksize * p.cblocks, split_epi ? -1 : (p.sk ? -2 : p.ksplit), terms, (int) halo);
+                 out->h, out->w, p.n_blk, total_tiles, grid, num_kb, split_epi ? -1 : (p.sk ? -2 : p.ksplit), terms, (int) halo);
         if (trace_end(ctx, p.trace, hdr)) return 1;
     }
     cudaError_t e = le != cudaSuccess ? le : cudaGetLastError();
@@ -1953,4 +2011,39 @@
     return n;
 }
 
-}
+int kblock_schedule(int ksize, int cblocks, int icp, int sc_cblocks, int tiles, int ksplit, int sms, int* rows, int capacity) {
+    if (ksize < 1 || cblocks < 1 || icp < 8 || sc_cblocks < 0 || tiles < 1 || ksplit < 0 || sms < 1) return -1;
+    UmmaParams p {};
+    p.ksize = ksize, p.cblocks = cblocks, p.ICp = icp, p.sc_cblocks = sc_cblocks, p.sc_stride = 1;
+    const int num_kb = ksize * ksize * cblocks + sc_cblocks;
+    std::vector<WorkItem> items;
+    if (ksplit > 0) {
+        p.ksplit = ksplit, p.kb_per_split = (num_kb + ksplit - 1) / ksplit;
+        for (int work = 0; work < tiles * ksplit; ++work) items.push_back(decode_work<false>(p, work, tiles, num_kb));
+    } else {
+        int dp = 0, ctas = 0;
+        long long units = 0;
+        if (tiles % sms == 0 || !streamk_split(tiles, num_kb, sms, dp, units, ctas)) return -1;
+        p.sk = 1, p.sk_dp = dp, p.sk_ctas = ctas, p.sk_units = units, p.ksplit = 1, p.kb_per_split = num_kb;
+        const int grid = dp > 0 ? sms : ctas, end = dp + 4 * ctas;
+        for (int cta = 0; cta < grid; ++cta)
+            for (int work = sk_first_work(p, cta, end); work < end; work = sk_next_work(p, work, cta, grid, num_kb, end)) items.push_back(decode_work<true>(p, work, tiles, num_kb));
+    }
+    struct Row {
+        int *rows, capacity, ksize, tile, n;
+        __host__ __device__ void operator()(int kb, bool sc, int cb, int kx, int ky, int wcol) {
+            if (n < capacity) {
+                int* r = rows + 6 * (size_t) n;
+                r[0] = tile, r[1] = kb, r[2] = sc, r[3] = ky * ksize + kx, r[4] = cb, r[5] = wcol;
+            }
+            ++n;
+        }
+    } row {rows, capacity, ksize, 0, 0};
+    for (const WorkItem& w : items) {
+        row.tile = w.tile;
+        for_each_kblock(p, w.kb0, w.kb1, row);
+    }
+    return row.n;
+}
+
+}
diff --git a/shadernn_b200/csrc/pack.cpp b/shadernn_b200/csrc/pack.cpp
--- a/shadernn_b200/csrc/pack.cpp
+++ b/shadernn_b200/csrc/pack.cpp
@@ -73,6 +73,30 @@
     }
 }
 
+void pack_shortcut_host(int IC, const float* w_oi, const float* bias, const float* g, const float* b, const float* m, const float* v, PackedHost& out) {
+    const int OC = out.out_ch;
+    std::vector<float> scale, shift;
+    bn_fold(OC, bias, g, b, m, v, scale, shift);
+    const int kp = out.kp + round_up(IC, 8);
+    std::vector<__half> hi((size_t) out.ocr * kp, __float2half_rn(0.0f)), lo((size_t) out.ocr * kp, __float2half_rn(0.0f));
+    for (int o = 0; o < out.ocr; ++o) {
+        std::memcpy(&hi[(size_t) o * kp], &out.w_hi[(size_t) o * out.kp], out.kp * sizeof(__half));
+        std::memcpy(&lo[(size_t) o * kp], &out.w_lo[(size_t) o * out.kp], out.kp * sizeof(__half));
+    }
+    for (int o = 0; o < OC; ++o) {
+        out.bias[o] += shift[o];
+        for (int i = 0; i < IC; ++i) {
+            const float wv  = w_oi[(size_t) o * IC + i] * scale[o];
+            const __half h  = __float2half_rn(wv);
+            const size_t at = (size_t) o * kp + out.kp + i;
+            hi[at] = h;
+            lo[at] = __float2half_rn(wv - __half2float(h));
+        }
+    }
+    out.w_hi.swap(hi), out.w_lo.swap(lo);
+    out.kp = kp;
+}
+
 void pack_rowwin_host(PackedHost& p, int stride, int pad_x) {
     RowPlan rp;
     if (p.kind != 1 || p.in_ch > 8 || p.out_ch > 64 || !make_row_plan(p.kernel, stride, pad_x, rp)) return;
diff --git a/shadernn_b200/csrc/snnb_internal.h b/shadernn_b200/csrc/snnb_internal.h
--- a/shadernn_b200/csrc/snnb_internal.h
+++ b/shadernn_b200/csrc/snnb_internal.h
@@ -145,10 +145,14 @@
     float alpha;
     int precision = -1;
     bool stream_k = false;
+    const snnb_tensor* shortcut = nullptr;
+    int sc_stride = 1;
 };
 int launch_conv2d_simt(snnb_context* ctx, const ConvArgs& a);
 int launch_conv2d_umma(snnb_context* ctx, const ConvArgs& a);
 bool conv2d_umma_supported(const ConvArgs& a);
+bool conv2d_umma_fold_supported(const snnb_context* ctx, const ConvArgs& a);
+int kblock_schedule(int ksize, int cblocks, int icp, int sc_cblocks, int tiles, int ksplit, int sms, int* rows, int capacity);
 int streamk_schedule(int tiles, int num_kb, int sms, int* rows, int capacity);
 int launch_depthwise(snnb_context* ctx, const ConvArgs& a);
 bool depthwise_tma_supported(const ConvArgs& a);
@@ -238,6 +242,7 @@
 };
 void pack_conv2d_host(int IC, int OC, int k, const float* w_oihw, const float* bias, const float* g, const float* b, const float* m, const float* v,
                       PackedHost& out);
+void pack_shortcut_host(int IC, const float* w_oi, const float* bias, const float* g, const float* b, const float* m, const float* v, PackedHost& out);
 void pack_rowwin_host(PackedHost& p, int stride, int pad_x);
 void pack_feed_host(PackedHost& p, int stride, int pad_x);
 void pack_depthwise_host(int C, int k, const float* w_chw, const float* bias, const float* g, const float* b, const float* m, const float* v,
```

Result: faster. 61410 (median of 6 runs) (+5.0%).
